# SoyeonHH/MMDA

Measured on AMD Instinct MI355X. Metric: training samples/sec on MOSEI-shaped synthetic batch, higher is better.
Workload: dtype bf16; 1 GPU; MISA train step, MOSEI shapes B=32/GPU T=50 (d_t,d_v,d_a)=(300,35,74) hidden=128 V=20000, bf16 MFMA operands fp32 accumulate, dropout on, full lengths; global_batch=32, seq_len=50, parallelism=single, use_confidNet=False, rnncell=lstm, dp_global_stats=False

## Files before the change

include/mmda_hip.h:

```cpp
#ifndef MMDA_HIP_H
#define MMDA_HIP_H
#include <stddef.h>
#include <stdint.h>

#ifdef __cplusplus
extern "C" {
#endif

#define MMDA_F32 0
#define MMDA_BF16 1

#define MMDA_CELL_LSTM 0
#define MMDA_CELL_GRU 1

#define MMDA_OK 0
#define MMDA_EINVAL (-1)
#define MMDA_ELAUNCH (-2)

#define MMDA_ACT_NONE 0
#define MMDA_ACT_RELU 1
#define MMDA_ACT_SIGMOID 2
#define MMDA_ACT_LEAKYRELU 3
#define MMDA_ACT_TANH 4
#define MMDA_ACT_ELU 5
// ... 323 lines not shown
int mmda_clamp(float* g, int64_t n, float clip, void* stream);
int mmda_clamp_adam_rows(float* p, const float* g, float* m, float* v, int rows, int dim, const unsigned char* mask, int want, float lr,
                         float beta1, float beta2, float eps, float clip, float grad_scale, int step, void* stream);
int mmda_mark_rows(unsigned char* mask, int rows, const int64_t* ids, int n, void* stream);
int mmda_embed_rows_sparse_adam(float* P, float* M, float* V, const int64_t* ids, int n, int D, const float* rows, const int32_t* lengths,
                                int B, int table_rows, float lr, float beta1, float beta2, float eps, float clip, float grad_scale, int step,
                                void* stream);
int64_t mmda_embed_deferred_scalar_floats(int window);
int mmda_embed_deferred_reset(int32_t* row_step, int table_rows, void* stream);
int mmda_embed_rows_dense_adam(float* P, float* M, float* V, int32_t* row_step, float* step_scalars, int window, const int64_t* ids, int n,
                               int D, const float* rows, const int32_t* lengths, int B, int table_rows, float lr, float beta1, float beta2,
                               float eps, float clip, float grad_scale, int seq, int step, void* stream);
int mmda_embed_rows_catch_up(float* P, float* M, float* V, int32_t* row_step, const float* step_scalars, int window, const int64_t* ids,
                             int n, int D, const int32_t* lengths, int B, int table_rows, float beta1, float beta2, float eps, int upto,
                             void* stream);
int mmda_embed_rows_flush(float* P, float* M, float* V, int32_t* row_step, const float* step_scalars, int window, int D, int table_rows,
                          float beta1, float beta2, float eps, int upto, void* stream);
int mmda_clamp_rmsprop(float* p, const float* g, float* square_avg, int64_t n, float lr, float alpha, float eps, float clip,
                       float grad_scale, void* stream);
int mmda_grad_accumulate(float* acc, const float* g, int64_t n, int first, void* stream);
int mmda_clamp_adam_sum(float* p, const float* acc, const float* g, float* m, float* v, int64_t n, float lr, float beta1, float beta2,
                        float eps, float clip, float grad_scale, int step, void* stream);
int mmda_embed_rows_append(int64_t* ids_out, float* rows_out, int64_t offset, int64_t capacity, const int64_t* ids, const float* rows,
                           int n, int D, const int32_t* lengths, int B, void* stream);
typedef struct mmda_run { int64_t begin, len, first; } mmda_run;
int64_t mmda_runs_build(const int64_t* begin, const int64_t* len, int n, int64_t bucket_floats, mmda_run* out, int* n_out);
int mmda_clamp_adam_runs(float* p, const float* g, float* m, float* v, const mmda_run* runs, int n_runs, int64_t items, float lr,
                         float beta1, float beta2, float eps, float clip, float grad_scale, int step, void* stream);
int mmda_clamp_adam_sum_runs(float* p, const float* acc, const float* g, float* m, float* v, const mmda_run* runs, int n_runs,
                             int64_t items, float lr, float beta1, float beta2, float eps, float clip, float grad_scale, int step,
                             void* stream);
int mmda_clamp_rmsprop_runs(float* p, const float* g, float* square_avg, const mmda_run* runs, int n_runs, int64_t items, float lr,
                            float alpha, float eps, float clip, float grad_scale, void* stream);
typedef struct mmda_adam_opts {
  float beta1, beta2, eps, weight_decay;
  int decoupled;
  const float* scale_dev;
} mmda_adam_opts;
int mmda_clamp_adam_opts(float* p, const float* acc, const float* g, float* m, float* v, int64_t n, const mmda_run* runs, int n_runs,
                         int64_t items, float lr, float clip, float grad_scale, int step, const mmda_adam_opts* opts, void* stream);
int mmda_clamp_adam_rows_opts(float* p, const float* g, float* m, float* v, int rows, int dim, const unsigned char* mask, int want, float lr,
                              float clip, float grad_scale, int step, const mmda_adam_opts* opts, void* stream);
int64_t mmda_grad_norm_partials(int64_t n_or_items);
int mmda_grad_norm(const float* g, const float* acc, int64_t n, const mmda_run* runs, int n_runs, int64_t items, float max_norm,
                   float grad_scale, double* partials, int64_t partials_capacity, float* out2, void* stream);
int mmda_grad_scale(float* g, int64_t n, const mmda_run* runs, int n_runs, int64_t items, const float* scale_dev, void* stream);

typedef struct mmda_misa mmda_misa;
typedef struct mmda_misa_config {
  int vocab, d_t, d_v, d_a, hidden, ncls;
  int act;
  int use_cmd_sim, use_confidNet;
  float dropout;
  float fusion_dropout;
  float threshold, reverse_grad_weight;
  float diff_weight, sim_weight, recon_weight, conf_weight;
  int mode;
  int rnncell;
} mmda_misa_config;

int mmda_misa_create(const mmda_misa_config* cfg, mmda_misa** out);
void mmda_misa_destroy(mmda_misa* m);
int mmda_misa_num_params(const mmda_misa* m);
int mmda_misa_param_info(const mmda_misa* m, int i, const char** name, int64_t* offset, int* rows, int* cols);
int64_t mmda_misa_flat_floats(const mmda_misa* m);
int64_t mmda_misa_dense_floats(const mmda_misa* m);
int mmda_misa_bind(mmda_misa* m, float* params, float* grads, float* adam_m, float* adam_v);
int64_t mmda_misa_workspace_floats(const mmda_misa* m, int B, int T);
#define MMDA_MISA_STEP_SWITCHES 13
typedef struct mmda_misa_step_request { int fused, has_labels, has_opt_step, enc_cached; } mmda_misa_step_request;
typedef struct mmda_misa_step_plan {
  int fused, inf, enc_cut, enc_nostash, enc_cached, bfg, gm, kdg, tn_wgrad, want_b, want_c, want_wT, wT_merge, skinny, row_fuse,
      ffn_fuse_fwd, ffn_fuse_bwd, seed_recon, seed_cls, fj_on, fj_fwd, fj_device, zg_here, rec_hoisted, sort_early, embed_update,
      embed_deferred, embed_bg, embed_bg_late, embed_bg_wgs, embed_bg_lds;
} mmda_misa_step_plan;
int mmda_misa_plan_describe(const mmda_misa* m, int B, int T, const mmda_misa_step_request* req, const int* switches, int n_switches,
                            mmda_misa_step_plan* out);
int mmda_misa_set_workspace(mmda_misa* m, float* ws, int64_t floats, int B, int T);
int mmda_misa_set_workspace_async(mmda_misa* m, float* ws, int64_t floats, int B, int T, void* stream);
int64_t mmda_misa_tensor_offset(const mmda_misa* m, const char* name);
int mmda_misa_set_mode(mmda_misa* m, int mode);
int mmda_misa_set_recurrence(mmda_misa* m, int resident_weights);
int mmda_misa_set_gemm_operands(mmda_misa* m, int bf16_copies);
int mmda_misa_set_inference(mmda_misa* m, int forward_only);
int mmda_misa_set_fusion_fp8(mmda_misa* m, int on);
int mmda_misa_set_embed_update(mmda_misa* m, int mode);
int mmda_misa_set_trainable(mmda_misa* m, const unsigned char* flags, int n_params);
int mmda_misa_trainable_info(const mmda_misa* m, mmda_run* runs, int capacity, int* n_runs, int64_t* trainable_floats, int* encoder_cut_on);
int mmda_misa_set_cut_forward(mmda_misa* m, int keep_stash);
int mmda_misa_set_embed_deferred(mmda_misa* m, int32_t* row_step, float* step_scalars, int window, void* stream);
int mmda_misa_embed_deferred_step(mmda_misa* m, float lr, float beta1, float beta2, float eps, float clip, float grad_scale, int step,
                                  void* stream);
int mmda_misa_embed_flush(mmda_misa* m, void* stream);
int mmda_misa_set_embed_background(mmda_misa* m, int on, int workgroups);
int mmda_misa_embed_background_active(const mmda_misa* m);
int64_t mmda_misa_early_grad_floats(const mmda_misa* m);
int mmda_misa_wait_early_grads(mmda_misa* m, void* stream);
int mmda_misa_set_overlap(mmda_misa* m, int side_stream);
int mmda_misa_cluster_status(const mmda_misa* m, int* aborted_host);

int mmda_misa_forward(mmda_misa* m, const int64_t* t_ids, const float* v, const float* a, const int32_t* lengths,
                      int training, uint64_t seed, void* stream);
int mmda_misa_losses(mmda_misa* m, const float* emo, int with_grads, void* stream);
int mmda_misa_set_external_batch_losses(mmda_misa* m, int on);
int mmda_misa_backward(mmda_misa* m, const int64_t* t_ids, const float* v, const float* a, const int32_t* lengths,
                       void* stream);
int mmda_misa_zero_grad(mmda_misa* m, void* stream);
int mmda_misa_zero_act_grads(mmda_misa* m, void* stream);
int mmda_misa_adam_step(mmda_misa* m, float lr, float clip, float grad_scale, int step, void* stream);
int mmda_misa_set_adam(mmda_misa* m, const mmda_adam_opts* opts, float clip_norm);
int mmda_misa_set_cls_loss(mmda_misa* m, const mmda_cls_opts* opts);
int mmda_misa_set_task(mmda_misa* m, int task, int loss_kind);
int mmda_misa_grad_accumulate(mmda_misa* m, float* acc, int first, int64_t* list_ids, float* list_rows, int64_t list_used,
                              int64_t list_capacity, void* stream);
int mmda_misa_adam_step_accumulated(mmda_misa* m, const float* acc, int64_t* list_ids, float* list_rows, int64_t list_used,
                                    int64_t list_capacity, float lr, float clip, float grad_scale, int step, void* stream);
int mmda_misa_train_step(mmda_misa* m, const int64_t* t_ids, const float* v, const float* a, const int32_t* lengths,
                         const float* emo, int training, uint64_t seed, int do_adam, float lr, float clip, int step,
                         void* stream);

int mmda_misa_timing_stride(mmda_misa* m, int stride);
int mmda_misa_timing_rotate(mmda_misa* m, int on);
int mmda_misa_timing_begin(mmda_misa* m, int max_steps);
int mmda_misa_timing_collect(mmda_misa* m, float mean_ms[4], int* steps);
int mmda_misa_timing_end(mmda_misa* m);

int mmda_collate_gather(const int32_t* words, const float* visual, const float* acoustic, const int64_t* offsets, const float* emo,
                        const float* sentiment, const int32_t* order, int B, int T, int dv, int da, int pad_id, int64_t* out_ids,
                        float* out_v, float* out_a, float* out_emo, float* out_y, void* stream);

typedef struct mmda_infer_src {
  const float* scores; const float* labels; const float* tcp; const float* hfused; const float* x6; const float* probs;
  int ncls, hs, nhead;
} mmda_infer_src;
typedef struct mmda_infer_out {
  float* scores; float* labels; float* tcp; float* hidden; float* utterance; float* attention;
} mmda_infer_out;
int mmda_infer_collect(const mmda_infer_src* src, const mmda_infer_out* out, const int32_t* dst, int64_t base, int B, void* stream);
int mmda_misa_infer_collect(mmda_misa* m, const mmda_infer_out* out, const int32_t* dst, int64_t base, void* stream);

int mmda_encoded_collect(const float* utt_t, const float* utt_v, const float* utt_a, int wt, int wv, int wa, float* tab_t, float* tab_v,
                         float* tab_a, const int32_t* dst, int64_t base, int B, void* stream);
int mmda_encoded_gather(const float* tab_t, const float* tab_v, const float* tab_a, int wt, int wv, int wa, const float* tab_emo, int ncls,
                        const int32_t* rows, int B, float* utt_t, float* utt_v, float* utt_a, float* emo, void* stream);
int mmda_misa_encoded_collect(mmda_misa* m, float* tab_t, float* tab_v, float* tab_a, const int32_t* dst, int64_t base, void* stream);
typedef struct mmda_encoded_batch {
  const float* tab_t; const float* tab_v; const float* tab_a; const float* tab_emo;
  const int32_t* rows; int B;
} mmda_encoded_batch;
int mmda_misa_forward_encoded(mmda_misa* m, const mmda_encoded_batch* eb, int training, uint64_t seed, void* stream);
int mmda_misa_train_step_encoded(mmda_misa* m, const mmda_encoded_batch* eb, float* emo_out, int training, uint64_t seed, int do_adam,
                                 float lr, float clip, int step, void* stream);

typedef struct mmda_modality_p { float p[3]; } mmda_modality_p;
int mmda_collate_gather_masked(const int32_t* words, const float* visual, const float* acoustic, const int64_t* offsets, const float* emo,
                               const float* sentiment, const int32_t* order, int B, int T, int dv, int da, int pad_id, int keep_const,
                               mmda_modality_p p, uint64_t seed, int unk_id, int64_t* out_ids, float* out_v, float* out_a,
                               float* out_emo, float* out_y, uint8_t* out_keep, void* stream);
int mmda_modality_mask(const int64_t* ids, const float* v, const float* a, int T, int B, int dv, int da, const uint8_t* keep,
                       int keep_const, int pad_id, int unk_id, int64_t* out_ids, float* out_v, float* out_a, void* stream);
int mmda_modality_attrib(const float* V, int64_t n, int C, float* phi, float* loo, int32_t* dominant, int64_t* counts, void* stream);

#ifdef __cplusplus
}
#endif
#endif
// ... 1 lines not shown
```

mmda_amd/_lib.py:

```python
from __future__ import annotations

import ctypes as C
import os

_HERE = os.path.dirname(os.path.abspath(__file__))
LIB_PATH = os.path.join(_HERE, "libmmda_hip.so")

F32, BF16 = 0, 1
ACT = {"none": 0, "relu": 1, "sigmoid": 2, "leakyrelu": 3, "tanh": 4, "elu": 5, "hardtanh": 6, "hardshrink": 7, "prelu": 8, "rrelu": 9}

c_f32p = C.c_void_p
c_stream = C.c_void_p


class GemmArgs(C.Structure):
    _fields_ = [("mode", C.c_int), ("transA", C.c_int), ("transB", C.c_int), ("M", C.c_int), ("N", C.c_int), ("K", C.c_int),
                ("batch", C.c_int),
                ("A", C.c_void_p), ("lda", C.c_int), ("strideA", C.c_int64),
                ("A2", C.c_void_p), ("gather", C.c_void_p),
                ("B", C.c_void_p), ("ldb", C.c_int), ("strideB", C.c_int64),
                ("C", C.c_void_p), ("ldc", C.c_int), ("strideC", C.c_int64),
                ("bias", C.c_void_p), ("bias2", C.c_void_p), ("strideBias", C.c_int64),
                ("accumulate", C.c_int), ("act", C.c_int),
                ("drop_p", C.c_float), ("drop_seed", C.c_uint64), ("drop_site", C.c_int),
                ("gate", C.c_void_p), ("ldgate", C.c_int), ("gate_scale", C.c_float),
                ("alpha", C.c_float), ("bias_grad", C.c_void_p), ("bias_grad2", C.c_void_p)]


class GemmBf16Args(C.Structure):
    _fields_ = [("M", C.c_int), ("N", C.c_int), ("K", C.c_int), ("A", C.c_void_p), ("lda", C.c_int), ("B", C.c_void_p), ("ldb", C.c_int),
                ("C", C.c_void_p), ("ldc", C.c_int), ("bias", C.c_void_p), ("bias2", C.c_void_p), ("bias_grad", C.c_void_p),
                ("bias_grad2", C.c_void_p), ("accumulate", C.c_int), ("alpha", C.c_float), ("perm_n_H", C.c_int), ("perm_m_H", C.c_int),
                ("tn", C.c_int)]


class GemmBf16PlanRow(C.Structure):
    _fields_ = [("cls", C.c_int), ("mixed", C.c_int), ("tx", C.c_int), ("ty", C.c_int), ("sk", C.c_int), ("per", C.c_int),
                ("last", C.c_int), ("launch", C.c_int)]


class ConvertJob(C.Structure):
    _fields_ = [("src", C.c_void_p), ("ld", C.c_int), ("rows", C.c_int), ("cols", C.c_int), ("gather", C.c_void_p),
                ("plain", C.c_void_p), ("ldp", C.c_int), ("transposed", C.c_void_p), ("ldt", C.c_int), ("row_perm_H", C.c_int),
                ("src_bf16", C.c_int)]


class SkinnyArgs(C.Structure):
    _fields_ = [("M", C.c_int), ("N", C.c_int), ("K", C.c_int), ("transB", C.c_int),
                ("A", C.c_void_p), ("A2", C.c_void_p), ("lda", C.c_int), ("B", C.c_void_p), ("ldb", C.c_int),
                ("K2", C.c_int), ("A_2nd", C.c_void_p), ("lda_2nd", C.c_int), ("B_2nd", C.c_void_p), ("ldb_2nd", C.c_int),
                ("C", C.c_void_p), ("ldc", C.c_int), ("C2", C.c_void_p), ("ldc2", C.c_int), ("bias", C.c_void_p),
                ("accumulate", C.c_int), ("alpha", C.c_float), ("act", C.c_int),
                ("drop_p", C.c_float), ("drop_seed", C.c_uint64), ("drop_site", C.c_int),
                ("gate", C.c_void_p), ("ldgate", C.c_int), ("gate_scale", C.c_float),
                ("dsig", C.c_void_p), ("dsig2", C.c_void_p), ("lddsig", C.c_int)]


class TransposeJob(C.Structure):
    _fields_ = [("src", C.c_void_p), ("rows", C.c_int), ("cols", C.c_int), ("ld", C.c_int), ("dst", C.c_void_p), ("ldd", C.c_int)]


class ActParams(C.Structure):
    _fields_ = [("slope", C.c_void_p), ("dslope", C.c_void_p), ("lo", C.c_float), ("hi", C.c_float), ("rand", C.c_int),
                ("seed", C.c_uint64), ("site", C.c_int)]


class LnArgs(C.Structure):
    _fields_ = [("rows", C.c_int), ("n", C.c_int), ("x", C.c_void_p), ("res", C.c_void_p), ("gamma", C.c_void_p),
                ("beta", C.c_void_p), ("y", C.c_void_p), ("mean", C.c_void_p), ("rstd", C.c_void_p), ("act", C.c_int),
                ("drop_p", C.c_float), ("drop_seed", C.c_uint64), ("drop_site", C.c_int),
                ("permute_S", C.c_int), ("permute_B", C.c_int), ("eps", C.c_float), ("actp", ActParams),
                ("y_bf16", C.c_void_p), ("ld_bf16", C.c_int)]


class LnBwdArgs(C.Structure):
    _fields_ = [("rows", C.c_int), ("n", C.c_int), ("dy", C.c_void_p), ("x", C.c_void_p), ("res", C.c_void_p),
                ("gamma", C.c_void_p), ("mean", C.c_void_p), ("rstd", C.c_void_p),
                ("d_x", C.c_void_p), ("accumulate_dx", C.c_int), ("d_res", C.c_void_p),
                ("dgamma", C.c_void_p), ("dbeta", C.c_void_p),
                ("act", C.c_int), ("drop_p", C.c_float), ("drop_seed", C.c_uint64), ("drop_site", C.c_int),
                ("permute_S", C.c_int), ("permute_B", C.c_int), ("actp", ActParams)]


class LstmDesc(C.Structure):
    _fields_ = [("H", C.c_int), ("gates", C.c_void_p), ("cstash", C.c_void_p), ("hseq", C.c_void_p),
                ("wpack", C.c_void_p * 2), ("wpack_c", C.c_void_p * 2), ("utt", C.c_void_p), ("layer", C.c_int), ("d_hseq", C.c_void_p),
                ("xchg", C.c_void_p), ("epoch_base", C.c_uint32), ("gate_minor", C.c_int), ("forward_only", C.c_int),
                ("cell", C.c_int), ("dg_bf16", C.c_void_p), ("dg_bf16_only", C.c_int)]


class LstmPlan(C.Structure):
    _fields_ = [("ok", C.c_int), ("form", C.c_int), ("wpb", C.c_int), ("groups", C.c_int), ("groups_per_launch", C.c_int),
                ("launches", C.c_int), ("wg_per_group", C.c_int), ("wg_per_desc", C.c_int * 4), ("gru", C.c_int),
                ("gate_minor", C.c_int), ("no_stash", C.c_int), ("dhseq", C.c_int), ("pair", C.c_int),
                ("kernel", C.c_int)]


class MisaStepRequest(C.Structure):
    _fields_ = [("fused", C.c_int), ("has_labels", C.c_int), ("has_opt_step", C.c_int), ("enc_cached", C.c_int)]


STEP_PLAN_FIELDS = ("fused", "inf", "enc_cut", "enc_nostash", "enc_cached", "bfg", "gm", "kdg", "tn_wgrad", "want_b", "want_c", "want_wT",
                    "wT_merge", "skinny", "row_fuse", "ffn_fuse_fwd", "ffn_fuse_bwd", "seed_recon", "seed_cls", "fj_on", "fj_fwd",
                    "fj_device", "zg_here", "rec_hoisted", "sort_early", "embed_update", "embed_deferred", "embed_bg", "embed_bg_late",
                    "embed_bg_wgs", "embed_bg_lds")
STEP_SWITCHES = {"MMDA_GEMM_TN": 1, "MMDA_WT_MERGE": 1, "MMDA_ROW_FUSE": 1, "MMDA_FFN_FUSE": 1, "MMDA_LOSS_SEEDS": 1, "MMDA_FLAG_JOIN": 1,
                 "MMDA_ZERO_GRAD_SIDE": -1, "MMDA_FUSED_SPLIT": 1, "MMDA_SORT_EARLY": 1, "MMDA_EMBED_BG": 1, "MMDA_EMBED_BG_WGS": 0,
                 "MMDA_EMBED_BG_LATE": 0, "MMDA_EMBED_BG_LDS": 1024}


class MisaStepPlan(C.Structure):
    _fields_ = [(k, C.c_int) for k in STEP_PLAN_FIELDS]


class LossForms(C.Structure):
    _fields_ = [("diff_form", C.c_int), ("diff_products", C.c_int), ("diff_loss_sum", C.c_int), ("diff_combine_blocks", C.c_int),
                ("cmd_form", C.c_int), ("cmd_grid", C.c_int), ("recon_blocks", C.c_int), ("misc_recon_blocks", C.c_int)]


class RankPlan(C.Structure):
    _fields_ = [("rows_per_wg", C.c_int), ("tile", C.c_int), ("tiles", C.c_int), ("splits", C.c_int), ("tiles_per_split", C.c_int),
                ("grid_x", C.c_int), ("grid_y", C.c_int), ("grid_z", C.c_int), ("counts_bytes", C.c_int64)]


class GruPadJob(C.Structure):
    _fields_ = [("H", C.c_int), ("D", C.c_int), ("w_ih", C.c_void_p * 2), ("w_hh", C.c_void_p * 2), ("b_ih", C.c_void_p * 2),
                ("b_hh", C.c_void_p * 2), ("pw_ih", C.c_void_p), ("pw_hh", C.c_void_p * 2), ("pb_ih", C.c_void_p), ("pb_hh", C.c_void_p)]


class MisaConfig(C.Structure):
    _fields_ = [("vocab", C.c_int), ("d_t", C.c_int), ("d_v", C.c_int), ("d_a", C.c_int), ("hidden", C.c_int), ("ncls", C.c_int),
                ("act", C.c_int), ("use_cmd_sim", C.c_int), ("use_confidNet", C.c_int),
                ("dropout", C.c_float), ("fusion_dropout", C.c_float), ("threshold", C.c_float),
                ("reverse_grad_weight", C.c_float),
                ("diff_weight", C.c_float), ("sim_weight", C.c_float), ("recon_weight", C.c_float), ("conf_weight", C.c_float),
                ("mode", C.c_int), ("rnncell", C.c_int)]


# ... 103 lines not shown
    "mmda_attn_bwd": (_I, [_P, _P, _P, _I, _I, _I, _I, _P, _F, _U64, _I, _P]),
    "mmda_add": (_I, [_P, _P, _P, _I64, _P]),
    "mmda_sigmoid_bwd_inplace": (_I, [_P, _P, _I64, _P]),
    "mmda_act_dropout_fwd": (_I, [_P, _P, _I64, _I, _F, _U64, _I, _P]),
    "mmda_act_dropout_bwd": (_I, [_P, _P, _P, _I64, _I, _F, _U64, _I, _P]),
    "mmda_act_dropout_fwd_p": (_I, [_P, _P, _I64, _I, C.POINTER(ActParams), _F, _U64, _I, _P]),
    "mmda_act_dropout_bwd_p": (_I, [_P, _P, _P, _I64, _I, C.POINTER(ActParams), _F, _U64, _I, _P]),
    "mmda_heads_fwd": (_I, [_P, _I, _I, _F, _P, _P, _P, _F, _U64, _I, _P]),
    "mmda_heads_bwd": (_I, [_P, _P, _P, _P, _I, _I, _P, _F, _U64, _I, _P]),
    "mmda_heads_fwd_task": (_I, [_P, _I, _I, _F, _P, _P, _P, _F, _U64, _I, _I, _P]),
    "mmda_heads_bwd_task": (_I, [_P, _P, _P, _P, _I, _I, _P, _F, _U64, _I, _I, _P]),
    "mmda_loss_reg": (_I, [_P, _P, _I, _I, _I, _F, _P, _P, _P]),
    "mmda_senti_accumulate": (_I, [_P, _P, _I64, _P, _P]),
    "mmda_senti_finish": (_I, [_P, _P, _P]),
    "mmda_reliab_accumulate": (_I, [_P, _P, _I64, _I, _I, _P, _P]),
    "mmda_reliab_finish": (_I, [_P, _I, _I, _P, _P, _P]),
    "mmda_scaling_work_bytes": (_I64, [_I64, _I]),
    "mmda_scaling_fit": (_I, [_P, _P, _I64, _I, _I, _I, _I, _P, _I64, _P, _P, _P, _P, _P]),
    "mmda_scaling_apply": (_I, [_P, _P, _P, _I64, _I, _P, _P]),
    "mmda_misa_set_task": (_I, [_P, _I, _I]),
    "mmda_loss_cls": (_I, [_P, _P, _I, _I, _F, _P, _P, _P]),
    "mmda_loss_cls_opts": (_I, [_P, _P, _I, _I, _F, _P, _P, C.POINTER(ClsOpts), _P]),
    "mmda_loss_misc_opts": (_I, [_P, _P, _P, _I, _I, _P, _P, _I, _I, _F, _P, _P, _I64, _F, _P, _P, _P, _F, _F, _F, _F, _I,
                                 C.POINTER(ClsOpts), _P]),
    "mmda_label_counts": (_I, [_P, _I64, _I, _P, _P]),
    "mmda_misa_set_cls_loss": (_I, [_P, C.POINTER(ClsOpts)]),
    "mmda_loss_conf": (_I, [_P, _P, _P, _I, _I, _F, _P, _P, _P, _P]),
    "mmda_loss_diff": (_I, [_P, _I64, _I, _I, _F, _P, _P, _P, _P]),
    "mmda_loss_diff_work_floats": (_I64, [_I, _I]),
    "mmda_loss_diff_pairs": (_I, [_P, _I64, _I, _I, C.POINTER(C.c_int), _I, _I, _F, _P, _P, _P, _P]),
    "mmda_loss_cmd_pairs": (_I, [_P, _I64, _I, _I, C.POINTER(C.c_int), _I, _I, _I, _F, _F, _P, _P, _P]),
    "mmda_loss_cmd": (_I, [_P, _I64, _I, _I, _F, _P, _P, _P]),
    "mmda_loss_recon": (_I, [_P, _P, _I64, _I, _I, _F, _P, _P, _P, _P]),
    "mmda_loss_misc": (_I, [_P, _P, _P, _I, _I, _P, _P, _I, _I, _F, _P, _P, _I64, _F, _P, _P, _P, _F, _F, _F, _F, _I, _P]),
    "mmda_eval_accumulate": (_I, [_P, _P, _I, _I, _P, _P]),
    "mmda_calib_accumulate": (_I, [_P, _P, _I64, _I, _P, _I, _P, _P, _P]),
    "mmda_calib_select": (_I, [_P, _P, _I, _I, _P, _I, _I, _P, _P, _P, _P]),
    "mmda_eval_accumulate_thr": (_I, [_P, _P, _I, _I, _P, _P, _P, _P]),
    "mmda_rank_plan_describe": (_I, [_I64, _I, C.POINTER(RankPlan)]),
    "mmda_rank_counts": (_I, [_P, _P, _I64, _I, _P, _P]),
    "mmda_rank_finish": (_I, [_P, _P, _I64, _I, C.c_double, _P, _P]),
    "mmda_rank_rows_accumulate": (_I, [_P, _P, _I64, _I, _P, _P]),
    "mmda_loss_domain": (_I, [_P, _I, _F, _P, _P, _P]),
    "mmda_loss_forms_describe": (_I, [_I, _I, _I, _I, _I, _I64, C.POINTER(LossForms)]),
    "mmda_clamp_adam": (_I, [_P, _P, _P, _P, _I64, _F, _F, _F, _F, _F, _F, _I, _P]),
    "mmda_clamp_adam_rows": (_I, [_P, _P, _P, _P, _I, _I, _P, _I, _F, _F, _F, _F, _F, _F, _I, _P]),
    "mmda_embed_rows_sparse_adam": (_I, [_P, _P, _P, _P, _I, _I, _P, _P, _I, _I, _F, _F, _F, _F, _F, _F, _I, _P]),
    "mmda_mark_rows": (_I, [_P, _I, _P, _I, _P]),
    "mmda_embed_deferred_scalar_floats": (_I64, [_I]),
    "mmda_embed_deferred_reset": (_I, [_P, _I, _P]),
    "mmda_embed_rows_dense_adam": (_I, [_P, _P, _P, _P, _P, _I, _P, _I, _I, _P, _P, _I, _I, _F, _F, _F, _F, _F, _F, _I, _I, _P]),
    "mmda_embed_rows_catch_up": (_I, [_P, _P, _P, _P, _P, _I, _P, _I, _I, _P, _I, _I, _F, _F, _F, _I, _P]),
    "mmda_embed_rows_flush": (_I, [_P, _P, _P, _P, _P, _I, _I, _I, _F, _F, _F, _I, _P]),
    "mmda_clamp": (_I, [_P, _I64, _F, _P]),
    "mmda_clamp_rmsprop": (_I, [_P, _P, _P, _I64, _F, _F, _F, _F, _F, _P]),
    "mmda_grad_accumulate": (_I, [_P, _P, _I64, _I, _P]),
    "mmda_clamp_adam_sum": (_I, [_P, _P, _P, _P, _P, _I64, _F, _F, _F, _F, _F, _F, _I, _P]),
    "mmda_embed_rows_append": (_I, [_P, _P, _I64, _I64, _P, _P, _I, _I, _P, _I, _P]),
    "mmda_runs_build": (_I64, [C.POINTER(_I64), C.POINTER(_I64), _I, _I64, C.POINTER(Run), C.POINTER(_I)]),
    "mmda_clamp_adam_runs": (_I, [_P, _P, _P, _P, _P, _I, _I64, _F, _F, _F, _F, _F, _F, _I, _P]),
    "mmda_clamp_adam_sum_runs": (_I, [_P, _P, _P, _P, _P, _P, _I, _I64, _F, _F, _F, _F, _F, _F, _I, _P]),
    "mmda_clamp_rmsprop_runs": (_I, [_P, _P, _P, _P, _I, _I64, _F, _F, _F, _F, _F, _P]),
    "mmda_clamp_adam_opts": (_I, [_P, _P, _P, _P, _P, _I64, _P, _I, _I64, _F, _F, _F, _I, C.POINTER(AdamOpts), _P]),
    "mmda_clamp_adam_rows_opts": (_I, [_P, _P, _P, _P, _I, _I, _P, _I, _F, _F, _F, _I, C.POINTER(AdamOpts), _P]),
    "mmda_grad_norm_partials": (_I64, [_I64]),
    "mmda_grad_norm": (_I, [_P, _P, _I64, _P, _I, _I64, _F, _F, _P, _I64, _P, _P]),
    "mmda_grad_scale": (_I, [_P, _I64, _P, _I, _I64, _P, _P]),
    "mmda_misa_set_adam": (_I, [_P, C.POINTER(AdamOpts), _F]),
    "mmda_misa_create": (_I, [C.POINTER(MisaConfig), C.POINTER(C.c_void_p)]),
    "mmda_misa_destroy": (None, [_P]),
    "mmda_misa_num_params": (_I, [_P]),
    "mmda_misa_param_info": (_I, [_P, _I, C.POINTER(C.c_char_p), C.POINTER(_I64), C.POINTER(_I), C.POINTER(_I)]),
    "mmda_misa_flat_floats": (_I64, [_P]),
    "mmda_misa_dense_floats": (_I64, [_P]),
    "mmda_misa_bind": (_I, [_P, _P, _P, _P, _P]),
    "mmda_misa_workspace_floats": (_I64, [_P, _I, _I]),
    "mmda_misa_plan_describe": (_I, [_P, _I, _I, C.POINTER(MisaStepRequest), C.POINTER(C.c_int), _I, C.POINTER(MisaStepPlan)]),
    "mmda_misa_set_workspace": (_I, [_P, _P, _I64, _I, _I]),
    "mmda_misa_set_workspace_async": (_I, [_P, _P, _I64, _I, _I, _P]),
    "mmda_misa_tensor_offset": (_I64, [_P, C.c_char_p]),
    "mmda_misa_set_mode": (_I, [_P, _I]),
    "mmda_misa_set_overlap": (_I, [_P, _I]),
    "mmda_misa_set_recurrence": (_I, [_P, _I]),
    "mmda_misa_set_gemm_operands": (_I, [_P, _I]),
    "mmda_misa_early_grad_floats": (_I64, [_P]),
    "mmda_misa_wait_early_grads": (_I, [_P, _P]),
    "mmda_misa_set_inference": (_I, [_P, _I]),
    "mmda_misa_set_fusion_fp8": (_I, [_P, _I]),
    "mmda_misa_set_embed_update": (_I, [_P, _I]),
    "mmda_misa_set_trainable": (_I, [_P, C.c_char_p, _I]),
    "mmda_misa_trainable_info": (_I, [_P, C.POINTER(Run), _I, C.POINTER(_I), C.POINTER(_I64), C.POINTER(_I)]),
    "mmda_misa_set_cut_forward": (_I, [_P, _I]),
    "mmda_misa_set_embed_deferred": (_I, [_P, _P, _P, _I, _P]),
    "mmda_misa_embed_deferred_step": (_I, [_P, _F, _F, _F, _F, _F, _F, _I, _P]),
    "mmda_misa_embed_flush": (_I, [_P, _P]),
    "mmda_misa_set_embed_background": (_I, [_P, _I, _I]),
    "mmda_misa_embed_background_active": (_I, [_P]),
    "mmda_misa_cluster_status": (_I, [_P, C.POINTER(_I)]),
    "mmda_misa_forward": (_I, [_P, _P, _P, _P, _P, _I, _U64, _P]),
    "mmda_misa_losses": (_I, [_P, _P, _I, _P]),
    "mmda_misa_set_external_batch_losses": (_I, [_P, _I]),
    "mmda_misa_backward": (_I, [_P, _P, _P, _P, _P, _P]),
    "mmda_misa_zero_grad": (_I, [_P, _P]),
    "mmda_misa_zero_act_grads": (_I, [_P, _P]),
    "mmda_misa_adam_step": (_I, [_P, _F, _F, _F, _I, _P]),
    "mmda_misa_grad_accumulate": (_I, [_P, _P, _I, _P, _P, _I64, _I64, _P]),
    "mmda_misa_adam_step_accumulated": (_I, [_P, _P, _P, _P, _I64, _I64, _F, _F, _F, _I, _P]),
    "mmda_misa_timing_stride": (_I, [_P, _I]),
    "mmda_misa_timing_rotate": (_I, [_P, _I]),
    "mmda_misa_timing_begin": (_I, [_P, _I]),
    "mmda_misa_timing_collect": (_I, [_P, C.POINTER(C.c_float * 4), C.POINTER(_I)]),
    "mmda_misa_timing_end": (_I, [_P]),
    "mmda_misa_train_step": (_I, [_P, _P, _P, _P, _P, _P, _I, _U64, _I, _F, _F, _I, _P]),
    "mmda_collate_gather": (_I, [_P, _P, _P, _P, _P, _P, _P, _I, _I, _I, _I, _I, _P, _P, _P, _P, _P, _P]),
    "mmda_infer_collect": (_I, [C.POINTER(InferSrc), C.POINTER(InferOut), _P, _I64, _I, _P]),
    "mmda_misa_infer_collect": (_I, [_P, C.POINTER(InferOut), _P, _I64, _P]),
    "mmda_encoded_collect": (_I, [_P, _P, _P, _I, _I, _I, _P, _P, _P, _P, _I64, _I, _P]),
    "mmda_encoded_gather": (_I, [_P, _P, _P, _I, _I, _I, _P, _I, _P, _I, _P, _P, _P, _P, _P]),
    "mmda_misa_encoded_collect": (_I, [_P, _P, _P, _P, _P, _I64, _P]),
    "mmda_misa_forward_encoded": (_I, [_P, C.POINTER(EncodedBatch), _I, _U64, _P]),
    "mmda_misa_train_step_encoded": (_I, [_P, C.POINTER(EncodedBatch), _P, _I, _U64, _I, _F, _F, _I, _P]),
    "mmda_collate_gather_masked": (_I, [_P, _P, _P, _P, _P, _P, _P, _I, _I, _I, _I, _I, _I, ModalityP, _U64, _I, _P, _P, _P, _P, _P, _P, _P]),
    "mmda_modality_mask": (_I, [_P, _P, _P, _I, _I, _I, _I, _P, _I, _I, _I, _P, _P, _P, _P]),
    "mmda_modality_attrib": (_I, [_P, _I64, _I, _P, _P, _P, _P, _P]),
}

_lib = None


class MMDAError(RuntimeError):
    pass


def load():
    global _lib
    if _lib is not None:
        return _lib
    if not os.path.exists(LIB_PATH):
        raise MMDAError(f"{LIB_PATH} not found: the HIP hot-path library is not built (make -C mmda_amd/csrc); "
                        "there is no CPU/PyTorch fallback")
    lib = C.CDLL(LIB_PATH)
    for name, (res, args) in SIGNATURES.items():
        fn = getattr(lib, name)
        fn.restype = res
        fn.argtypes = args
    _lib = lib
    return lib


def check(rc, what=""):
    if rc != 0:
        lib = load()
        msg = lib.mmda_last_error()
        raise MMDAError(f"{what} failed with code {rc}: {msg.decode() if msg else ''}")


def ptr(t):
    return None if t is None else t.data_ptr()


def stream_ptr():
    import torch
    return torch.cuda.current_stream().cuda_stream
```

mmda_amd/csrc/lstm.hip:

```cpp
#include "common.h"
#include "internal.h"
#include "convert_tile.h"
#include "transpose_tile.h"

namespace {

constexpr int NW = 4;
constexpr int MAXDESC = 4;

struct LstmLaunch {
  mmda_lstm_desc d[MAXDESC];
  int n, B, T, nbt;
  const int32_t* lengths;
};

__device__ __forceinline__ int pad16(int h) { return (h + 15) & ~15; }
__device__ __forceinline__ int pad32(int h) { return (h + 31) & ~31; }

template <int MODE>
__global__ void pack_kernel(int H, const float* __restrict__ W, void* outF, void* outB) {
  const int Hp = pad16(H), nHT = Hp / 16;
  const int per = (MODE == MMDA_BF16) ? 8 : 4;
  const int kspan = (MODE == MMDA_BF16) ? 32 : 16;
  const int KS = (MODE == MMDA_BF16) ? pad32(H) / 32 : Hp / 16;
// ... 432 lines not shown
  if (mode == MMDA_BF16) {
    int used = 0;
    int rc = mmda_lstm_cluster_launch(n, descs, B, T, lengths, stream, bwd, &used);
    if (rc != MMDA_OK) return rc;
    if (used) return MMDA_OK;
  }
  for (int i = 0; i < n; ++i)
    if (descs[i].gate_minor) return MMDA_EINVAL;
  int Hp = round_up(maxH, 16), Kp = round_up(maxH, 32);
  size_t lds;
  if (!bwd) lds = (mode == MMDA_BF16) ? (size_t)2 * 16 * (Kp + 8) * 2 : (size_t)2 * 16 * (Kp + 2) * 4;
  else lds = (mode == MMDA_BF16) ? (size_t)16 * (4 * Hp + 8) * 2 : (size_t)16 * (4 * Hp + 2) * 4;
  if (lds > 160 * 1024) return MMDA_EINVAL;
  int maxt = pick_maxt(n, descs);
  hipStream_t s = (hipStream_t)stream;
  int rc;
  const bool gru = descs[0].cell == MMDA_CELL_GRU;
#define PICK(MODE_)                                                                                              \
  (gru ? (bwd ? launch<MODE_, true, MMDA_CELL_GRU>(maxt, L, lds, s) : launch<MODE_, false, MMDA_CELL_GRU>(maxt, L, lds, s))  \
       : (bwd ? launch<MODE_, true, MMDA_CELL_LSTM>(maxt, L, lds, s) : launch<MODE_, false, MMDA_CELL_LSTM>(maxt, L, lds, s)))
  if (mode == MMDA_BF16) rc = PICK(MMDA_BF16);
  else rc = PICK(MMDA_F32);
#undef PICK
  if (rc != MMDA_OK) return rc;
  MMDA_CHECK_LAUNCH(bwd ? "mmda_lstm_bwd" : "mmda_lstm_fwd");
  return MMDA_OK;
}

}

extern "C" int64_t mmda_lstm_packed_bytes(int mode, int H, int backward) {
  if (H <= 0 || H > 512) return MMDA_EINVAL;
  int Hp = round_up(H, 16), nHT = Hp / 16;
  if (backward == 2) return mode == MMDA_BF16 ? (int64_t)nHT * nHT * 2 * 64 * 8 * 2 : MMDA_EINVAL;
  if (mode == MMDA_BF16) {
    int KS = round_up(H, 32) / 32, KSB = 4 * Hp / 32;
    return backward ? (int64_t)nHT * KSB * 64 * 8 * 2 : (int64_t)nHT * 4 * KS * 64 * 8 * 2;
  } else if (mode == MMDA_F32) {
    int KG = Hp / 16, KGB = 4 * Hp / 16;
    return backward ? (int64_t)nHT * KGB * 64 * 4 * 4 : (int64_t)nHT * 4 * KG * 64 * 4 * 4;
  }
  return MMDA_EINVAL;
}

extern "C" int mmda_lstm_pack_whh(int mode, int H, const float* whh, void* packed_fwd, void* packed_bwd, void* stream) {
  if (!whh || H <= 0 || H > 512 || (!packed_fwd && !packed_bwd)) return MMDA_EINVAL;
  hipStream_t s = (hipStream_t)stream;
  int64_t total = (mmda_lstm_packed_bytes(mode, H, 0) + mmda_lstm_packed_bytes(mode, H, 1)) / (mode == MMDA_BF16 ? 2 : 4);
  int blocks = (int)((total + 255) / 256);
  if (blocks > 2048) blocks = 2048;
  if (mode == MMDA_BF16) hipLaunchKernelGGL(pack_kernel<MMDA_BF16>, dim3(blocks), dim3(256), 0, s, H, whh, packed_fwd, packed_bwd);
  else if (mode == MMDA_F32) hipLaunchKernelGGL(pack_kernel<MMDA_F32>, dim3(blocks), dim3(256), 0, s, H, whh, packed_fwd, packed_bwd);
  else return MMDA_EINVAL;
  MMDA_CHECK_LAUNCH("mmda_lstm_pack_whh");
  return MMDA_OK;
}

namespace {
int pack_build(int mode, int n, const int* H, const float* const* whh, void* const* packed_fwd, void* const* packed_bwd,
               void* const* packed_c, PackMulti& P, int& blocks) {
  if (n <= 0 || n > 16 || !H || !whh || !packed_fwd || !packed_bwd || (mode != MMDA_BF16 && mode != MMDA_F32)) return MMDA_EINVAL;
  P.n = n;
  blocks = 0;
  for (int i = 0; i < n; ++i) {
    if (H[i] <= 0 || H[i] > 512 || !whh[i] || (!packed_fwd[i] && !packed_bwd[i])) return MMDA_EINVAL;
    P.H[i] = H[i]; P.W[i] = whh[i]; P.F[i] = packed_fwd[i]; P.Bk[i] = packed_bwd[i];
    P.Ck[i] = (packed_c && mode == MMDA_BF16) ? packed_c[i] : nullptr;
    P.start[i] = blocks;
    int64_t total = (mmda_lstm_packed_bytes(mode, H[i], 0) + mmda_lstm_packed_bytes(mode, H[i], 1)) / 16;
    if (P.Ck[i]) total += mmda_lstm_packed_bytes(mode, H[i], 2) / 16;
    blocks += (int)((total + 255) / 256);
  }
  for (int i = n; i < 16; ++i) { P.H[i] = P.H[0]; P.W[i] = P.W[0]; P.F[i] = P.F[0]; P.Bk[i] = P.Bk[0]; P.Ck[i] = P.Ck[0]; }
  for (int i = n; i <= 16; ++i) P.start[i] = blocks;
  return MMDA_OK;
}
}

int mmda_lstm_pack_convert_transpose_stamped(int n, const int* H, const float* const* whh, void* const* packed_fwd, void* const* packed_bwd,
                                             void* const* packed_c, const mmda_convert_job* jobs, int njobs, const mmda_transpose_job* tjobs,
                                             int ntjobs, const RowStamp* st, void* stream) {
  if (!jobs || njobs < 0 || njobs > CONV_MAX) return MMDA_EINVAL;
  if (st && (!st->stamp || !st->ids || st->n < 0 || st->table_rows <= 0)) return MMDA_EINVAL;
  PackMulti P;
  int pblocks = 0, cblocks = 0, tblocks = 0;
  int rc = pack_build(MMDA_BF16, n, H, whh, packed_fwd, packed_bwd, packed_c, P, pblocks);
  if (rc) return rc;
  ConvLaunch L;
  rc = conv_build(jobs, njobs, L, cblocks);
  if (rc) return rc;
  TrLaunch R;
  rc = tr_build(tjobs, ntjobs, R, tblocks);
  if (rc) return rc;
  if (pblocks + cblocks + tblocks == 0) return st ? MMDA_EINVAL : MMDA_OK;
  hipLaunchKernelGGL(pack_convert_kernel, dim3(pblocks + cblocks + tblocks), dim3(256), 0, (hipStream_t)stream, P, L, R, pblocks,
                     pblocks + cblocks, st ? *st : RowStamp{nullptr, 0u, 0, nullptr, 0});
  MMDA_CHECK_LAUNCH("mmda_lstm_pack_convert_transpose");
  return MMDA_OK;
}

extern "C" int mmda_lstm_pack_convert_transpose(int n, const int* H, const float* const* whh, void* const* packed_fwd,
                                                void* const* packed_bwd, void* const* packed_c, const mmda_convert_job* jobs, int njobs,
                                                const mmda_transpose_job* tjobs, int ntjobs, void* stream) {
  return mmda_lstm_pack_convert_transpose_stamped(n, H, whh, packed_fwd, packed_bwd, packed_c, jobs, njobs, tjobs, ntjobs, nullptr, stream);
}

extern "C" int mmda_lstm_pack_whh_and_convert(int n, const int* H, const float* const* whh, void* const* packed_fwd, void* const* packed_bwd,
                                              void* const* packed_c, const mmda_convert_job* jobs, int njobs, void* stream) {
  return mmda_lstm_pack_convert_transpose(n, H, whh, packed_fwd, packed_bwd, packed_c, jobs, njobs, nullptr, 0, stream);
}

extern "C" int mmda_lstm_pack_whh_multi(int mode, int n, const int* H, const float* const* whh, void* const* packed_fwd,
                                        void* const* packed_bwd, void* const* packed_c, void* stream) {
  PackMulti P;
  int blocks = 0;
  const int rc0 = pack_build(mode, n, H, whh, packed_fwd, packed_bwd, packed_c, P, blocks);
  if (rc0) return rc0;
  hipStream_t s = (hipStream_t)stream;
  if (mode == MMDA_BF16) hipLaunchKernelGGL(pack_multi_kernel<MMDA_BF16>, dim3(blocks), dim3(256), 0, s, P);
  else hipLaunchKernelGGL(pack_multi_kernel<MMDA_F32>, dim3(blocks), dim3(256), 0, s, P);
  MMDA_CHECK_LAUNCH("mmda_lstm_pack_whh_multi");
  return MMDA_OK;
}

extern "C" int mmda_lstm_pack_whh_cluster(int H, const float* whh, void* packed_c, void* stream) {
  if (!whh || !packed_c || H <= 0 || H > 512) return MMDA_EINVAL;
  PackMulti P;
  P.n = 1;
  for (int i = 0; i < 16; ++i) { P.H[i] = H; P.W[i] = whh; P.F[i] = nullptr; P.Bk[i] = nullptr; P.Ck[i] = packed_c; }
  const int64_t total = (mmda_lstm_packed_bytes(MMDA_BF16, H, 0) + mmda_lstm_packed_bytes(MMDA_BF16, H, 1) +
                         mmda_lstm_packed_bytes(MMDA_BF16, H, 2)) / 16;
  const int blocks = (int)((total + 255) / 256);
  P.start[0] = 0;
  for (int i = 1; i <= 16; ++i) P.start[i] = blocks;
  hipLaunchKernelGGL(pack_multi_kernel<MMDA_BF16>, dim3(blocks), dim3(256), 0, (hipStream_t)stream, P);
  MMDA_CHECK_LAUNCH("mmda_lstm_pack_whh_cluster");
  return MMDA_OK;
}

namespace {
struct GruPad { mmda_gru_pad_job j[MMDA_GRU_PAD_MAX]; int start[MMDA_GRU_PAD_MAX + 1]; int n; };

template <bool UNPAD>
__global__ void gru_pad_kernel(GruPad P) {
  int i = 0;
#pragma unroll
  for (int k = 1; k < MMDA_GRU_PAD_MAX; ++k)
    if (k < P.n && (int)blockIdx.x >= P.start[k]) i = k;
  const mmda_gru_pad_job& J = P.j[i];
  const int H = J.H, D = J.D;
  const int64_t nih = (int64_t)8 * H * D, nhh = (int64_t)4 * H * H, nb = 8 * H;
  int64_t e = (int64_t)(blockIdx.x - P.start[i]) * blockDim.x + threadIdx.x;
  if (e < nih) {
    const int row = (int)(e / D), col = (int)(e % D);
    const int dir = row / (4 * H), slot = (row % (4 * H)) / H, u = row % H;
    float* t = J.w_ih[dir] + ((int64_t)slot * H + u) * D + col;
    if (!UNPAD) J.pw_ih[e] = slot < 3 ? *t : 0.f;
    else { float v = J.pw_ih[e]; J.pw_ih[e] = 0.f; if (slot < 3) *t += v; }
    return;
  }
  e -= nih;
  if (e < 2 * nhh) {
    const int dir = (int)(e / nhh);
    const int64_t e3 = e % nhh;
    const int row = (int)(e3 / H), col = (int)(e3 % H), slot = row / H, u = row % H;
    const int tg = slot == 3 ? 2 : slot;
    float* t = J.w_hh[dir] + ((int64_t)tg * H + u) * H + col;
    if (!UNPAD) J.pw_hh[dir][e3] = slot != 2 ? *t : 0.f;
    else { float v = J.pw_hh[dir][e3]; J.pw_hh[dir][e3] = 0.f; if (slot != 2) *t += v; }
    return;
  }
  e -= 2 * nhh;
  if (e < nb) {
    const int dir = (int)e / (4 * H), slot = ((int)e % (4 * H)) / H, u = (int)e % H;
    const int tg = slot == 3 ? 2 : slot;
    float* ti = J.b_ih[dir] + slot * H + u;
    float* th = J.b_hh[dir] + tg * H + u;
    if (!UNPAD) {
      J.pb_ih[e] = slot < 3 ? *ti : 0.f;
      J.pb_hh[e] = slot != 2 ? *th : 0.f;
    } else {
      float v = J.pb_ih[e]; J.pb_ih[e] = 0.f;
      if (slot < 3) *ti += v;
      if (slot != 2) *th += v;
    }
  }
// ... 36 lines not shown
```

mmda_amd/csrc/misa.hip:

```cpp
#include "step_plan.h"
#include <algorithm>
#include <cstring>

using namespace mmda_step;

namespace {

enum { SITE_ATTN = 1, SITE_DROP1 = 2, SITE_FFN = 3, SITE_DROP2 = 4, SITE_CLS = 5, SITE_DISC = 6,
       SITE_RRELU = 7 , SITE_RRELU_DISC = 10 };

struct OptStep { float lr, clip, grad_scale; int step; const float* acc; bool norm; };
struct PendingRows {
  const int64_t* ids = nullptr; const int32_t* lengths = nullptr; bool on = false;
  void set(const int64_t* i, const int32_t* l) { ids = i; lengths = l; on = true; }
  PendingRows take() { const PendingRows r = *this; *this = PendingRows{}; return r; }
};
struct RowList { int64_t* ids; float* rows; int64_t used, capacity; };
struct StepRequest {
  bool fused = false;
  const float* emo = nullptr;
  const OptStep* opt = nullptr;
  bool enc_cached = false;
};

}

struct mmda_misa {
  explicit mmda_misa(const mmda_misa_config& c) : cfg(c), par(build_params(c)) {}
  mmda_misa(const mmda_misa&) = delete;
  mmda_misa_config cfg;
  const ParamTable par;
  const Workspace& lay = lay_;
  void rebind(const Workspace& v) { lay_ = v; }
  float *P = nullptr, *G = nullptr, *M1 = nullptr, *V1 = nullptr;
  float* ws = nullptr;
  float* xchg_ws = nullptr; int xchg_B = 0; int abort_sticky = 0;
  mmda_adam_opts adam = {0.9f, 0.999f, 1e-8f, 0.f, 0, nullptr};
  float clip_norm = 0.f;
  mmda_cls_opts cls_opts = {}; int cls_on = 0;
  const mmda_cls_opts* cls() const { return cls_on ? &cls_opts : nullptr; }
  int reg = REG_NONE;
  int fusion_fp8 = 0;
  int embed_update = EU_DENSE;
  std::vector<mmda_run> runs;
  int prefix_frozen = 0;
  int embed_flag = 1;
  int enc_frozen = 0;
  int cut_keep_stash = 0;
  int32_t* df_row_step = nullptr; float* df_ring = nullptr; int df_window = 0;
  int use_side = 1;
  int use_cluster = 1;
  int use_bf16_gemm = 1;
  int inference = 0;
  int ext_batch_losses = 0;
  int ev_stride = 1;
  int ev_rotate = 0;
  hipStream_t side = nullptr;
  hipEvent_t ev_fork = nullptr, ev_join = nullptr, ev_pack = nullptr;
  hipEvent_t ev_early = nullptr;
  hipStream_t bg = nullptr; hipEvent_t ev_bg_fork = nullptr, ev_bg_done = nullptr;
  unsigned* row_stamp = nullptr; unsigned bg_epoch = 0u;
  int bg_on = -1, bg_wgs = 0;
  int bg_pending = 0, bg_active = 0;
  unsigned* jflags = nullptr;
  mmda_run* runs_dev = nullptr; int runs_dev_cap = 0; int runs_dirty = 1;
  std::vector<hipEvent_t> ev;
  StepPlan plan;
  int64_t early_floats = 0; int early_valid = 0;
  int64_t adam_early_done = 0;
  int wT_valid = 0;
  int wT_pending = 0;
  PendingRows eu;
  int df_seq = 0, df_flushed = 0;
  int training = 0; uint64_t seed = 0;
  unsigned epoch = 1;
  int side_pending = 0;
  int zero_grad_pending = 0;
  int eager_done = 0;
  const float* misc_deferred = nullptr;
  unsigned jval[2] = {0u, 0u};
  int esort_valid = 0; unsigned esort_val = 0u;
  int fj1 = 0, fj2 = 0, fj1_armed = 0;
  int ev_steps = 0, ev_fwd = 0, ev_bwd = 0;
  int ev_seen_f = 0, ev_seen_b = 0;
  std::vector<char> ev_done;

 private:
  Workspace lay_{};
};

namespace {

struct Ctx {
  mmda_misa* m; void* s; int rc = 0;
  bool grouping = false; std::vector<mmda_gemm_args> pending;
  bool absent_next = false; std::vector<mmda_gemm_args> absent;
  bool deferring = false; std::vector<mmda_gemm_args> deferred;
};

void group_begin(Ctx& c) { c.grouping = true; c.pending.clear(); c.absent.clear(); }
void group_end(Ctx& c) {
  c.grouping = false;
  if (!c.rc && !c.pending.empty())
    c.rc = mmda_gemm_grouped_sized(c.pending.data(), (int)c.pending.size(), c.absent.data(), (int)c.absent.size(), c.s);
  c.pending.clear(); c.absent.clear();
}

void gemm(Ctx& c, int mode, int tA, int tB, int M, int N, int K, const float* A, int lda, const float* Bp, int ldb, float* C,
          int ldc, const float* bias = nullptr, const float* bias2 = nullptr, int acc = 0, int act = 0, int batch = 1,
          int64_t sA = 0, int64_t sB = 0, int64_t sC = 0, int64_t sBias = 0, mmda_gemm_args* extra = nullptr) {
  if (c.rc) return;
  mmda_gemm_args g = {};
  if (extra) g = *extra;
  g.mode = mode; g.transA = tA; g.transB = tB; g.M = M; g.N = N; g.K = K; g.batch = batch;
  g.A = A; g.lda = lda; g.strideA = sA; g.B = Bp; g.ldb = ldb; g.strideB = sB; g.C = C; g.ldc = ldc; g.strideC = sC;
  g.bias = bias; g.bias2 = bias2; g.strideBias = sBias; g.accumulate = acc; g.act = act;
  if (c.absent_next) { c.absent_next = false; if (c.grouping) c.absent.push_back(g); return; }
  if (c.deferring && tA && acc) c.deferred.push_back(g);
  else if (c.grouping) c.pending.push_back(g);
  else c.rc = mmda_gemm(&g, c.s);
}

int side_fork(mmda_misa* m, void* main_stream, void** out);
int side_launch(mmda_misa* m, std::vector<mmda_gemm_args>& list, void* main_stream);
int side_join(mmda_misa* m, void* main_stream);
void lin_fwd(Ctx& c, int mode, int M, int N, int K, const float* x, const float* W, const float* b, float* y, int act = 0) {
  gemm(c, mode, 0, 1, M, N, K, x, K, W, K, y, N, b, nullptr, 0, act);
}
void lin_dx(Ctx& c, int mode, int M, int N, int K, const float* dy, const float* W, float* dx, int acc) {
  gemm(c, mode, 0, 0, M, K, N, dy, N, W, K, dx, K, nullptr, nullptr, acc);
}
void lin_dw(Ctx& c, int mode, int M, int N, int K, const float* dy, const float* x, float* dW, float* db) {
  mmda_gemm_args e = {};
  e.bias_grad = db;
  gemm(c, mode, 1, 0, N, K, M, dy, N, x, K, dW, K, nullptr, nullptr, 1, 0, 1, 0, 0, 0, 0, &e);
}

mmda_skinny_args sk_nt(int M, int N, int K, const float* x, int ldx, const float* W, const float* b, float* y, int ldy, int act = 0) {
  mmda_skinny_args g = {};
  g.M = M; g.N = N; g.K = K; g.transB = 1; g.A = x; g.lda = ldx; g.B = W; g.ldb = K; g.C = y; g.ldc = ldy; g.bias = b; g.act = act;
  return g;
}
mmda_skinny_args sk_nn(int M, int N, int K, const float* dy, int lddy, const float* W, float* dx, int lddx, int acc) {
  mmda_skinny_args g = {};
  g.M = M; g.N = K; g.K = N; g.transB = 0; g.A = dy; g.lda = lddy; g.B = W; g.ldb = K; g.C = dx; g.ldc = lddx; g.accumulate = acc;
  return g;
}
mmda_skinny_args sk_dx(int M, int N, int K, const float* dy, int lddy, const float* WT, float* dx, int lddx, int acc) {
  mmda_skinny_args g = {};
  g.M = M; g.N = K; g.K = N; g.transB = 1; g.A = dy; g.lda = lddy; g.B = WT; g.ldb = N; g.C = dx; g.ldc = lddx; g.accumulate = acc;
  return g;
}
mmda_skinny_args sk_dxw(bool wt, int M, int N, int K, const float* dy, int lddy, const float* WT, const float* W, float* dx, int lddx,
// ... 188 lines not shown
  *r0 = a; *n = b - a; *items = m->runs[b].first - m->runs[a].first;
}
int runs_ready(mmda_misa* m, void* stream) {
  if (!m->runs_dirty && m->runs_dev) return MMDA_OK;
  const int need = (int)m->runs.size();
  if (hipStreamSynchronize((hipStream_t)stream) != hipSuccess) return MMDA_ELAUNCH;
  if (m->side && hipStreamSynchronize(m->side) != hipSuccess) return MMDA_ELAUNCH;
  if (need > m->runs_dev_cap) {
    if (m->runs_dev) (void)hipFree(m->runs_dev);
    m->runs_dev = nullptr; m->runs_dev_cap = 0;
    const int cap = (int)m->par.params.size() + 1;
    if (hipMalloc(reinterpret_cast<void**>(&m->runs_dev), sizeof(mmda_run) * cap) != hipSuccess) { m->runs_dev = nullptr; return MMDA_ELAUNCH; }
    m->runs_dev_cap = cap;
  }
  if (hipMemcpy(m->runs_dev, m->runs.data(), sizeof(mmda_run) * need, hipMemcpyHostToDevice) != hipSuccess) return MMDA_ELAUNCH;
  m->runs_dirty = 0;
  return MMDA_OK;
}
constexpr mmda_adam_opts kAdamDefaults = {0.9f, 0.999f, 1e-8f, 0.f, 0, nullptr};
int bucket_adam(mmda_misa* m, int64_t lo, int64_t hi, const float* acc, float lr, float clip, float grad_scale, int step, const FlagWait& w,
                void* stream, const float* scale_dev = nullptr) {
  const AdamHyper h{lr, m->adam.beta1, m->adam.beta2, m->adam.eps, clip, grad_scale, step, m->adam.weight_decay, m->adam.decoupled, scale_dev};
  if (!masked(m)) return mmda_adam_launch(m->P + lo, acc ? acc + lo : nullptr, m->G + lo, m->M1 + lo, m->V1 + lo, hi - lo, nullptr, h, w, stream);
  int r0 = 0, n = 0; int64_t items = 0;
  runs_slice(m, lo, hi, &r0, &n, &items);
  if (n > 0 && (m->runs_dirty || !m->runs_dev)) return MMDA_EINVAL;
  const RunTable t{n > 0 ? m->runs_dev + r0 : nullptr, n, items};
  return mmda_adam_launch(m->P, acc, m->G, m->M1, m->V1, 0, &t, h, w, stream);
}
int bucket_norm(mmda_misa* m, const float* acc, float grad_scale, void* stream) {
  if (!m->ws || m->lay.gnorm < 0) return MMDA_EINVAL;
  double* parts = reinterpret_cast<double*>(m->ws + m->lay.gnorm_parts);
  const int64_t cap = mmda_grad_norm_partials(INT64_MAX);
  const int64_t hi = grad_floats(m);
  if (!masked(m)) return mmda_grad_norm_launch(m->G, acc, hi, nullptr, m->clip_norm, grad_scale, parts, cap, m->ws + m->lay.gnorm, stream);
  int r0 = 0, n = 0; int64_t items = 0;
  runs_slice(m, 0, hi, &r0, &n, &items);
  if (n > 0 && (m->runs_dirty || !m->runs_dev)) return MMDA_EINVAL;
  const RunTable t{n > 0 ? m->runs_dev + r0 : nullptr, n, items};
  return mmda_grad_norm_launch(m->G, acc, 0, &t, m->clip_norm, grad_scale, parts, cap, m->ws + m->lay.gnorm, stream);
}
bool adam_settings_refused(const mmda_misa* m) {
  if (m->adam.weight_decay > 0.f && m->df_row_step) return true;
  if (m->clip_norm > 0.f && (m->embed_update == EU_SPARSE || m->df_row_step)) return true;
  return false;
}
int apply_trainable(mmda_misa* m, const unsigned char* flags) {
  const int np = (int)m->par.params.size();
  std::vector<int64_t> begin, len;
  int prefix_frozen = 0, embed_flag = 1, enc_frozen = 1;
  for (int i = 0; i < np; ++i) {
    const ParamInfo& p = m->par.params[i];
    const bool on = !flags || flags[i] != 0;
    const std::string top = p.name.substr(0, p.name.find('.'));
    if (p.off == m->par.embed) embed_flag = on ? 1 : 0;
    else if (!on) prefix_frozen = 1;
    if (on && ((p.off >= m->par.rnn2_begin && p.off < m->par.embed) || top == "tlayer_norm" || top == "vlayer_norm" || top == "alayer_norm")) enc_frozen = 0;
    if (!on) continue;
    begin.push_back(p.off);
    len.push_back((i + 1 < np ? m->par.params[i + 1].off : m->par.flat) - p.off);
  }
  const int64_t cuts[3] = {m->par.rnn2_begin, m->par.rnn1_begin, m->par.embed};
  std::vector<mmda_run> runs(begin.size() + 1);
  int n = 0;
  const int64_t items = mmda_runs_build_cut(begin.data(), len.data(), (int)begin.size(), m->par.flat, cuts, 3, runs.data(), &n);
  if (items < 0) return MMDA_EINVAL;
  runs.resize(n + 1);
  runs[n] = mmda_run{m->par.flat, 0, items};
  m->runs.swap(runs);
  m->prefix_frozen = prefix_frozen; m->embed_flag = embed_flag; m->enc_frozen = enc_frozen;
  m->runs_dirty = 1;
  return MMDA_OK;
}

const StepSwitches& step_switches() {
  static const StepSwitches d, sw = {
      mmda_env_int("MMDA_GEMM_TN", d.gemm_tn), mmda_env_int("MMDA_WT_MERGE", d.wt_merge), mmda_env_int("MMDA_ROW_FUSE", d.row_fuse),
      mmda_env_int("MMDA_FFN_FUSE", d.ffn_fuse), mmda_env_int("MMDA_LOSS_SEEDS", d.loss_seeds), mmda_env_int("MMDA_FLAG_JOIN", d.flag_join),
      mmda_env_int("MMDA_ZERO_GRAD_SIDE", d.zero_grad_side), mmda_env_int("MMDA_FUSED_SPLIT", d.fused_split),
      mmda_env_int("MMDA_SORT_EARLY", d.sort_early), mmda_env_int("MMDA_EMBED_BG", d.embed_bg), mmda_env_int("MMDA_EMBED_BG_WGS", d.embed_bg_wgs),
      mmda_env_int("MMDA_EMBED_BG_LATE", d.embed_bg_late), mmda_env_int("MMDA_EMBED_BG_LDS", d.embed_bg_lds)};
  return sw;
}
PlanInput plan_input(const mmda_misa* m, const StepRequest& r, int B, int T) {
  PlanInput in = {};
  in.cfg = m->cfg; in.B = B; in.T = T;
  for (int i = 0; i < 3; ++i) { in.H[i] = m->par.mod[i].H; in.xchg[i] = mmda_lstm_xchg_bytes(in.H[i], B) > 0; }
  in.use_side = m->use_side != 0; in.use_cluster = m->use_cluster != 0; in.use_bf16_gemm = m->use_bf16_gemm != 0;
  in.inference = m->inference != 0; in.fusion_fp8 = m->fusion_fp8 != 0;
  in.embed_update = m->embed_update; in.embed_deferred = m->embed_update == EU_DENSE && m->df_row_step != nullptr;
  in.masked = masked(m); in.encoder_cut = encoder_cut(m); in.cut_keep_stash = m->cut_keep_stash != 0;
  in.bg_on = m->bg_on; in.bg_wgs = m->bg_wgs; in.moments = m->M1 && m->V1;
  in.fused = r.fused; in.has_labels = r.emo != nullptr; in.has_opt = r.opt != nullptr; in.enc_cached = r.enc_cached;
  return in;
}

}

extern "C" int mmda_misa_create(const mmda_misa_config* cfg, mmda_misa** out) {
  if (!cfg || !out) return MMDA_EINVAL;
  if (cfg->vocab <= 0 || cfg->d_t <= 0 || cfg->d_v <= 0 || cfg->d_a <= 0 || cfg->hidden <= 0 || cfg->ncls <= 0) return MMDA_EINVAL;
  if (cfg->d_t > 512 || cfg->d_v > 512 || cfg->d_a > 512 || cfg->hidden % NHEAD || cfg->hidden > 1024) return MMDA_EINVAL;
  if (cfg->mode != MMDA_F32 && cfg->mode != MMDA_BF16) return MMDA_EINVAL;
  if (cfg->rnncell != MMDA_CELL_LSTM && cfg->rnncell != MMDA_CELL_GRU) return MMDA_EINVAL;
  mmda_misa* m = new mmda_misa(*cfg);
  if (apply_trainable(m, nullptr)) { delete m; return MMDA_EINVAL; }
  *out = m;
  return MMDA_OK;
}
extern "C" void mmda_misa_destroy(mmda_misa* m) {
  if (!m) return;
  if (m->ev_fork) (void)hipEventDestroy(m->ev_fork);
  if (m->ev_join) (void)hipEventDestroy(m->ev_join);
  if (m->ev_pack) (void)hipEventDestroy(m->ev_pack);
  if (m->ev_early) (void)hipEventDestroy(m->ev_early);
  if (m->bg) { (void)hipStreamSynchronize(m->bg); (void)hipStreamDestroy(m->bg); }
  if (m->ev_bg_fork) (void)hipEventDestroy(m->ev_bg_fork);
  if (m->ev_bg_done) (void)hipEventDestroy(m->ev_bg_done);
  if (m->row_stamp) (void)hipFree(m->row_stamp);
  if (m->side) (void)hipStreamDestroy(m->side);
  if (m->jflags) (void)hipFree(m->jflags);
  if (m->runs_dev) (void)hipFree(m->runs_dev);
  for (hipEvent_t e : m->ev) (void)hipEventDestroy(e);
  delete m;
}
extern "C" int mmda_misa_num_params(const mmda_misa* m) { return m ? (int)m->par.params.size() : MMDA_EINVAL; }
extern "C" int mmda_misa_param_info(const mmda_misa* m, int i, const char** name, int64_t* offset, int* rows, int* cols) {
  if (!m || i < 0 || i >= (int)m->par.params.size()) return MMDA_EINVAL;
  const ParamInfo& p = m->par.params[i];
  if (name) *name = p.name.c_str();
  if (offset) *offset = p.off;
  if (rows) *rows = p.rows;
  if (cols) *cols = p.cols;
  return MMDA_OK;
}
extern "C" int64_t mmda_misa_flat_floats(const mmda_misa* m) { return m ? m->par.flat : MMDA_EINVAL; }
extern "C" int64_t mmda_misa_dense_floats(const mmda_misa* m) { return m ? m->par.dense : MMDA_EINVAL; }
extern "C" int mmda_misa_bind(mmda_misa* m, float* params, float* grads, float* adam_m, float* adam_v) {
  if (!m || !params) return MMDA_EINVAL;
  if (((uintptr_t)params | (uintptr_t)grads | (uintptr_t)adam_m | (uintptr_t)adam_v) & 15) return MMDA_EINVAL;
  m->P = params; m->G = grads; m->M1 = adam_m; m->V1 = adam_v;
  return MMDA_OK;
}
extern "C" int64_t mmda_misa_workspace_floats(const mmda_misa* m, int B, int T) {
  if (!m || B <= 0 || T <= 0) return MMDA_EINVAL;
  return carve(m->cfg, m->par, B, T).floats;
}
extern "C" int mmda_misa_plan_describe(const mmda_misa* m, int B, int T, const mmda_misa_step_request* req, const int* switches,
                                       int n_switches, mmda_misa_step_plan* out) {
  if (!m || !req || !out || B <= 0 || T <= 0 || (switches && n_switches != MMDA_MISA_STEP_SWITCHES)) return MMDA_EINVAL;
  static const float labels = 0.f; static const OptStep opt = {};
  const StepRequest r{req->fused != 0, req->has_labels ? &labels : nullptr, req->has_opt_step ? &opt : nullptr, req->enc_cached != 0};
  StepSwitches sw;
  if (switches) memcpy(&sw, switches, sizeof(sw));
  const StepPlan P = plan_step(plan_input(m, r, B, T), sw);
  *out = mmda_misa_step_plan{P.fused, P.inf, P.enc_cut, P.enc_nostash, P.enc_cached, P.bfg, P.gm, P.kdg, P.tn_wgrad, P.want_b, P.want_c,
                             P.want_wT, P.wT_merge, P.skinny, P.row_fuse, P.ffn_fuse_fwd, P.ffn_fuse_bwd, P.seed_recon, P.seed_cls, P.fj_on,
                             P.fj_fwd, P.fj_device, P.zg_here, P.rec_hoisted, P.sort_early, P.embed_update, P.embed_deferred, P.embed_bg,
                             P.embed_bg_late, P.embed_bg_wgs, P.embed_bg_lds};
  return MMDA_OK;
}
namespace {
int harvest_abort(mmda_misa* m) {
  if (!m->ws || !m->xchg_ws || m->xchg_ws != m->ws) return MMDA_OK;
  for (int i = 0; i < 3; ++i) {
    if (m->lay.mod[i].xchg < 0) continue;
    unsigned w = 0;
    if (hipMemcpy(&w, m->ws + m->lay.mod[i].xchg, sizeof(w), hipMemcpyDeviceToHost) != hipSuccess) return MMDA_ELAUNCH;
    if (w) m->abort_sticky = 1;
  }
  return MMDA_OK;
}
}

extern "C" int mmda_misa_set_workspace_async(mmda_misa* m, float* ws, int64_t floats, int B, int T, void* stream) {
  if (!m || !ws || B <= 0 || T <= 0 || ((uintptr_t)ws & 15)) return MMDA_EINVAL;
  const Workspace w = carve(m->cfg, m->par, B, T);
  if (floats < w.floats) return MMDA_EINVAL;
  const bool keep = m->xchg_ws == ws && m->xchg_B == B;
  if (!keep && m->xchg_ws == ws) { int rc = harvest_abort(m); if (rc) return rc; }
  m->rebind(w);
  m->ws = ws;
  hipStream_t s = (hipStream_t)stream;
  if (!keep) {
    for (int i = 0; i < 3; ++i)
      if (w.mod[i].xchg >= 0 && hipMemsetAsync(ws + w.mod[i].xchg, 0, sizeof(float) * w.mod[i].xchg_floats, s) != hipSuccess) return MMDA_ELAUNCH;
    m->xchg_ws = ws; m->xchg_B = B;
  }
  if (w.gpad_end > w.gpad_begin && hipMemsetAsync(ws + w.gpad_begin, 0, sizeof(float) * (w.gpad_end - w.gpad_begin), s) != hipSuccess)
    return MMDA_ELAUNCH;
  return MMDA_OK;
}
extern "C" int mmda_misa_set_workspace(mmda_misa* m, float* ws, int64_t floats, int B, int T) {
  return mmda_misa_set_workspace_async(m, ws, floats, B, T, nullptr);
}
extern "C" int64_t mmda_misa_tensor_offset(const mmda_misa* m, const char* name) {
  if (!m || !name || !m->ws) return -1;
  return tensor_offset(m->lay, name);
}
extern "C" int mmda_misa_set_mode(mmda_misa* m, int mode) {
  if (!m || (mode != MMDA_F32 && mode != MMDA_BF16)) return MMDA_EINVAL;
  m->cfg.mode = mode;
  return MMDA_OK;
}
extern "C" int mmda_misa_set_overlap(mmda_misa* m, int side_stream) {
  if (!m) return MMDA_EINVAL;
  m->use_side = side_stream ? 1 : 0;
  return MMDA_OK;
}
extern "C" int mmda_misa_set_recurrence(mmda_misa* m, int resident_weights) {
  if (!m) return MMDA_EINVAL;
  m->use_cluster = resident_weights ? 1 : 0;
  return MMDA_OK;
}
extern "C" int mmda_misa_set_gemm_operands(mmda_misa* m, int bf16_copies) {
  if (!m) return MMDA_EINVAL;
  m->use_bf16_gemm = bf16_copies ? 1 : 0;
  return MMDA_OK;
}
extern "C" int64_t mmda_misa_early_grad_floats(const mmda_misa* m) {
  return (m && m->early_valid) ? m->early_floats : 0;
}
extern "C" int mmda_misa_wait_early_grads(mmda_misa* m, void* stream) {
  if (!m || !m->early_valid || !m->ev_early) return MMDA_EINVAL;
  if (hipStreamWaitEvent((hipStream_t)stream, m->ev_early, 0) != hipSuccess) return MMDA_ELAUNCH;
  return MMDA_OK;
}
extern "C" int mmda_misa_set_external_batch_losses(mmda_misa* m, int on) {
  if (!m) return MMDA_EINVAL;
  m->ext_batch_losses = on ? 1 : 0;
  return MMDA_OK;
}
extern "C" int mmda_misa_set_inference(mmda_misa* m, int forward_only) {
  if (!m) return MMDA_EINVAL;
  m->inference = forward_only ? 1 : 0;
  return MMDA_OK;
}
extern "C" int mmda_misa_cluster_status(const mmda_misa* m, int* aborted_host) {
  if (!m || !m->ws || !aborted_host) return MMDA_EINVAL;
  *aborted_host = m->abort_sticky;
  if (m->jflags) {
    unsigned w = 0;
    if (hipMemcpy(&w, m->jflags + 2, sizeof(w), hipMemcpyDeviceToHost) != hipSuccess) return MMDA_ELAUNCH;
    if (w) *aborted_host |= 2;
  }
  for (int i = 0; i < 3; ++i) {
    if (m->lay.mod[i].xchg < 0) continue;
    unsigned w = 0;
    if (hipMemcpy(&w, m->ws + m->lay.mod[i].xchg, sizeof(w), hipMemcpyDeviceToHost) != hipSuccess) return MMDA_ELAUNCH;
    if (w) *aborted_host = 1;
  }
  return MMDA_OK;
}

namespace {
void weight_transpose_jobs(mmda_misa* m, std::vector<mmda_transpose_job>& tj) {
  const mmda_misa_config& c = m->cfg;
  const ParamTable& p = m->par; const Workspace& w = m->lay;
  const int hs_ = c.hidden, NC_ = 6 + c.ncls;
  auto T_ = [&](int64_t src, int rows, int cols, int64_t dst) { tj.push_back(mmda_transpose_job{PP(src), rows, cols, cols, WS(dst), rows}); };
  T_(p.head_w, NC_, 6 * hs_, w.head_wT); T_(p.l2_w, hs_, FFN, w.l2_wT); T_(p.l1_w, FFN, hs_, w.l1_wT);
  T_(p.out_w, hs_, hs_, w.out_wT); T_(p.in_w, 3 * hs_, hs_, w.in_wT); T_(p.sh_w, hs_, hs_, w.sh_wT);
  for (int i = 0; i < 3; ++i) {
    T_(p.rec_w + (int64_t)i * hs_ * hs_, hs_, hs_, w.rec_wT + (int64_t)i * hs_ * hs_);
    T_(p.priv_w + (int64_t)i * hs_ * hs_, hs_, hs_, w.priv_wT + (int64_t)i * hs_ * hs_);
    T_(p.mod[i].pw, hs_, 4 * p.mod[i].H, w.pwT[i]);
  }
  if (!c.use_cmd_sim) { T_(p.d1_w, hs_, hs_, w.d1_wT); T_(p.d2_w, 3, hs_, w.d2_wT); }
}
int weight_transposes(mmda_misa* m, void* ss) {
  std::vector<mmda_transpose_job> tj;
  weight_transpose_jobs(m, tj);
  const int rc = mmda_transpose_f32(tj.data(), (int)tj.size(), ss);
  m->wT_valid = rc ? 0 : 1;
  m->wT_pending = 0;
  return rc;
}

int backward_only_jobs(mmda_misa* m, mmda_convert_job* cj) {
  const ParamTable& p = m->par; const Workspace& w = m->lay;
  const int R = w.B * w.T;
  int n = 0;
  for (int i = 0; i < 3; ++i) {
    const ModP& md = p.mod[i]; const ModW& mw = w.mod[i];
    for (int l = 0; l < 2; ++l) {
      const RnnP& r = md.rnn[l]; const RnnW& rw = mw.rnn[l];
      if (m->plan.tn_wgrad) {
        for (int d = 0; d < 2; ++d)
          cj[n++] = mmda_convert_job{WS(mw.hseq[l]) + d * md.H, 2 * md.H, R, md.H, nullptr, WS(rw.hbp[d]), r.ldH, nullptr, 0};
      } else {
        cj[n++] = mmda_convert_job{WS(mw.hseq[l]), 2 * md.H, R, 2 * md.H, nullptr, nullptr, 0, WS(rw.hbT), w.ldR};
      }
    }
    if (!m->plan.tn_wgrad) cj[n++] = mmda_convert_job{WS(mw.normed), 2 * md.H, R, 2 * md.H, nullptr, nullptr, 0, WS(mw.rnn[1].xbT), w.ldR};
  }
  return n;
}

int eager_side_losses(mmda_misa* m, void* stream) {
  const StepPlan& P = m->plan;
  if (!P.fused) return MMDA_OK;
  const mmda_misa_config& c = m->cfg; const Workspace& w = m->lay;
  const int B = w.B, hs = c.hidden;
  const int64_t BH = (int64_t)B * hs;
  void* ss = nullptr;
  int rc = side_fork(m, stream, &ss);
  if (!rc && m->wT_pending) rc = weight_transposes(m, B >= 128 ? stream : ss);
  const int64_t zend = P.seed_cls ? w.zero_cls : P.seed_recon ? w.zero_recon : w.zero_end;
  if (!rc && P.zg_here && m->zero_grad_pending) {
    rc = mmda_zero2(WS(w.zero_begin), zend - w.zero_begin, m->G, grad_floats(m), ss);
    m->zero_grad_pending = 0;
  } else if (!rc) {
    if (hipMemsetAsync(WS(w.zero_begin), 0, sizeof(float) * (zend - w.zero_begin), (hipStream_t)ss) != hipSuccess) rc = MMDA_ELAUNCH;
  }
  float* L = WS(w.losses);
  if (!rc) rc = mmda_loss_diff(WS(w.x6), BH, B, hs, c.diff_weight, L + 1, WS(w.d_x6), WS(w.diff_work), ss);
  m->fj1_armed = (!rc && c.use_cmd_sim && P.fj_fwd && m->jflags && mmda_loss_cmd_sets_flag(B, hs)) ? 1 : 0;
  if (!rc && c.use_cmd_sim) {
    static const int sim_pairs[6] = {0, 1, 0, 2, 2, 1};
    rc = mmda_loss_cmd_pairs_tail(WS(w.x6 + 3 * BH), BH, 3, 3, sim_pairs, 5, B, hs, c.sim_weight, 1.0f / 3.0f, L + 2, WS(w.d_x6 + 3 * BH), ss,
                                  m->fj1_armed ? m->jflags + 0 : nullptr, m->jval[0] + 1);
  }
  if (!rc && m->zero_grad_pending) { rc = mmda_misa_zero_grad(m, stream); m->zero_grad_pending = 0; }
  m->eager_done = 1;
  return rc;
}
}

namespace {
int ffn_fp8(mmda_misa* m, float p_tf, uint64_t seed, void* stream) {
  const mmda_misa_config& c = m->cfg; const ParamTable& p = m->par; const Workspace& w = m->lay;
  const int hs = c.hidden, R6 = 6 * w.B;
  if ((hs % 128) != 0) return MMDA_EINVAL;
  auto U8 = [&](int64_t off) { return reinterpret_cast<unsigned char*>(m->ws + off); };
  mmda_mx8_quant_job q[3] = {
      {m->ws + w.x1, hs, R6, hs, U8(w.x1q), U8(w.x1s)},
      {m->P + p.l1_w, hs, FFN, hs, U8(w.w1q), U8(w.w1s)},
      {m->P + p.l2_w, FFN, hs, FFN, U8(w.w2q), U8(w.w2s)}};
  int rc = mmda_mx8_quant(q, 3, stream);
  if (rc) return rc;
  mmda_mx8_args g = {};
  g.M = R6; g.N = FFN; g.K = hs; g.Aq = U8(w.x1q); g.As = U8(w.x1s); g.Bq = U8(w.w1q); g.Bs = U8(w.w1s);
  g.C = m->ws + w.f1; g.ldc = FFN; g.bias = m->P + p.l1_b; g.act = MMDA_ACT_RELU; g.drop_p = p_tf; g.drop_seed = seed; g.drop_site = SITE_FFN;
  rc = mmda_gemm_mx8(&g, stream);
  if (rc) return rc;
  mmda_mx8_quant_job qf = {m->ws + w.f1, FFN, R6, FFN, U8(w.f1q), U8(w.f1s)};
  rc = mmda_mx8_quant(&qf, 1, stream);
  if (rc) return rc;
  mmda_mx8_args h = {};
  h.M = R6; h.N = hs; h.K = FFN; h.Aq = U8(w.f1q); h.As = U8(w.f1s); h.Bq = U8(w.w2q); h.Bs = U8(w.w2s);
  h.C = m->ws + w.f2; h.ldc = hs; h.bias = m->P + p.l2_b;
  return mmda_gemm_mx8(&h, stream);
}
}

extern "C" int mmda_misa_set_adam(mmda_misa* m, const mmda_adam_opts* opts, float clip_norm) {
  if (!m || !(clip_norm >= 0.f)) return MMDA_EINVAL;
  const mmda_adam_opts o = opts ? *opts : kAdamDefaults;
  if (!mmda_adam_opts_valid(&o)) return MMDA_EINVAL;
// ... 117 lines not shown
    end = r.begin + r.len;
  }
  if (n_runs) *n_runs = n;
  if (trainable_floats) *trainable_floats = floats;
  if (encoder_cut_on) *encoder_cut_on = encoder_cut(m) ? 1 : 0;
  return MMDA_OK;
}
extern "C" int mmda_misa_set_cut_forward(mmda_misa* m, int keep_stash) {
  if (!m) return MMDA_EINVAL;
  m->cut_keep_stash = keep_stash ? 1 : 0;
  return MMDA_OK;
}

namespace {
struct Pass : Ctx {
  const StepPlan& P;
  const mmda_misa_config& c;
  const ParamTable& p; const Workspace& w;
  const int B, T, R, hs, NC, mode;
  static constexpr int fmode = MMDA_F32;
  const int64_t BH; const float p_tf, p_cls; const uint64_t seed;
  const float* emo; const OptStep* opt;
  Pass(mmda_misa* m_, void* s_, const float* emo_ = nullptr, const OptStep* opt_ = nullptr)
      : Ctx{m_, s_}, P(m_->plan), c(m_->cfg), p(m_->par), w(m_->lay), B(w.B), T(w.T), R(w.T * w.B), hs(c.hidden), NC(6 + c.ncls), mode(c.mode),
        BH((int64_t)B * hs), p_tf(m_->training ? c.fusion_dropout : 0.f), p_cls(m_->training ? c.dropout : 0.f), seed(m_->seed), emo(emo_), opt(opt_) {}
  mmda_ln_args proj_ln_fwd(int i), norm1_fwd(), norm2_fwd();
  mmda_ln_bwd_args proj_ln_bwd(int i), norm1_bwd(), norm2_bwd();
  void fwd_operands(const int64_t* t_ids, const float* const* xin);
  void fwd_encoder_layer(int l, const float* const* xin, const int32_t* lengths);
  void fwd_fusion_skinny(), fwd_fusion_tiled();
  void bwd_fusion_fused(), bwd_fusion_skinny(), bwd_fusion_tiled(), skinny_ffn_dx(bool wt), skinny_proj_dx(bool wt);
  void fusion_wgrads(), bwd_side_chain(bool pg_pending, const int64_t* t_ids, const int32_t* lengths);
  void bwd_encoder_layer(int l, const float* const* xin, const int64_t* t_ids, const int32_t* lengths);
  void bwd_text_rows(const int64_t* t_ids, const int32_t* lengths);
  const unsigned* take_sorted();
};

mmda_ln_args Pass::proj_ln_fwd(int i) {
  mmda_ln_args ln = {};
  ln.rows = B; ln.n = hs; ln.x = WS(w.z + i * BH); ln.gamma = PP(p.mod[i].plw); ln.beta = PP(p.mod[i].plb);
  ln.y = WS(w.orig + i * BH); ln.mean = WS(w.pmean + i * B); ln.rstd = WS(w.prstd + i * B); ln.act = c.act;
  ln.eps = 1e-5f; ln.actp = act_params(m, m->training, seed, SITE_RRELU + i, false);
  return ln;
}
mmda_ln_args Pass::norm1_fwd() {
  mmda_ln_args ln = {};
  ln.rows = 6 * B; ln.n = hs; ln.x = WS(w.x6); ln.res = WS(w.attn_out); ln.gamma = PP(p.n1_w); ln.beta = PP(p.n1_b);
  ln.y = WS(w.x1); ln.mean = WS(w.ln1_mean); ln.rstd = WS(w.ln1_rstd); ln.drop_p = p_tf; ln.drop_seed = seed;
  ln.drop_site = SITE_DROP1; ln.eps = 1e-5f;
  return ln;
}
mmda_ln_args Pass::norm2_fwd() {
  mmda_ln_args ln = {};
  ln.rows = 6 * B; ln.n = hs; ln.x = WS(w.x1); ln.res = WS(w.f2); ln.gamma = PP(p.n2_w); ln.beta = PP(p.n2_b);
  ln.y = WS(w.hfused); ln.mean = WS(w.ln2_mean); ln.rstd = WS(w.ln2_rstd); ln.drop_p = p_tf; ln.drop_seed = seed;
  ln.drop_site = SITE_DROP2; ln.permute_S = S6; ln.permute_B = B; ln.eps = 1e-5f;
  return ln;
}
mmda_ln_bwd_args Pass::proj_ln_bwd(int i) {
  mmda_ln_bwd_args l = {};
  l.rows = B; l.n = hs; l.dy = WS(w.d_orig + i * BH); l.x = WS(w.z + i * BH); l.gamma = PP(p.mod[i].plw);
  l.mean = WS(w.pmean + i * B); l.rstd = WS(w.prstd + i * B); l.d_x = WS(w.d_z + i * BH);
  l.dgamma = GG(p.mod[i].plw); l.dbeta = GG(p.mod[i].plb); l.act = c.act;
  l.actp = act_params(m, m->training, seed, SITE_RRELU + i, true);
  return l;
}
mmda_ln_bwd_args Pass::norm1_bwd() {
  mmda_ln_bwd_args l = {};
  l.rows = 6 * B; l.n = hs; l.dy = WS(w.d_x1); l.x = WS(w.x6); l.res = WS(w.attn_out); l.gamma = PP(p.n1_w);
  l.mean = WS(w.ln1_mean); l.rstd = WS(w.ln1_rstd); l.d_x = WS(w.d_x6); l.accumulate_dx = 1; l.d_res = WS(w.d_attn_out);
  l.dgamma = GG(p.n1_w); l.dbeta = GG(p.n1_b); l.drop_p = p_tf; l.drop_seed = seed; l.drop_site = SITE_DROP1;
  return l;
}
mmda_ln_bwd_args Pass::norm2_bwd() {
  mmda_ln_bwd_args l = {};
  l.rows = 6 * B; l.n = hs; l.dy = WS(w.d_hfused); l.x = WS(w.x1); l.res = WS(w.f2); l.gamma = PP(p.n2_w);
  l.mean = WS(w.ln2_mean); l.rstd = WS(w.ln2_rstd); l.d_x = WS(w.d_x1); l.d_res = WS(w.d_f2);
  l.dgamma = GG(p.n2_w); l.dbeta = GG(p.n2_b); l.drop_p = p_tf; l.drop_seed = seed; l.drop_site = SITE_DROP2;
  l.permute_S = S6; l.permute_B = B;
  return l;
}

void Pass::fwd_operands(const int64_t* t_ids, const float* const* xin) {
  auto first_jobs = [&](bool transposed, mmda_convert_job* cj) -> int {
    int n = 0;
    for (int i = 0; i < 3; ++i) {
      for (int l = 0; l < 2; ++l) {
        const RnnP& r = p.mod[i].rnn[l]; const RnnW& rw = w.mod[i].rnn[l];
        cj[n++] = mmda_convert_job{rW_ih(m, i, l), r.D, 8 * r.H, r.D, nullptr, WS(rw.wb), r.ldD,
                                   transposed ? WS(rw.wbT) : nullptr, transposed ? r.ldG : 0, P.gm ? r.H : 0};
      }
      const RnnP& r0 = p.mod[i].rnn[0]; const RnnW& rw0 = w.mod[i].rnn[0];
      const float* src = i == 0 ? PP(p.embed) : xin[i];
      const bool xt = transposed && !P.tn_wgrad;
      cj[n++] = mmda_convert_job{src, r0.D, R, r0.D, i == 0 ? t_ids : nullptr, WS(rw0.xb), r0.ldD, xt ? WS(rw0.xbT) : nullptr, xt ? w.ldR : 0};
    }
    return n;
  };
  m->wT_pending = 0;
  int Hs[12]; const float* Wp[12]; void* Fp[12]; void* Bp[12]; void* Cp[12];
  int k = 0;
  for (int i = 0; i < 3; ++i)
    for (int l = 0; l < 2; ++l)
      for (int d = 0; d < 2; ++d, ++k) {
        const RnnP& r = p.mod[i].rnn[l]; const RnnW& rw = w.mod[i].rnn[l];
        Hs[k] = r.H; Wp[k] = rW_hh(m, i, l, d); Fp[k] = WS(rw.pack_f[d]); Bp[k] = P.want_b ? WS(rw.pack_b[d]) : nullptr; Cp[k] = WS(rw.pack_c[d]);
      }
  m->wT_valid = 0;
  if (P.bfg) {
    mmda_convert_job cj[9];
    const int nj = first_jobs(!P.enc_nostash, cj);
    std::vector<mmda_transpose_job> tj;
    if (P.wT_merge) weight_transpose_jobs(m, tj);
    if (tj.size() > 20) tj.clear();
    RowStamp st;
    if (P.embed_bg) rc = bg_begin(m, t_ids, R, s, &st);
    if (!rc) rc = mmda_lstm_pack_convert_transpose_stamped(12, Hs, Wp, Fp, Bp, P.want_c ? Cp : nullptr, cj, nj, tj.data(), (int)tj.size(),
                                                           P.embed_bg ? &st : nullptr, s);
    m->wT_pending = (P.want_wT && tj.empty()) ? 1 : 0;
    if (!tj.empty()) m->wT_valid = rc ? 0 : 1;
  } else {
    void* ss = nullptr;
    rc = side_fork(m, s, &ss);
    if (!rc) rc = mmda_lstm_pack_whh_multi(mode, 12, Hs, Wp, Fp, Bp, P.want_c ? Cp : nullptr, ss);
    if (!rc && ss != s && hipEventRecord(m->ev_pack, (hipStream_t)ss) != hipSuccess) rc = MMDA_ELAUNCH;
    if (!rc && P.want_wT) rc = weight_transposes(m, ss);
    RowStamp st;
    if (!rc && P.embed_bg) rc = bg_begin(m, t_ids, R, s, &st);
    if (!rc) rc = mmda_embed_gather_stamped(PP(p.embed), t_ids, R, m->cfg.d_t, WS(w.mod[0].x), P.embed_bg ? &st : nullptr, s);
  }
  if (!rc && P.embed_bg && !P.embed_bg_late) rc = bg_launch(m, opt, s);
}

void Pass::fwd_encoder_layer(int l, const float* const* xin, const int32_t* lengths) {
  mmda_lstm_desc desc[3];
  mmda_gemm_bf16_args bg[3];
  group_begin(*this);
  for (int i = 0; i < 3; ++i) {
    const RnnP& r = p.mod[i].rnn[l]; const ModW& mw = w.mod[i]; const RnnW& rw = mw.rnn[l];
    const float* in = l == 0 ? xin[i] : WS(mw.normed);
    if (P.bfg) {
      bg[i] = mmda_gemm_bf16_args{};
      bg[i].M = R; bg[i].N = 8 * r.H; bg[i].K = r.D; bg[i].A = WS(rw.xb); bg[i].lda = r.ldD; bg[i].B = WS(rw.wb); bg[i].ldb = r.ldD;
      bg[i].C = WS(mw.gates[l]); bg[i].ldc = 8 * r.H; bg[i].bias = rB_ih(m, i, l); bg[i].bias2 = rB_hh(m, i, l);
      bg[i].perm_n_H = P.gm ? r.H : 0;
    } else {
      gemm(*this, mode, 0, 1, R, 8 * r.H, r.D, in, r.D, rW_ih(m, i, l), r.D, WS(mw.gates[l]), 8 * r.H, rB_ih(m, i, l), rB_hh(m, i, l));
    }
    desc[i] = lstm_desc(m, i, l, false, P.gm, false);
    desc[i].forward_only = P.enc_nostash;
  }
  if (P.bfg && !rc) rc = mmda_gemm_bf16_grouped(bg, 3, s);
  m->epoch += (unsigned)T + 2u;
  group_end(*this);
  if (!rc && l == 0 && m->side_pending && m->use_side) {
    if (hipStreamWaitEvent((hipStream_t)s, m->ev_pack, 0) != hipSuccess) rc = MMDA_ELAUNCH;
  }
  if (rc) return;
  ev_rec(m, m->ev_fwd, l, 0, s);
  rc = mmda_lstm_fwd(mode, 3, desc, B, T, lengths, s);
  ev_rec(m, m->ev_fwd, l, 1, s);
  if (rc) return;
  if (l == 0 && P.embed_bg && P.embed_bg_late) { rc = bg_launch(m, opt, s); if (rc) return; }
  if (l == 0) {
    mmda_ln_args ln[3];
    for (int i = 0; i < 3; ++i) {
      const ModP& md = p.mod[i]; const ModW& mw = w.mod[i];
      ln[i] = mmda_ln_args{};
      ln[i].rows = R; ln[i].n = 2 * md.H; ln[i].x = WS(mw.hseq[0]); ln[i].gamma = PP(md.ln_w); ln[i].beta = PP(md.ln_b);
      ln[i].y = WS(mw.normed); ln[i].mean = WS(mw.ln_mean); ln[i].rstd = WS(mw.ln_rstd); ln[i].eps = 1e-5f;
    }
    if (P.bfg)
      for (int i = 0; i < 3; ++i) { ln[i].y_bf16 = WS(w.mod[i].rnn[1].xb); ln[i].ld_bf16 = p.mod[i].rnn[1].ldD; }
    if (P.bfg && (P.enc_nostash || P.tn_wgrad))
      for (int i = 0; i < 3; ++i) ln[i].y = nullptr;
    rc = mmda_layernorm_fwd_multi(ln, 3, s);
  } else if (!P.fused && ((P.bfg && !P.enc_nostash) || m->zero_grad_pending || m->wT_pending)) {
    void* ss = nullptr;
    rc = side_fork(m, s, &ss);
    if (!rc && m->wT_pending) rc = weight_transposes(m, ss);
    if (!rc && m->zero_grad_pending && !P.fused) { rc = mmda_misa_zero_grad(m, ss); m->zero_grad_pending = 0; }
  }
}

void Pass::fwd_fusion_skinny() {
  mmda_skinny_args g[8];
  mmda_ln_args ln[3];
  for (int i = 0; i < 3; ++i) {
    const ModP& md = p.mod[i]; const ModW& mw = w.mod[i];
    g[i] = sk_nt(B, hs, 4 * md.H, WS(mw.utt), 4 * md.H, PP(md.pw), PP(md.pb), WS(w.z + i * BH), hs);
    ln[i] = proj_ln_fwd(i);
  }
  sk_launch(*this, g, 3);
  if (!rc) rc = mmda_layernorm_fwd_multi(ln, 3, s);
  for (int i = 0; i < 3; ++i)
    g[i] = sk_nt(B, hs, hs, WS(w.orig + i * BH), hs, PP(p.priv_w + (int64_t)i * hs * hs), PP(p.priv_b + i * hs), WS(w.x6 + i * BH), hs,
                 MMDA_ACT_SIGMOID);
  g[3] = sk_nt(3 * B, hs, hs, WS(w.orig), hs, PP(p.sh_w), PP(p.sh_b), WS(w.x6 + 3 * BH), hs, MMDA_ACT_SIGMOID);
  sk_launch(*this, g, 4);
  if (!rc) rc = eager_side_losses(m, s);
  const mmda_ln_args l1 = norm1_fwd();
  if (P.row_fuse) {
    if (!rc) {
      FusedFwdA f = {};
// ... 63 lines not shown
    if (!rc)
      rc = mmda_heads_fwd_task(WS(w.logits), B, c.ncls, c.threshold, WS(w.tcp), WS(w.scores), WS(w.labels), p_cls, seed, SITE_CLS,
                                 m->reg != REG_NONE, s);
  }
}

void Pass::fwd_fusion_tiled() {
  for (int i = 0; i < 3 && !rc; ++i) {
    const ModP& md = p.mod[i]; const ModW& mw = w.mod[i];
    lin_fwd(*this, fmode, B, hs, 4 * md.H, WS(mw.utt), PP(md.pw), PP(md.pb), WS(w.z + i * BH));
    if (rc) break;
    const mmda_ln_args ln = proj_ln_fwd(i);
    rc = mmda_layernorm_fwd(&ln, s);
  }
  gemm(*this, fmode, 0, 1, B, hs, hs, WS(w.orig), hs, PP(p.priv_w), hs, WS(w.x6), hs, PP(p.priv_b), nullptr, 0, MMDA_ACT_SIGMOID, 3,
       BH, (int64_t)hs * hs, BH, hs);
  gemm(*this, fmode, 0, 1, 3 * B, hs, hs, WS(w.orig), hs, PP(p.sh_w), hs, WS(w.x6 + 3 * BH), hs, PP(p.sh_b), nullptr, 0,
       MMDA_ACT_SIGMOID);
  if (!rc) rc = eager_side_losses(m, s);
  if (!rc) rc = mmda_add(WS(w.x6), WS(w.x6 + 3 * BH), WS(w.rsum), 3 * BH, s);
  gemm(*this, fmode, 0, 1, B, hs, hs, WS(w.rsum), hs, PP(p.rec_w), hs, WS(w.recon), hs, PP(p.rec_b), nullptr, 0, 0, 3, BH,
       (int64_t)hs * hs, BH, hs);
  if (!c.use_cmd_sim) {
    lin_fwd(*this, fmode, 3 * B, hs, hs, WS(w.x6 + 3 * BH), PP(p.d1_w), PP(p.d1_b), WS(w.dom_z));
    if (!rc) {
      const mmda_act_params ap = act_params(m, m->training, seed, SITE_RRELU_DISC, false);
      rc = mmda_act_dropout_fwd_p(WS(w.dom_z), WS(w.dom_h), 3 * BH, c.act, &ap, p_cls, seed, SITE_DISC, s);
    }
    lin_fwd(*this, fmode, 3 * B, 3, hs, WS(w.dom_h), PP(p.d2_w), PP(p.d2_b), WS(w.dom));
  }
  lin_fwd(*this, fmode, 6 * B, 3 * hs, hs, WS(w.x6), PP(p.in_w), PP(p.in_b), WS(w.qkv));
  if (!rc) rc = mmda_attn_fwd(WS(w.qkv), S6, B, hs, NHEAD, WS(w.ctx), WS(w.probs), p_tf, seed, SITE_ATTN, s);
  lin_fwd(*this, fmode, 6 * B, hs, hs, WS(w.ctx), PP(p.out_w), PP(p.out_b), WS(w.attn_out));
  const mmda_ln_args l1 = norm1_fwd(), l2 = norm2_fwd();
  if (!rc) rc = mmda_layernorm_fwd(&l1, s);
  if (m->fusion_fp8) {
    if (!rc) rc = ffn_fp8(m, p_tf, seed, s);
  } else {
    mmda_gemm_args e = {};
    e.drop_p = p_tf; e.drop_seed = seed; e.drop_site = SITE_FFN;
    gemm(*this, fmode, 0, 1, 6 * B, FFN, hs, WS(w.x1), hs, PP(p.l1_w), hs, WS(w.f1), FFN, PP(p.l1_b), nullptr, 0, MMDA_ACT_RELU, 1, 0,
         0, 0, 0, &e);
    lin_fwd(*this, fmode, 6 * B, hs, FFN, WS(w.f1), PP(p.l2_w), PP(p.l2_b), WS(w.f2));
  }
  if (!rc) rc = mmda_layernorm_fwd(&l2, s);
  lin_fwd(*this, fmode, B, NC, 6 * hs, WS(w.hfused), PP(p.head_w), PP(p.head_b), WS(w.logits));
  if (!rc)
    rc = mmda_heads_fwd_task(WS(w.logits), B, c.ncls, c.threshold, WS(w.tcp), WS(w.scores), WS(w.labels), p_cls, seed, SITE_CLS,
                               m->reg != REG_NONE, s);
}
}

namespace {
int forward_from_projections(Pass& x, void* stream) {
  mmda_misa* m = x.m;
  if (m->plan.skinny) x.fwd_fusion_skinny();
  else x.fwd_fusion_tiled();
  if (!x.rc && m->wT_pending) {
    void* ss = nullptr;
    x.rc = side_fork(m, stream, &ss);
    if (!x.rc) x.rc = weight_transposes(m, ss);
  }
  if (!x.rc && m->plan.fj_fwd && m->side_pending && m->jflags) {
    x.rc = side_flag_signal(m, 0, m->fj1_armed != 0);
    m->fj1 = x.rc ? 0 : 1; m->fj1_armed = 0;
    return x.rc;
  }
  if (m->fj1_armed) return MMDA_ELAUNCH;
  if (!x.rc) x.rc = side_join(m, stream);
  return x.rc;
}

bool encoded_batch_ok(const mmda_misa* m, const mmda_encoded_batch* eb) {
  return eb && eb->tab_t && eb->tab_v && eb->tab_a && eb->rows && eb->B > 0 && eb->B == m->lay.B;
}

int forward_encoded(mmda_misa* m, const StepRequest& req, const mmda_encoded_batch* eb, float* emo_out, int training, uint64_t seed,
                    void* stream) {
  m->training = training; m->seed = seed;
  m->plan = plan_step(plan_input(m, req, m->lay.B, m->lay.T), step_switches());
  Pass x(m, stream, req.emo, req.opt);
  m->wT_valid = 0;
  m->wT_pending = m->plan.want_wT ? 1 : 0;
  x.rc = mmda_encoded_gather(eb->tab_t, eb->tab_v, eb->tab_a, 4 * m->par.mod[0].H, 4 * m->par.mod[1].H, 4 * m->par.mod[2].H,
                             emo_out ? eb->tab_emo : nullptr, m->cfg.ncls, eb->rows, m->lay.B, WS(m->lay.mod[0].utt), WS(m->lay.mod[1].utt),
                             WS(m->lay.mod[2].utt), emo_out, stream);
  if (x.rc) return x.rc;
  return forward_from_projections(x, stream);
}

int forward_pass(mmda_misa* m, const StepRequest& req, const int64_t* t_ids, const float* v, const float* a, const int32_t* lengths,
                 int training, uint64_t seed, void* stream) {
  if (check_ready(m) || !t_ids || !v || !a || !lengths) return MMDA_EINVAL;
  m->training = training; m->seed = seed;
  m->plan = plan_step(plan_input(m, req, m->lay.B, m->lay.T), step_switches());
  Pass x(m, stream, req.emo, req.opt);
  if (is_gru(m)) {
    mmda_gru_pad_job gj[MMDA_GRU_PAD_MAX];
    int n = gru_jobs(m, m->P, false, gj);
    x.rc = mmda_gru_pad_params(gj, n, stream);
    if (x.rc) return x.rc;
  }
  if (m->plan.embed_deferred) {
    if (!m->M1 || !m->V1) return MMDA_EINVAL;
    x.rc = mmda_embed_rows_catch_up(PP(m->par.embed), m->M1 + m->par.embed, m->V1 + m->par.embed, m->df_row_step, m->df_ring, m->df_window, t_ids,
                                    m->lay.B * m->lay.T, m->cfg.d_t, lengths, m->lay.B, m->cfg.vocab, m->adam.beta1, m->adam.beta2, m->adam.eps, m->df_seq, stream);
    if (x.rc) return x.rc;
  }
  const float* xin[3] = {WS(m->lay.mod[0].x), v, a};
  x.fwd_operands(t_ids, xin);
  for (int l = 0; l < 2 && !x.rc; ++l) x.fwd_encoder_layer(l, xin, lengths);
  if (x.rc) return x.rc;
  if (!m->ev.empty()) { if (m->ev_seen_f % m->ev_stride == 0) m->ev_fwd++; m->ev_seen_f++; }
  return forward_from_projections(x, stream);
}
}

extern "C" int mmda_misa_forward_encoded(mmda_misa* m, const mmda_encoded_batch* eb, int training, uint64_t seed, void* stream) {
  if (check_ready(m) || !encoded_batch_ok(m, eb)) return MMDA_EINVAL;
  if (!m->inference && !encoder_cut(m)) return MMDA_EINVAL;
  return forward_encoded(m, StepRequest{false, nullptr, nullptr, true}, eb, nullptr, training, seed, stream);
}

extern "C" int mmda_misa_forward(mmda_misa* m, const int64_t* t_ids, const float* v, const float* a, const int32_t* lengths,
                                 int training, uint64_t seed, void* stream) {
  return forward_pass(m, StepRequest{}, t_ids, v, a, lengths, training, seed, stream);
}

extern "C" int mmda_misa_zero_act_grads(mmda_misa* m, void* stream) {
  if (check_ready(m)) return MMDA_EINVAL;
  if (hipMemsetAsync(WS(m->lay.zero_begin), 0, sizeof(float) * (m->lay.zero_end - m->lay.zero_begin), (hipStream_t)stream) != hipSuccess)
    return MMDA_ELAUNCH;
  return MMDA_OK;
}

extern "C" int mmda_misa_losses(mmda_misa* m, const float* emo, int with_grads, void* stream) {
  if (check_ready(m) || !emo) return MMDA_EINVAL;
  const mmda_misa_config& c = m->cfg; const Workspace& w = m->lay;
  const int B = w.B, hs = c.hidden;
  const int64_t BH = (int64_t)B * hs;
  hipStream_t s = (hipStream_t)stream;
  int rc = MMDA_OK;
  float* L = WS(w.losses);
  const bool ext = m->ext_batch_losses && with_grads && c.use_cmd_sim;
  const bool eager = (m->eager_done || ext) && with_grads;
  const bool s_recon = m->eager_done && with_grads && m->plan.seed_recon, s_cls = m->eager_done && with_grads && m->plan.seed_cls;
  m->eager_done = 0;
  if (eager) {
    rc = side_join(m, stream);
    if (rc) return rc;
  } else {
    if (with_grads) { rc = mmda_misa_zero_act_grads(m, stream); if (rc) return rc; }
    else if (hipMemsetAsync(WS(w.losses), 0, sizeof(float) * 8, s) != hipSuccess) return MMDA_ELAUNCH;
    rc = mmda_loss_diff(WS(w.x6), BH, B, hs, c.diff_weight, L + 1, with_grads ? WS(w.d_x6) : nullptr, WS(w.diff_work), stream);
    if (rc) return rc;
  }
  if (c.use_cmd_sim) {
    if (!eager) rc = mmda_loss_cmd(WS(w.x6 + 3 * BH), BH, B, hs, c.sim_weight, L + 2, with_grads ? WS(w.d_x6 + 3 * BH) : nullptr, stream);
  } else {
    rc = mmda_loss_domain(WS(w.dom), B, c.sim_weight, L + 2, with_grads ? WS(w.d_dom) : nullptr, stream);
  }
  if (rc) return rc;
  if (s_recon && s_cls && c.use_cmd_sim) {
    m->misc_deferred = emo;
    return MMDA_OK;
  }
// ... 259 lines not shown
      if (tn) { g.tn = 1; g.A = WS(rw.dgb); g.lda = r.ldG; g.B = WS(rw.xb); g.ldb = r.ldD; }
      wq.push_back(g);
    } else {
      mmda_gemm_args e = {};
      e.bias_grad = gB_ih(m, i, l); e.bias_grad2 = gB_hh(m, i, l);
      gemm(*this, mode, 1, 0, G8, r.D, R, dG, G8, in, r.D, gW_ih(m, i, l), r.D, nullptr, nullptr, 1, 0, 1, 0, 0, 0, 0, &e);
    }
    if (T > 1) {
      if (bf_hh) {
        mmda_gemm_bf16_args g = {};
        g.M = 4 * H; g.N = H; g.K = (T - 1) * B; g.lda = w.ldR; g.ldb = w.ldR; g.ldc = H; g.accumulate = 1;
        g.perm_m_H = P.gm ? H : 0;
        if (tn) {
          const unsigned short* dg = reinterpret_cast<const unsigned short*>(WS(rw.dgb));
          const unsigned short* h0 = reinterpret_cast<const unsigned short*>(WS(rw.hbp[0]));
          const unsigned short* h1 = reinterpret_cast<const unsigned short*>(WS(rw.hbp[1]));
          g.tn = 1; g.lda = r.ldG; g.ldb = r.ldH;
          g.A = dg + (int64_t)B * r.ldG; g.B = h0; g.C = gW_hh(m, i, l, 0);
          wq.push_back(g);
          g.A = dg + 4 * H; g.B = h1 + (int64_t)B * r.ldH; g.C = gW_hh(m, i, l, 1);
          wq.push_back(g);
        } else {
          g.A = dgT + B; g.B = hT; g.C = gW_hh(m, i, l, 0);
          wq.push_back(g);
          g.A = dgT + (int64_t)4 * H * w.ldR; g.B = hT + (int64_t)H * w.ldR + B; g.C = gW_hh(m, i, l, 1);
          wq.push_back(g);
        }
      } else {
        const float* hs_ = WS(mw.hseq[l]);
        gemm(*this, mode, 1, 0, 4 * H, H, (T - 1) * B, dG + (int64_t)B * G8, G8, hs_, 2 * H, gW_hh(m, i, l, 0), H, nullptr, nullptr, 1);
        gemm(*this, mode, 1, 0, 4 * H, H, (T - 1) * B, dG + 4 * H, G8, hs_ + (int64_t)B * 2 * H + H, 2 * H, gW_hh(m, i, l, 1), H, nullptr,
             nullptr, 1);
      }
    }
    if (l == 1 || i == 0) {
      float* dst = l == 1 ? WS(mw.d_normed) : WS(mw.d_x);
      const bool skip = l == 0 && frozen;
      if (bfg) {
        mmda_gemm_bf16_args g = {};
        g.M = R; g.N = r.D; g.K = G8; g.A = WS(rw.dgb); g.lda = r.ldG; g.B = WS(rw.wbT); g.ldb = r.ldG; g.C = dst; g.ldc = r.D;
        if (!skip) bmain.push_back(g);
      } else {
        absent_next = skip;
        gemm(*this, mode, 0, 0, R, r.D, G8, dG, G8, rW_ih(m, i, l), r.D, dst, r.D);
      }
    }
  }
  group_end(*this);
  deferring = false;
  if (!rc && !bmain.empty()) rc = mmda_gemm_bf16_grouped(bmain.data(), (int)bmain.size(), s);
  if (rc) return;
  if (l == 1) {
    mmda_ln_bwd_args lb[3];
    for (int i = 0; i < 3; ++i) {
      const ModP& md = p.mod[i]; const ModW& mw = w.mod[i];
      lb[i] = mmda_ln_bwd_args{};
      lb[i].rows = R; lb[i].n = 2 * md.H; lb[i].dy = WS(mw.d_normed); lb[i].x = WS(mw.hseq[0]); lb[i].gamma = PP(md.ln_w);
      lb[i].mean = WS(mw.ln_mean); lb[i].rstd = WS(mw.ln_rstd); lb[i].d_x = WS(mw.d_hseq1);
    }
    const bool ln_split = mmda_ln_bwd_parts_applies(lb, 3) &&
                          mmda_ln_parts_floats(lb, 3) <= (int64_t)512 * 2 * 2 * (p.mod[0].H + p.mod[1].H + p.mod[2].H);
    if (ln_split) {
      for (int i = 0; i < 3; ++i) { lb[i].dgamma = GG(p.mod[i].ln_w); lb[i].dbeta = GG(p.mod[i].ln_b); }
      rc = mmda_ln_bwd_parts(lb, 3, WS(w.ln_parts), s);
    } else {
      rc = mmda_layernorm_bwd_multi(lb, 3, s);
    }
    void* ss = nullptr;
    if (!rc) rc = side_fork(m, s, &ss);
    for (int i = 0; i < 3; ++i) { lb[i].dgamma = GG(p.mod[i].ln_w); lb[i].dbeta = GG(p.mod[i].ln_b); if (!ln_split) lb[i].d_x = nullptr; }
    if (!rc && dg_on_side) rc = mmda_convert_bf16(dgj, 3, ss);
    if (!rc) rc = ln_split ? mmda_ln_parts_finish(lb, 3, WS(w.ln_parts), ss) : mmda_layernorm_param_grads(lb, 3, ss);
    if (!rc && !deferred.empty()) rc = mmda_gemm_grouped(deferred.data(), (int)deferred.size(), ss);
    const bool l2_early = !bside.empty();
    if (!rc && l2_early) { rc = mmda_gemm_bf16_grouped(bside.data(), (int)bside.size(), ss); bside.clear(); }
    deferred.clear();
    if (rc) return;
    if (!m->ev_early && hipEventCreateWithFlags(&m->ev_early, hipEventDisableTiming) != hipSuccess) rc = MMDA_ELAUNCH;
    if (!rc && hipEventRecord(m->ev_early, (hipStream_t)ss) != hipSuccess) rc = MMDA_ELAUNCH;
    m->early_floats = (l2_early && !is_gru(m) && P.bfg) ? p.rnn1_begin : p.rnn2_begin;
    m->early_valid = 1;
    if (!rc && opt && m->early_floats > 0 && m->M1 && m->V1) {
      rc = bucket_adam(m, 0, m->early_floats, nullptr, opt->lr, opt->clip, opt->grad_scale, opt->step, kNoWait, ss);
      if (!rc) m->adam_early_done = m->early_floats;
    }
  } else {
    bwd_text_rows(t_ids, lengths);
  }
}

const unsigned* Pass::take_sorted() {
  if (!m->esort_valid) return nullptr;
  if (m->esort_valid == 2) {
    hipLaunchKernelGGL(flag_wait_kernel, dim3(1), dim3(64), 0, (hipStream_t)s, m->jflags + 3, m->esort_val, m->jflags + 2);
    if (hipGetLastError() != hipSuccess) rc = MMDA_ELAUNCH;
  }
  m->esort_valid = 0;
  return reinterpret_cast<const unsigned*>(WS(w.esort));
}

void Pass::bwd_text_rows(const int64_t* t_ids, const int32_t* lengths) {
  const float* dx = WS(w.mod[0].d_x);
  if (P.embed_update == EU_SPARSE || P.embed_deferred) {
    m->eu.take();
    if (!opt) { m->eu.set(t_ids, lengths); return; }
  }
  if (P.embed_update == EU_FROZEN) return;
  const EmbedList list{t_ids, take_sorted(), R, c.d_t, dx, lengths, B};
  if (rc) return;
  if (P.embed_update == EU_SPARSE) {
    SparseAdamArgs ad;
    rc = mmda_sparse_adam_args(&ad, PP(p.embed), m->M1 ? m->M1 + p.embed : nullptr, m->V1 ? m->V1 + p.embed : nullptr, c.vocab, opt->lr,
                               m->adam.beta1, m->adam.beta2, m->adam.eps, opt->clip, opt->grad_scale, opt->step);
    if (!rc) rc = mmda_embed_list_sparse_adam(ad, list, s);
  } else if (P.embed_deferred) {
    if (!m->M1 || !m->V1) { rc = MMDA_EINVAL; return; }
    rc = deferred_apply(m, t_ids, list.sorted, lengths, opt->lr, m->adam.beta1, m->adam.beta2, m->adam.eps, opt->clip, opt->grad_scale,
                        opt->step, false, s);
  } else {
    rc = mmda_embed_list_add(GG(p.embed), list, c.vocab, s);
  }
}
}

namespace {
int backward_pass(mmda_misa* m, const int64_t* t_ids, const float* v, const float* a, const int32_t* lengths, const OptStep* opt,
                  void* stream) {
  if (check_ready(m) || !m->G) return MMDA_EINVAL;
  if (m->plan.inf) return MMDA_EINVAL;
  if ((!t_ids || !v || !a || !lengths) && !(m->plan.enc_cached && m->plan.enc_cut)) return MMDA_EINVAL;
  if (m->plan.enc_cached && !m->plan.enc_cut) return MMDA_EINVAL;
  if (m->plan.enc_cut && !encoder_cut(m)) return MMDA_EINVAL;
  if (masked(m) && opt) { const int rr = runs_ready(m, stream); if (rr) return rr; }
  m->early_valid = 0; m->adam_early_done = 0;
  Pass x(m, stream, nullptr, opt);
  const StepPlan& P = m->plan;
  const bool row_fuse = P.row_fuse && m->wT_valid;
  if (m->fj1 && !row_fuse) { x.rc = flag_join_fallback(m, stream); m->fj1 = 0; if (x.rc) return x.rc; }
  if (row_fuse) x.bwd_fusion_fused();
  else if (P.skinny) x.bwd_fusion_skinny();
  else x.bwd_fusion_tiled();
  x.fusion_wgrads();
  if (x.rc) return x.rc;
  x.bwd_side_chain(row_fuse, t_ids, lengths);
  const float* xin[3] = {WS(m->lay.mod[0].x), v, a};
  for (int l = 1; l >= 0 && !x.rc && !P.enc_cut; --l) x.bwd_encoder_layer(l, xin, t_ids, lengths);
  if (x.rc) return x.rc;
  if (!m->ev.empty() && !P.enc_cached) { if (m->ev_seen_b % m->ev_stride == 0) m->ev_bwd++; m->ev_seen_b++; }
  if (P.fj_on && opt && !is_gru(m) && m->side_pending && m->jflags && m->adam_early_done > 0 &&
      m->adam_early_done == m->par.rnn1_begin) {
    x.rc = bg_join(m, m->side);
    if (!x.rc) x.rc = side_flag_signal(m, 1);
    m->fj2 = x.rc ? 0 : 1;
    return x.rc;
  }
  x.rc = side_join(m, stream);
  if (!x.rc && is_gru(m) && !P.enc_cut) {
    mmda_gru_pad_job gj[MMDA_GRU_PAD_MAX];
    int n = gru_jobs(m, m->G, true, gj);
    x.rc = mmda_gru_unpad_grads(gj, n, stream);
  }
  return x.rc;
}
}

extern "C" int mmda_misa_backward(mmda_misa* m, const int64_t* t_ids, const float* v, const float* a, const int32_t* lengths,
                                  void* stream) {
  if (!t_ids || !v || !a || !lengths) return MMDA_EINVAL;
  return backward_pass(m, t_ids, v, a, lengths, nullptr, stream);
}

extern "C" int mmda_misa_timing_end(mmda_misa* m) {
  if (!m) return MMDA_EINVAL;
  for (hipEvent_t e : m->ev) (void)hipEventDestroy(e);
  m->ev.clear(); m->ev_steps = m->ev_fwd = m->ev_bwd = 0; m->ev_seen_f = m->ev_seen_b = 0;
  return MMDA_OK;
}
extern "C" int mmda_misa_timing_stride(mmda_misa* m, int stride) {
  if (!m || stride < 1) return MMDA_EINVAL;
  m->ev_stride = stride;
  return MMDA_OK;
}
extern "C" int mmda_misa_timing_begin(mmda_misa* m, int max_steps) {
  if (!m || max_steps <= 0 || max_steps > 4096) return MMDA_EINVAL;
  mmda_misa_timing_end(m);
  m->ev.resize((size_t)max_steps * 8);
  for (auto& e : m->ev)
    if (hipEventCreateWithFlags(&e, hipEventDisableSystemFence) != hipSuccess) return MMDA_ELAUNCH;
  m->ev_steps = max_steps;
  m->ev_done.assign((size_t)max_steps * 4, 0);
  return MMDA_OK;
}
extern "C" int mmda_misa_timing_rotate(mmda_misa* m, int on) {
  if (!m) return MMDA_EINVAL;
  m->ev_rotate = on ? 1 : 0;
  return MMDA_OK;
}
extern "C" int mmda_misa_timing_collect(mmda_misa* m, float mean_ms[4], int* steps) {
  if (!m || !mean_ms || m->ev.empty()) return MMDA_EINVAL;
  int n = m->ev_fwd < m->ev_bwd ? m->ev_fwd : m->ev_bwd;
  if (n > m->ev_steps) n = m->ev_steps;
  double acc[4] = {0, 0, 0, 0};
  int cnt[4] = {0, 0, 0, 0};
  for (int s = 0; s < n; ++s)
    for (int k = 0; k < 4; ++k) {
      if ((size_t)(s * 4 + k) >= m->ev_done.size() || !m->ev_done[s * 4 + k]) continue;
      float ms = 0.f;
      if (hipEventSynchronize(m->ev[(s * 4 + k) * 2 + 1]) != hipSuccess) return MMDA_ELAUNCH;
      if (hipEventElapsedTime(&ms, m->ev[(s * 4 + k) * 2], m->ev[(s * 4 + k) * 2 + 1]) != hipSuccess) return MMDA_ELAUNCH;
      acc[k] += ms; cnt[k]++;
    }
  int least = n;
  for (int k = 0; k < 4; ++k) { mean_ms[k] = cnt[k] > 0 ? (float)(acc[k] / cnt[k]) : 0.f; least = cnt[k] < least ? cnt[k] : least; }
  if (steps) *steps = least;
  return MMDA_OK;
}

namespace {
int accum_append_rows(mmda_misa* m, const RowList& l, void* stream) {
  if (!m->eu.on || !m->ws || m->lay.T <= 0 || !l.ids || !l.rows) return MMDA_EINVAL;
  const PendingRows r = m->eu.take();
  return mmda_embed_rows_append(l.ids, l.rows, l.used, l.capacity, r.ids, WS(m->lay.mod[0].d_x), m->lay.B * m->lay.T, m->cfg.d_t, r.lengths, m->lay.B, stream);
}
bool accum_ready(const mmda_misa* m) { return m && m->P && m->G && !m->df_row_step; }
bool accum_list_ok(const mmda_misa* m, const RowList& l) {
  if (m->embed_update != EU_SPARSE) return true;
  const int64_t R = (int64_t)m->lay.B * m->lay.T;
  return m->eu.on && m->ws && m->lay.T > 0 && l.ids && l.rows && l.used >= 0 && l.used <= l.capacity && R <= l.capacity - l.used &&
         l.used + R <= INT32_MAX;
}

int opt_step_refused(const mmda_misa* m, const OptStep& o) {
  if (!m->P || !m->G || !m->M1 || !m->V1 || o.step < 1 || (o.norm && !m->ws)) return MMDA_EINVAL;
  return adam_settings_refused(m) ? MMDA_EINVAL : MMDA_OK;
}

int opt_step(mmda_misa* m, const OptStep& o, int64_t lo, const FlagWait& w, const RowList* list, void* stream) {
  int rc = masked(m) ? runs_ready(m, stream) : MMDA_OK;
  if (!rc && o.norm) rc = bucket_norm(m, o.acc, o.grad_scale, stream);
  if (!rc) rc = bucket_adam(m, lo, grad_floats(m), o.acc, o.lr, o.clip, o.grad_scale, o.step, w, stream, o.norm ? m->ws + m->lay.gnorm + 1 : nullptr);
  if (rc) return rc;
  float* const p = PP(m->par.embed); float* const m1 = m->M1 + m->par.embed; float* const v1 = m->V1 + m->par.embed; const mmda_adam_opts& h = m->adam;
  if (m->embed_update == EU_SPARSE && list) {
    const int n = (int)(list->used + (int64_t)m->lay.B * m->lay.T);
    rc = accum_append_rows(m, *list, stream);
    if (!rc) rc = mmda_embed_rows_sparse_adam(p, m1, v1, list->ids, n, m->cfg.d_t, list->rows, nullptr, 0, m->cfg.vocab, o.lr, h.beta1, h.beta2,
                                              h.eps, o.clip, o.grad_scale, o.step, stream);
  } else if (m->embed_update == EU_SPARSE && m->eu.on) {
    const PendingRows r = m->eu.take();
    if (!m->ws || m->lay.T <= 0) return MMDA_EINVAL;
    rc = mmda_embed_rows_sparse_adam(p, m1, v1, r.ids, m->lay.B * m->lay.T, m->cfg.d_t, WS(m->lay.mod[0].d_x), r.lengths, m->lay.B, m->cfg.vocab, o.lr, h.beta1,
                                     h.beta2, h.eps, o.clip, o.grad_scale, o.step, stream);
  } else if (m->embed_update == EU_DENSE && m->df_row_step && m->eu.on) {
    rc = mmda_misa_embed_deferred_step(m, o.lr, h.beta1, h.beta2, h.eps, o.clip, o.grad_scale, o.step, stream);
  }
  return rc;
}
}

extern "C" int mmda_misa_adam_step(mmda_misa* m, float lr, float clip, float grad_scale, int step, void* stream) {
  if (!m) return MMDA_EINVAL;
  const OptStep o{lr, clip, grad_scale, step, nullptr, m->clip_norm > 0.f};
  const int rc = opt_step_refused(m, o);
  return rc ? rc : opt_step(m, o, 0, kNoWait, nullptr, stream);
}

extern "C" int mmda_misa_grad_accumulate(mmda_misa* m, float* acc, int first, int64_t* list_ids, float* list_rows, int64_t list_used,
                                         int64_t list_capacity, void* stream) {
  const RowList l{list_ids, list_rows, list_used, list_capacity};
  if (!accum_ready(m) || !acc || !accum_list_ok(m, l)) return MMDA_EINVAL;
  int rc = mmda_grad_accumulate(acc, m->G, grad_floats(m), first, stream);
  if (!rc && m->embed_update == EU_SPARSE) rc = accum_append_rows(m, l, stream);
  return rc;
}

extern "C" int mmda_misa_adam_step_accumulated(mmda_misa* m, const float* acc, int64_t* list_ids, float* list_rows, int64_t list_used,
                                               int64_t list_capacity, float lr, float clip, float grad_scale, int step, void* stream) {
  const RowList l{list_ids, list_rows, list_used, list_capacity};
  if (!accum_ready(m) || !accum_list_ok(m, l)) return MMDA_EINVAL;
  const OptStep o{lr, clip, grad_scale, step, acc, m->clip_norm > 0.f};
  const int rc = opt_step_refused(m, o);
  return rc ? rc : opt_step(m, o, 0, kNoWait, &l, stream);
}

namespace {
int train_step_body(mmda_misa* m, const int64_t* t_ids, const float* v, const float* a, const int32_t* lengths, const mmda_encoded_batch* eb,
                    float* emo_gathered, const float* emo, int training, uint64_t seed, int do_adam, float lr, float clip, int step,
                    void* stream) {
  if (check_ready(m) || !m->G) return MMDA_EINVAL;
  const OptStep o{lr, clip, 1.0f, step, nullptr, do_adam && m->clip_norm > 0.f};
  const bool early = do_adam && !o.norm;
  int rc = do_adam ? opt_step_refused(m, o) : MMDA_OK;
  if (!rc && do_adam && masked(m)) rc = runs_ready(m, stream);
  if (rc) return rc;
  m->inference = 0;
  m->zero_grad_pending = m->lay.T > 0 ? 1 : 0;
  m->eager_done = 0; m->misc_deferred = nullptr;
  m->fj1 = m->fj2 = 0;
  const StepRequest req{true, emo, (early && !eb) ? &o : nullptr, eb != nullptr};
  rc = m->zero_grad_pending ? MMDA_OK : mmda_misa_zero_grad(m, stream);
  if (!rc) rc = eb ? forward_encoded(m, req, eb, emo_gathered, training, seed, stream) : forward_pass(m, req, t_ids, v, a, lengths, training, seed, stream);
  if (rc) return rc;
  if (m->zero_grad_pending) return MMDA_ELAUNCH;
  rc = mmda_misa_losses(m, emo, 1, stream);
  if (rc) return rc;
  rc = backward_pass(m, t_ids, v, a, lengths, early ? &o : nullptr, stream);
  if (rc) return rc;
  if (m->fj1) { rc = flag_join_fallback(m, stream); m->fj1 = 0; if (rc) return rc; }
  if (m->fj2 && !early) { rc = flag_join_fallback(m, stream); m->fj2 = 0; if (rc) return rc; }
  if (!do_adam) return MMDA_OK;
  const bool fj = m->fj2 != 0;
  m->fj2 = 0;
  const FlagWait w = fj ? FlagWait{m->jflags + 1, m->jval[1], m->jflags + 2} : kNoWait;
  if (!m->bg_active) return opt_step(m, o, m->adam_early_done, w, nullptr, stream);
  const int64_t lo = m->adam_early_done;
  return mmda_adam_tail_launch(m->P + lo, m->G + lo, m->M1 + lo, m->V1 + lo, m->par.embed - lo, bg_table(m), bg_hyper(m, o), w, stream);
}

int train_step(mmda_misa* m, const int64_t* t_ids, const float* v, const float* a, const int32_t* lengths, const mmda_encoded_batch* eb,
               float* emo_gathered, const float* emo, int training, uint64_t seed, int do_adam, float lr, float clip, int step,
               void* stream) {
  if (m) m->bg_active = 0;
  const int rc = train_step_body(m, t_ids, v, a, lengths, eb, emo_gathered, emo, training, seed, do_adam, lr, clip, step, stream);
  const int rj = (m && m->bg_pending) ? bg_join(m, stream) : MMDA_OK;
  return rc ? rc : rj;
}
}

extern "C" int mmda_misa_train_step(mmda_misa* m, const int64_t* t_ids, const float* v, const float* a, const int32_t* lengths,
                                    const float* emo, int training, uint64_t seed, int do_adam, float lr, float clip, int step,
                                    void* stream) {
  return train_step(m, t_ids, v, a, lengths, nullptr, nullptr, emo, training, seed, do_adam, lr, clip, step, stream);
}

extern "C" int mmda_misa_train_step_encoded(mmda_misa* m, const mmda_encoded_batch* eb, float* emo_out, int training, uint64_t seed,
                                            int do_adam, float lr, float clip, int step, void* stream) {
  if (check_ready(m) || !m->G || !encoded_batch_ok(m, eb) || !eb->tab_emo || !emo_out) return MMDA_EINVAL;
  if (!encoder_cut(m)) return MMDA_EINVAL;
  return train_step(m, nullptr, nullptr, nullptr, nullptr, eb, emo_out, emo_out, training, seed, do_adam, lr, clip, step, stream);
}

extern "C" int mmda_misa_encoded_collect(mmda_misa* m, float* tab_t, float* tab_v, float* tab_a, const int32_t* dst, int64_t base,
                                         void* stream) {
  if (!m || !m->ws || m->lay.B <= 0) return MMDA_EINVAL;
  return mmda_encoded_collect(tab_t ? WS(m->lay.mod[0].utt) : nullptr, tab_v ? WS(m->lay.mod[1].utt) : nullptr, tab_a ? WS(m->lay.mod[2].utt) : nullptr,
                              4 * m->par.mod[0].H, 4 * m->par.mod[1].H, 4 * m->par.mod[2].H, tab_t, tab_v, tab_a, dst, base, m->lay.B, stream);
}

extern "C" int mmda_misa_infer_collect(mmda_misa* m, const mmda_infer_out* out, const int32_t* dst, int64_t base, void* stream) {
  if (!m || !out || !m->ws || m->lay.B <= 0) return MMDA_EINVAL;
  const Workspace& w = m->lay;
  mmda_infer_src src = {};
  src.scores = WS(w.scores); src.labels = WS(w.labels); src.tcp = WS(w.tcp); src.hfused = WS(w.hfused); src.x6 = WS(w.x6);
  src.probs = WS(w.probs);
  src.ncls = m->cfg.ncls; src.hs = m->cfg.hidden; src.nhead = NHEAD;
  return mmda_infer_collect(&src, out, dst, base, w.B, stream);
}
```

mmda_amd/models.py:

```python
from __future__ import annotations

import ctypes as C
import math
import operator
import os
from typing import Dict, List, Tuple

import torch
import torch.nn as nn

from . import _lib, step_rules
from . import optim as _optim
from .config import activation_name

FFN_DIM = 2048
FUSION_DROPOUT = 0.1

_TOP_ORDER = ["activation", "embed", "trnn1", "trnn2", "vrnn1", "vrnn2", "arnn1", "arnn2", "project_t", "project_v", "project_a",
              "private_t", "private_v", "private_a", "shared", "recon_t", "recon_v", "recon_a", "discriminator",
              "sp_discriminator", "confidence", "classifier", "tlayer_norm", "vlayer_norm", "alayer_norm",
              "transformer_encoder"]
_RNN_ORDER = ["weight_ih_l0", "weight_hh_l0", "bias_ih_l0", "bias_hh_l0", "weight_ih_l0_reverse", "weight_hh_l0_reverse",
              "bias_ih_l0_reverse", "bias_hh_l0_reverse"]

# ... 72 lines not shown
            raise ValueError("config.accum_steps must be an int >= 1")

        step_rules.task_check(getattr(config, "task", "emotion"), getattr(config, "senti_loss", "l1"), num_classes=self.output_size,
                              use_confidNet=bool(getattr(config, "use_confidNet", False)), pos_weight=getattr(config, "pos_weight", None),
                              focal_gamma=getattr(config, "focal_gamma", 0.0))

        lib = _lib.load()
        cc = _lib.MisaConfig(
            vocab=len(config.word2id), d_t=self.text_size, d_v=self.visual_size, d_a=self.acoustic_size,
            hidden=config.hidden_size, ncls=config.num_classes, act=_lib.ACT[self.activation_name],
            use_cmd_sim=int(bool(config.use_cmd_sim)), use_confidNet=int(bool(getattr(config, "use_confidNet", False))),
            dropout=float(config.dropout), fusion_dropout=FUSION_DROPOUT, threshold=float(config.threshold),
            reverse_grad_weight=float(getattr(config, "reverse_grad_weight", 1.0)),
            diff_weight=float(getattr(config, "diff_weight", 0.3)), sim_weight=float(getattr(config, "sim_weight", 0.7)),
            recon_weight=float(getattr(config, "recon_weight", 0.7)), conf_weight=float(getattr(config, "conf_weight", 0.3)),
            mode=_lib.BF16 if self.precision == "bf16" else _lib.F32, rnncell=_lib.CELL[self.rnncell])
        h = C.c_void_p()
        _lib.check(lib.mmda_misa_create(C.byref(cc), C.byref(h)), "mmda_misa_create")
        self._h = h
        self._lib = lib
        self.fusion_fp8 = bool(getattr(config, "fusion_fp8", False))
        if self.fusion_fp8:
            _lib.check(lib.mmda_misa_set_fusion_fp8(h, 1), "set_fusion_fp8")
        _lib.check(lib.mmda_misa_set_embed_update(h, EMBED_UPDATE[self.embed_update]), "set_embed_update")
        pw = getattr(config, "pos_weight", None)
        if isinstance(pw, str) and pw != "balanced":
            raise ValueError("config.pos_weight must be None, a list of num_classes floats or 'balanced'")
        self.task, self.senti_loss = "emotion", "l1"
        self.set_cls_loss(None if isinstance(pw, str) else pw, getattr(config, "focal_gamma", 0.0))
        self.set_task(getattr(config, "task", "emotion"), getattr(config, "senti_loss", "l1"))
        self._layout: Dict[str, Tuple[int, Tuple[int, ...]]] = {}
        self._native_names: List[str] = []
        for i in range(lib.mmda_misa_num_params(h)):
            name, off, rows, cols = C.c_char_p(), C.c_int64(), C.c_int(), C.c_int()
            _lib.check(lib.mmda_misa_param_info(h, i, C.byref(name), C.byref(off), C.byref(rows), C.byref(cols)))
            shape = (rows.value, cols.value) if cols.value > 0 else (rows.value,)
            self._layout[name.value.decode()] = (off.value, shape)
            self._native_names.append(name.value.decode())
        self._flat_floats = lib.mmda_misa_flat_floats(h)
        self._dense_floats = lib.mmda_misa_dense_floats(h)
        self._names: List[str] = sorted(self._layout, key=_reference_sort_key)
        self._aliases: Dict[str, str] = {}
        if "activation.weight" in self._layout:
            after = {f"project_{m_}.project_{m_}.bias": f"project_{m_}.project_{m_}_activation.weight" for m_ in "tva"}
            after["discriminator.discriminator_layer_1.bias"] = "discriminator.discriminator_layer_1_activation.weight"
            names = []
            for n_ in self._names:
                names.append(n_)
                if n_ in after:
                    names.append(after[n_])
                    self._aliases[after[n_]] = "activation.weight"
            self._names = names
        for name in self._names:
            if name in self._aliases:
                self._layout[name] = self._layout[self._aliases[name]]
                self._register(name, None, shared=self._get(self._aliases[name]))
            else:
                self._register(name, self._layout[name][1])
        self._plist = [(n, self._get(n)) for n in self._names]
        self.reset_parameters()
        if self.embed_update == "frozen":
            self.embed.weight.requires_grad_(False)
        self._native_params = [self._get(n) for n in self._native_names]
        self._embed_index = self._native_names.index("embed.weight")
        self._trainable_sent = (True,) * len(self._native_names)
        self._trainable_sends = 0
        self._runs_cache = None
        self._cut_flags = None
        self._rules_passed = None
        self._adam_pushed = _ADAM_DEFAULTS
        self._df_row_step = self._df_ring = None
        self._df_dirty = False
        self._rows_pending = False
        self._rows_clip = None
        self._rows_keep = None

        self._acc = None
        self._acc_list = None
        self._acc_used = 0
        self._acc_next = 0
        self._acc_count = 1

        self._P = self._G = self._M = self._V = None
        self._ws = None
        self._ws_shape = None
        self._len_dev = None
        self._len_cache = None
        self._fwd_id = 0
        self._step = 0
        self._seed = 0x5EED
        self._anchor = None
        self._last = {}
        self._abort_seen = False
        self._seg_work = None

    def _register(self, dotted: str, shape, shared=None):
        mod = self
        parts = dotted.split(".")
        for p in parts[:-1]:
            if not hasattr(mod, p):
                mod.add_module(p, _Bag())
            mod = getattr(mod, p)
        mod.register_parameter(parts[-1], shared if shared is not None else nn.Parameter(torch.empty(shape, dtype=torch.float32)))

    def _get(self, dotted: str) -> nn.Parameter:
        mod = self
        for p in dotted.split("."):
            mod = getattr(mod, p)
        return mod

    @torch.no_grad()
    def reset_parameters(self):
        for name, p in self._plist:
            if name.endswith("activation.weight"):
                p.fill_(0.25)
            elif name == "embed.weight":
                p.normal_(0.0, 1.0)
            elif "rnn" in name.split(".")[0]:
                h = self._layout[name.rsplit(".", 1)[0] + ".weight_hh_l0"][1][1]
                k = 1.0 / math.sqrt(h)
                p.uniform_(-k, k)
            elif "layer_norm" in name or ".norm1." in name or ".norm2." in name:
                p.fill_(1.0 if name.endswith("weight") else 0.0)
            elif name.endswith("in_proj_weight"):
                nn.init.xavier_uniform_(p)
            elif name.endswith("in_proj_bias") or name.endswith("out_proj.bias"):
                p.zero_()
            elif name.endswith("weight"):
                k = 1.0 / math.sqrt(p.shape[1])
                p.uniform_(-k, k)
            else:
                w = self._get(name[:-4] + "weight")
                k = 1.0 / math.sqrt(w.shape[1])
                p.uniform_(-k, k)

    def _apply(self, fn, *args, **kwargs):
        self.flush_embedding()
        out = super()._apply(fn, *args, **kwargs)
        self._P = None
        return out

    def _views_valid(self) -> bool:
        if self._P is None:
            return False
        base = self._P.data_ptr()
        for name, p in self._plist:
            if p.data_ptr() != base + 4 * self._layout[name][0]:
                return False
        return True

    @torch.no_grad()
    def _materialize(self, device):
        if device.type != "cuda":
            raise _lib.MMDAError("mmda_amd.MISA runs on an MI355X only (no CPU fallback); move the model with .to('cuda')")
        P = torch.zeros(self._flat_floats, dtype=torch.float32, device=device)
        for name, p in self._plist:
            off, shape = self._layout[name]
            n = p.numel()
            P[off:off + n].copy_(p.data.reshape(-1))
            p.data = P[off:off + n].view(shape)
        self._P = P
        if self._G is None or self._G.device != device:
            self._G = torch.zeros_like(P)
            self._M = torch.zeros_like(P)
            self._V = torch.zeros_like(P)
        for name, p in self._plist:
            off, shape = self._layout[name]
            p.grad = None
        _lib.check(self._lib.mmda_misa_bind(self._h, P.data_ptr(), self._G.data_ptr(), self._M.data_ptr(), self._V.data_ptr()),
                   "mmda_misa_bind")
        self._ws_shape = None
        if self.embed_update == "deferred":
            self._bind_deferred()

    def _bind_deferred(self):
        V = self._layout["embed.weight"][1][0]
        dev = self._P.device
        if self._df_row_step is None or self._df_row_step.device != dev:
            self._df_row_step = torch.zeros(V, dtype=torch.int32, device=dev)
            self._df_ring = torch.zeros(int(self._lib.mmda_embed_deferred_scalar_floats(self.embed_window)), dtype=torch.float32, device=dev)
        _lib.check(self._lib.mmda_misa_set_embed_deferred(self._h, self._df_row_step.data_ptr(), self._df_ring.data_ptr(), self.embed_window,
                                                          _lib.stream_ptr()), "set_embed_deferred")
        self._df_dirty = False

    def flush_embedding(self):
        if self.embed_update != "deferred" or not self._df_dirty or self._P is None or not self._views_valid():
            return
        _lib.check(self._lib.mmda_misa_embed_flush(self._h, _lib.stream_ptr()), "embed_flush")
        self._df_dirty = False

    def state_dict(self, *args, **kwargs):
        self.flush_embedding()
        return super().state_dict(*args, **kwargs)

    def load_state_dict(self, state_dict, *args, **kwargs):
        self.flush_embedding()
        out = super().load_state_dict(state_dict, *args, **kwargs)
        if self.embed_update == "deferred" and self._P is not None and self._views_valid():
            self._bind_deferred()
        return out

    def set_embed_update(self, mode: str):
        if not isinstance(mode, str) or mode not in EMBED_UPDATE:
            raise ValueError("embed_update must be 'dense', 'sparse', 'frozen' or 'deferred'")
        self.flush_embedding()
        bound = self._P is not None and self._views_valid()
        if self.embed_update == "deferred":
            _lib.check(self._lib.mmda_misa_set_embed_deferred(self._h, None, None, 0, _lib.stream_ptr()), "set_embed_deferred")
        _lib.check(self._lib.mmda_misa_set_embed_update(self._h, EMBED_UPDATE[mode]), "set_embed_update")
        self.embed_update = mode
        if mode == "deferred" and self.embed_window < 1:
            self.embed_window = int(os.environ.get("MMDA_EMBED_WINDOW", 0) or getattr(self.config, "embed_deferred_window", 256))
        self._rows_pending = False
        self._rows_clip = None
        self._cut_flags = None
        self.embed.weight.requires_grad_(mode != "frozen")
        if mode != "dense":
            self.embed.weight.grad = None
        if mode == "deferred" and bound:
            self._bind_deferred()

    def set_cls_loss(self, pos_weight=None, focal_gamma: float = 0.0):
        w, g = step_rules.cls_setting(pos_weight, focal_gamma, self.output_size)
        step_rules.task_check(self.task, self.senti_loss, num_classes=self.output_size, pos_weight=w, focal_gamma=g)
        _lib.check(self._lib.mmda_misa_set_cls_loss(self._h, _lib.cls_opts(w, g)), "mmda_misa_set_cls_loss")
        self.cls_loss = dict(pos_weight=w, focal_gamma=g)
        return self.cls_loss

    def set_task(self, task: str = "emotion", senti_loss: str = "l1"):
        step_rules.task_check(task, senti_loss, num_classes=self.output_size,
                              use_confidNet=bool(getattr(self.config, "use_confidNet", False)),
                              pos_weight=self.cls_loss["pos_weight"], focal_gamma=self.cls_loss["focal_gamma"])
        _lib.check(self._lib.mmda_misa_set_task(self._h, _lib.TASK[task], _lib.SENTI_LOSS[senti_loss if task == "sentiment" else "l1"]),
                   "mmda_misa_set_task")
        self.task, self.senti_loss = task, (senti_loss if task == "sentiment" else self.senti_loss)
        return self.task

    def _match(self, prefixes) -> List[str]:
        names = []
        for pre in prefixes:
            hit = [n for n in self._names if n.startswith(pre)]
            if not isinstance(pre, str) or not pre or not hit:
                raise ValueError(f"no parameter of the state dict begins with {pre!r}")
            names += [n for n in hit if n not in names]
        return [n for n in self._names if n in names]

    def freeze(self, *prefixes: str) -> List[str]:
        names = self._match(prefixes)
        for n in names:
            self._get(n).requires_grad_(False)
        return names

    def unfreeze(self, *prefixes: str) -> List[str]:
        names = self._match(prefixes)
        if "embed.weight" in names and self.embed_update == "frozen":
            raise _lib.MMDAError("embed.weight is frozen by embed_update='frozen': switch the mode with set_embed_update('dense')")
        for n in names:
            self._get(n).requires_grad_(True)
        return names

    def _trainable_flags(self) -> Tuple[bool, ...]:
        flags = tuple(map(_REQUIRES_GRAD, self._native_params))
        if self.embed_update == "frozen" and flags[self._embed_index]:
            flags = flags[:self._embed_index] + (False,) + flags[self._embed_index + 1:]
        return flags

    def frozen_names(self, beyond_embed_update: bool = False) -> List[str]:
        out = [n for n in self._names if not self._get(n).requires_grad]
        if beyond_embed_update and self.embed_update == "frozen":
            out = [n for n in out if n != "embed.weight"]
        return out

    def _sync_trainable(self, exchange: bool = False) -> Tuple[bool, ...]:
        flags = self._trainable_flags()
        if flags == self._trainable_sent and not exchange and (flags[self._embed_index] or self.embed_update not in ("sparse", "deferred")):
            return flags
        frozen = [n for n, f in zip(self._native_names, flags) if not f]
        if "embed.weight" in frozen and self.embed_update in ("sparse", "deferred"):
            raise _lib.MMDAError(f"embed.weight.requires_grad=False under embed_update='{self.embed_update}': freeze the table with "
# ... 62 lines not shown
        lmin, lmax = int(lens.min()), int(lens.max())
        if lmin <= 0:
            raise RuntimeError("Length of all samples has to be greater than 0")
        if lmax > T:
            raise RuntimeError("a length exceeds the padded sequence length")
        self._carve(B, T, dev)
        lens32 = lens.to(device="cpu", dtype=torch.int32)
        cached = self._len_cache
        if cached is not None and cached[0].shape == lens32.shape and torch.equal(cached[0], lens32) and cached[1].device == dev:
            len_dev = cached[1]
        else:
            pin = torch.empty(B, dtype=torch.int32, pin_memory=True)
            pin.copy_(lens32)
            len_dev = pin.to(device=dev, non_blocking=True)
            self._len_cache = (lens32.clone(), len_dev, pin)
        t = sentences.contiguous()
        if t.dtype != torch.int64:
            t = t.long()
        v = video.contiguous().float()
        a = acoustic.contiguous().float()
        return t, v, a, len_dev

    def _carve(self, B: int, T: int, dev):
        if self._ws_shape != (B, T):
            need = self._lib.mmda_misa_workspace_floats(self._h, B, T)
            if self._ws is None or self._ws.numel() < need or self._ws.device != dev:
                if self._ws is not None and self._ws_shape is not None:
                    self._abort_seen = self._abort_seen or self.cluster_aborted()
                self._ws = torch.zeros(need, dtype=torch.float32, device=dev)
            _lib.check(self._lib.mmda_misa_set_workspace_async(self._h, self._ws.data_ptr(), self._ws.numel(), B, T, _lib.stream_ptr()),
                       "set_workspace")
            self._ws_shape = (B, T)

    def _off(self, name: str) -> int:
        o = self._lib.mmda_misa_tensor_offset(self._h, name.encode())
        if o < 0:
            raise KeyError(name)
        return o

    def _ws_view(self, name: str, shape):
        n = 1
        for s in shape:
            n *= s
        o = self._off(name)
        return self._ws[o:o + n].view(shape)

    def _public(self) -> Dict[str, torch.Tensor]:
        B, _ = self._ws_shape
        hs, nc = self.config.hidden_size, self.config.num_classes
        x6 = self._ws_view("x6", (6, B, hs))
        orig = self._ws_view("orig", (3, B, hs))
        recon = self._ws_view("recon", (3, B, hs))
        out = {"scores": self._ws_view("scores", (B, nc)), "tcp": self._ws_view("tcp", (B, 6)),
               "labels": self._ws_view("labels", (B, nc))}
        for i, m in enumerate("tva"):
            out[f"utt_{m}_orig"] = orig[i]
            out[f"utt_private_{m}"] = x6[i]
            out[f"utt_shared_{m}"] = x6[3 + i]
            out[f"utt_{m}_recon"] = recon[i]
        if not self.config.use_cmd_sim:
            dom = self._ws_view("dom", (3, B, 3))
            for i, m in enumerate("tva"):
                out[f"domain_label_{m}"] = dom[i]
        return out

    def _grad_slots(self) -> Dict[str, torch.Tensor]:
        B, _ = self._ws_shape
        hs, nc = self.config.hidden_size, self.config.num_classes
        dx6 = self._ws_view("d_x6", (6, B, hs))
        dorig = self._ws_view("d_orig", (3, B, hs))
        drec = self._ws_view("d_recon", (3, B, hs))
        out = {"scores": self._ws_view("d_scores", (B, nc)), "tcp": self._ws_view("d_tcp", (B, 6))}
        for i, m in enumerate("tva"):
            out[f"utt_{m}_orig"] = dorig[i]
            out[f"utt_private_{m}"] = dx6[i]
            out[f"utt_shared_{m}"] = dx6[3 + i]
            out[f"utt_{m}_recon"] = drec[i]
        if not self.config.use_cmd_sim:
            ddom = self._ws_view("d_dom", (3, B, 3))
            for i, m in enumerate("tva"):
                out[f"domain_label_{m}"] = ddom[i]
        return out

    def _next_seed(self) -> int:
        self._seed = (self._seed * 6364136223846793005 + 1442695040888963407) & 0xFFFFFFFFFFFFFFFF
        return self._seed

    def _forward_raw(self, t, v, a, len_dev, training: bool, seed: int, inference: bool = False):
        if not inference:
            self._sync_trainable()
        _lib.check(self._lib.mmda_misa_set_inference(self._h, int(inference)), "set_inference")
        _lib.check(self._lib.mmda_misa_forward(self._h, t.data_ptr(), v.data_ptr(), a.data_ptr(), len_dev.data_ptr(),
                                               int(training), seed, _lib.stream_ptr()), "mmda_misa_forward")
        self._fwd_id += 1
        self._last = dict(t=t, v=v, a=a, len_dev=len_dev)

    def alignment(self, sentences, visual, acoustic, lengths, bert_sent=None, bert_sent_type=None, bert_sent_mask=None):
        t, v, a, len_dev = self._prepare(sentences, visual, acoustic, lengths)
        seed = self._next_seed()
        if torch.is_grad_enabled():
            if self._anchor is None or self._anchor.device != t.device:
                self._anchor = torch.zeros(1, device=t.device, requires_grad=True)
            outs = _MISAFn.apply(self._anchor, self, t, v, a, len_dev, self.training, seed)
            named = dict(zip(_PUB, outs[:-1]))
            labels = outs[-1]
        else:
            self._forward_raw(t, v, a, len_dev, self.training, seed, inference=True)
            pub = self._public()
            named = {k: pub[k].clone() if k in pub else None for k in _PUB}
            labels = pub["labels"].clone()
        for k in _PUB:
            if k in ("scores",):
                continue
            val = named.get(k)
            if k.startswith("domain_label") and self.config.use_cmd_sim:
                val = None
            setattr(self, k, val)
        return named["scores"], labels

    def forward(self, sentences, video, acoustic, lengths, bert_sent=None, bert_sent_type=None, bert_sent_mask=None):
        return self.alignment(sentences, video, acoustic, lengths, bert_sent, bert_sent_type, bert_sent_mask)

    @property
    def utt_t(self):
        return self.utt_private_t + self.utt_shared_t

    @property
    def utt_v(self):
        return self.utt_private_v + self.utt_shared_v

    @property
    def utt_a(self):
        return self.utt_private_a + self.utt_shared_a

    def _sp_disc(self, x):
        from . import ops
        w = self.sp_discriminator.sp_discriminator_layer_1.weight
        b = self.sp_discriminator.sp_discriminator_layer_1.bias
        return ops.gemm(x.detach().contiguous(), w.detach(), mode="fp32", bias=b.detach())

    @property
    def shared_or_private_p_t(self):
        return self._sp_disc(self.utt_private_t)

    @property
    def shared_or_private_p_v(self):
        return self._sp_disc(self.utt_private_v)

    @property
    def shared_or_private_p_a(self):
        return self._sp_disc(self.utt_private_a)

    @property
    def shared_or_private_s(self):
        return self._sp_disc((self.utt_shared_t + self.utt_shared_v + self.utt_shared_a) / 3.0)

    def train_step(self, sentences, video, acoustic, lengths, emo_label, lr: float, clip: float, do_adam: bool = True,
                   training: bool = True, seed=None, grad_sync=None, optimizer=None, accum_index: int = 0, accum_count: int = 1,
                   clip_norm=None):
        if accum_count != 1 or accum_index != 0 or self._acc_next:
            return self._accum_micro_step(sentences, video, acoustic, lengths, emo_label, lr, clip, do_adam, training, seed, grad_sync,
                                          optimizer, accum_index, accum_count, clip_norm)
        (t, v, a, len_dev), emo, seed, custom, adam = self._step_begin((sentences, video, acoustic, lengths), emo_label, optimizer, clip_norm,
                                                                       do_adam, seed, exchange=grad_sync is not None)
        s = _lib.stream_ptr()
        fused_adam = do_adam and grad_sync is None and not custom
        gs_owner = getattr(grad_sync, "__self__", None)
        global_stats = getattr(gs_owner, "global_stats", False) and (gs_owner.world > 1 or gs_owner.force_collectives)
        if global_stats:
            self._global_stats_step(t, v, a, len_dev, emo, training, seed, gs_owner)
        else:
            _lib.check(self._lib.mmda_misa_train_step(self._h, t.data_ptr(), v.data_ptr(), a.data_ptr(), len_dev.data_ptr(),
                                                      emo.data_ptr(), int(training), seed, int(fused_adam), lr, clip, max(self._step, 1), s),
                       "mmda_misa_train_step")
        rows = self.embed_update in ("sparse", "deferred") and not fused_adam
        self._step_end(dict(t=t, v=v, a=a, len_dev=len_dev, emo=emo), rows, (t, len_dev) if rows else None, forwarded=not global_stats)
        self._df_dirty = self._df_dirty or (self.embed_update == "deferred" and fused_adam)
        if not do_adam or fused_adam:
            return
        step_no = max(self._step, 1)
        early = None
        if not custom:
            def early(n_floats, stream, _gs=1.0 / float(getattr(gs_owner, "world", 1))):
                self._adam_range(0, int(n_floats), lr, clip, _gs, step_no, stream.cuda_stream, adam, "adam(early)")
        scale, done = self._exchange(grad_sync, early) if grad_sync is not None else (1.0, 0)
        if custom:
            optimizer.step(clip_value=clip, grad_scale=scale)
        elif done > 0:
            self._adam_range(done, self.grad_floats - done, lr, clip, scale, step_no, s, adam, "adam(rest)")
        else:
            _lib.check(self._lib.mmda_misa_adam_step(self._h, lr, clip, scale, self._step, s), "adam_step")

    def _step_begin(self, batch, emo_label, optimizer, clip_norm, do_adam, seed, exchange=False, accumulate=False, encoded=False):
        if encoded:
            io, adam = self._encoded_begin(batch, "train_step_encoded", optimizer, clip_norm, exchange, accumulate, do_adam)
            if batch.cache.emo is None:
                raise _lib.MMDAError("train_step_encoded: the cache has no emotion labels (its dataset had none)")
            if batch.cache.task != self.task:
                raise _lib.MMDAError(f"train_step_encoded: the cache's label table was stored under task='{batch.cache.task}', the model's "
                                     f"task is '{self.task}': rebuild it (EncoderCache.build)")
            self._send_adam(adam)
            emo = torch.empty(batch.B, self.config.num_classes, dtype=torch.float32, device=batch.cache.device)
        else:
            adam = self._send_adam(self._rules(optimizer, clip_norm, exchange, accumulate, False, do_adam))
            self._sync_trainable(exchange=exchange)
            io = self._prepare(*batch)
            emo = emo_label.to(device=io[0].device, dtype=torch.float32).contiguous()
            if self.task == "sentiment" and emo.numel() != io[0].shape[1]:
                raise ValueError(f"task='sentiment' takes the (B,) or (B, 1) sentiment column: the target has {emo.numel()} entries, the "
                                 f"batch {io[0].shape[1]} samples")
        if seed is None:
            seed = self._next_seed()
        custom = do_adam and optimizer is not None and not isinstance(optimizer, _optim.Adam)
        if not custom and not accumulate:
            self._step += 1
        return io, emo, seed, custom, adam

    def _step_end(self, last, rows_pending=False, rows_keep=None, forwarded=True):
        if forwarded:
            self._fwd_id += 1
        self._last = last
        self._rows_pending, self._rows_clip, self._rows_keep = rows_pending, None, rows_keep

    def _exchange(self, grad_sync, early=None):
        owner = getattr(grad_sync, "__self__", None)
        hook = early is not None and all(hasattr(owner, x) for x in ("early_step", "early_stepped", "world"))
        if hook:
            owner.early_step = early
        try:
            scale = grad_sync(self._G, self._dense_floats, self) if _takes_model(grad_sync) else grad_sync(self._G, self._dense_floats)
        finally:
            if hook:
                owner.early_step = None
        return float(scale), (int(owner.early_stepped) if hook else 0)

    def _rules(self, optimizer=None, clip_norm=None, exchange=False, accumulate=False, encoded=False, do_adam=True):
        key = optimizer.settings() if isinstance(optimizer, _optim.Adam) else _ADAM_DEFAULTS[:5]
        case = (self.embed_update, type(optimizer), key[3], clip_norm, exchange, accumulate, encoded, do_adam)
        if case != self._rules_passed:
            kind, name = _optim.rule_kind(optimizer)
            step_rules.check(embed_update=self.embed_update, optimizer=kind, optimizer_name=name, weight_decay=key[3], clip_norm=clip_norm,
                             exchange=exchange, accumulate=accumulate, encoded=encoded, do_adam=do_adam)
            self._rules_passed = case
        return key + (0.0 if clip_norm is None else float(clip_norm),)

    def _send_adam(self, key):
        if key != self._adam_pushed:
            if self.embed_update == "deferred" and key[:3] != self._adam_pushed[:3]:
                self.flush_embedding()
            opts = _lib.AdamOpts(beta1=key[0], beta2=key[1], eps=key[2], weight_decay=key[3], decoupled=int(key[4]), scale_dev=None)
            _lib.check(self._lib.mmda_misa_set_adam(self._h, C.byref(opts), key[5]), "mmda_misa_set_adam")
            self._adam_pushed = key
        return key

    def _push_adam(self, optimizer, clip_norm, exchange: bool = False):
        return self._send_adam(self._rules(optimizer, clip_norm, exchange))

    def _adam_range(self, first: int, n: int, lr, clip, grad_scale, step, stream, adam, what: str):
        ptrs = [x.data_ptr() + first * 4 for x in (self._P, self._G, self._M, self._V)]
        _optim.clamp_adam(self._lib, *ptrs, n, None, lr, clip, grad_scale, step, adam, None, stream, what)

    def grad_norm(self) -> torch.Tensor:
        if self._ws is None:
            raise _lib.MMDAError("grad_norm(): no step has run yet")
        return self._ws_view("grad_norm", (2,))[0]

    def _encoded_begin(self, batch, what: str, optimizer=None, clip_norm=None, exchange=False, accumulate=False, do_adam=True):
        from .encoded import EncodedBatch
        if not isinstance(batch, EncodedBatch):
            raise TypeError(f"{what} takes an EncodedBatch (EncodedLoader yields them), not {type(batch).__name__}")
        dist = torch.distributed
        adam = self._rules(optimizer, clip_norm, exchange or (dist.is_available() and dist.is_initialized() and dist.get_world_size() > 1),
                           accumulate or self.accum_steps > 1 or bool(self._acc_next), True, do_adam)
        cache = batch.cache
        cache._refuse(self)
        flags = self._sync_trainable()
        if flags != self._cut_flags:
            if not self.trainable_info()[2]:
                from .encoded import ENCODER_PREFIXES
                live = [n for n, f in zip(self._native_names, flags) if f and n.split(".")[0] in ENCODER_PREFIXES]
                if self.embed_update in ("sparse", "deferred"):
                    live.append(f"embed.weight (embed_update='{self.embed_update}' trains the table through its rows)")
                raise _lib.MMDAError(f"{what} needs the encoder cut -- every recurrent layer, the three inter-layer LayerNorms and the "
                                     f"table frozen (MISA.freeze): the cached rows are constants only then.  Still trainable: {live}")
            self._cut_flags = flags
        if cache.device.type != "cuda":
            raise _lib.MMDAError(f"{what}: the cache is on {cache.device}: mmda_amd.MISA has no CPU path (HIP kernels only)")
        if not self._views_valid():
            self._materialize(cache.device)
        self._carve(batch.B, 1, cache.device)
        return _lib.EncodedBatch(tab_t=cache.utt_t.data_ptr(), tab_v=cache.utt_v.data_ptr(), tab_a=cache.utt_a.data_ptr(),
                                 tab_emo=_lib.ptr(cache.emo), rows=batch.rows_ptr, B=batch.B), adam

    def train_step_encoded(self, batch, lr: float, clip: float, do_adam: bool = True, training: bool = True, seed=None, optimizer=None,
                           grad_sync=None, accum_index: int = 0, accum_count: int = 1, clip_norm=None):
        eb, emo, seed, custom, _ = self._step_begin(batch, None, optimizer, clip_norm, do_adam, seed, exchange=grad_sync is not None,
                                                    accumulate=accum_index != 0 or accum_count != 1, encoded=True)
        _lib.check(self._lib.mmda_misa_train_step_encoded(self._h, C.byref(eb), emo.data_ptr(), int(training), seed, int(do_adam and not custom),
                                                          lr, clip, max(self._step, 1), _lib.stream_ptr()), "mmda_misa_train_step_encoded")
        self._step_end(dict(encoded=batch, emo=emo))
        if custom:
            optimizer.step(clip_value=clip, grad_scale=1.0)

    def forward_encoded(self, batch, keep=None):
        if keep is not None:
            from .modality import parse_keep
            step_rules.modality_check(parse_keep(keep), encoded=True)
        if torch.is_grad_enabled():
            raise _lib.MMDAError("autograd through forward_encoded is not built: call it under torch.no_grad() (train with train_step_encoded)")
        eb, _ = self._encoded_begin(batch, "forward_encoded")
        eb.tab_emo = None
        seed = self._next_seed()
        _lib.check(self._lib.mmda_misa_set_inference(self._h, 1), "set_inference")
        _lib.check(self._lib.mmda_misa_forward_encoded(self._h, C.byref(eb), int(self.training), seed, _lib.stream_ptr()),
                   "mmda_misa_forward_encoded")
        self._fwd_id += 1
        self._last = dict(encoded=batch)
        pub = self._public()
        for k in _PUB:
            if k == "scores":
                continue
            val = pub[k].clone() if k in pub else None
            if k.startswith("domain_label") and self.config.use_cmd_sim:
                val = None
            setattr(self, k, val)
        return pub["scores"].clone(), pub["labels"].clone()

    def _accum_micro_step(self, sentences, video, acoustic, lengths, emo_label, lr, clip, do_adam, training, seed, grad_sync, optimizer,
                          index, count, clip_norm=None) -> None:
        expected, self._acc_next = self._acc_next, 0
        self._acc_used = 0 if expected == 0 else self._acc_used
        for x in (index, count):
            if isinstance(x, bool) or not isinstance(x, int):
                raise _lib.MMDAError("accum_index / accum_count must be ints")
        if count < 1 or not 0 <= index < count:
            raise _lib.MMDAError(f"accum_index {index} is outside [0, accum_count = {count})")
        if index != expected or (index > 0 and count != self._acc_count):
            raise _lib.MMDAError(f"accumulated step: micro-batch {index} of {count} arrived where {expected} of "
                                 f"{self._acc_count if expected else count} was due (indices run 0 .. count - 1 with one count); "
                                 "the sequence starts over")
        (t, v, a, len_dev), emo, seed, _, _ = self._step_begin((sentences, video, acoustic, lengths), emo_label, optimizer, clip_norm, do_adam,
                                                               seed, exchange=grad_sync is not None, accumulate=True)
        s = _lib.stream_ptr()
        lib, h = self._lib, self._h
        _lib.check(lib.mmda_misa_train_step(h, t.data_ptr(), v.data_ptr(), a.data_ptr(), len_dev.data_ptr(), emo.data_ptr(), int(training),
                                            seed, 0, lr, clip, max(self._step, 1), s), "mmda_misa_train_step")
        self._step_end(dict(t=t, v=v, a=a, len_dev=len_dev, emo=emo))
        closing = index == count - 1
        n = self.grad_floats
        if count > 1 and (self._acc is None or self._acc.numel() < n or self._acc.device != t.device):
            if index > 0:
                raise _lib.MMDAError("accumulated step: the gradient bucket changed size or device between micro-batches")
            self._acc = torch.empty(n, dtype=torch.float32, device=t.device)
        ids_p = rows_p = None
        cap = 0
        if self.embed_update == "sparse":
            D = self._layout["embed.weight"][1][1]
            need = self._acc_used + t.numel()
            old = self._acc_list
            if old is None or old[0].numel() < need or old[0].device != t.device:
                room = max(need, count * t.numel())
                ids = torch.empty(room, dtype=torch.int64, device=t.device)
                rows = torch.empty((room, D), dtype=torch.float32, device=t.device)
                if old is not None and self._acc_used > 0:
                    ids[:self._acc_used].copy_(old[0][:self._acc_used])
                    rows[:self._acc_used].copy_(old[1][:self._acc_used])
                self._acc_list = (ids, rows)
            ids_p, rows_p, cap = self._acc_list[0].data_ptr(), self._acc_list[1].data_ptr(), self._acc_list[0].numel()
        if not closing:
            _lib.check(lib.mmda_misa_grad_accumulate(h, self._acc.data_ptr(), int(index == 0), ids_p, rows_p, self._acc_used, cap, s),
                       "mmda_misa_grad_accumulate")
            self._acc_used += t.numel()
            self._acc_next, self._acc_count = index + 1, count
            return
        self._step += 1
        _lib.check(lib.mmda_misa_adam_step_accumulated(h, self._acc.data_ptr() if count > 1 else None, ids_p, rows_p, self._acc_used, cap,
                                                       lr, clip, 1.0 / count, self._step, s), "mmda_misa_adam_step_accumulated")
        self._acc_used = 0

    def _global_stats_step(self, t, v, a, len_dev, emo, training: bool, seed: int, dp) -> None:
        lib, h, cfg = self._lib, self._h, self.config
        if not cfg.use_cmd_sim:
            raise NotImplementedError("global_stats: the CMD similarity branch only (config.use_cmd_sim)")
        s = _lib.stream_ptr()
        W, r = int(dp.world), int(dp.rank)
        _lib.check(lib.mmda_misa_zero_grad(h, s), "zero_grad")
        self._forward_raw(t, v, a, len_dev, training, seed, inference=False)
        _lib.check(lib.mmda_misa_zero_act_grads(h, s), "zero_act_grads")
        B, _ = self._ws_shape
        hs, nc = int(cfg.hidden_size), int(cfg.num_classes)
        Bg = W * B
        L = self._ws_view("losses", (8,))
        X = dp.gather_rows(self._ws_view("x6", (6, B, hs)), dim=1)
        dX = torch.zeros_like(X)
        work = torch.empty(int(lib.mmda_loss_diff_work_floats(Bg, hs)), dtype=torch.float32, device=X.device)
        _lib.check(lib.mmda_loss_diff(X.data_ptr(), Bg * hs, Bg, hs, float(getattr(cfg, "diff_weight", 0.3)), L.data_ptr() + 4, dX.data_ptr(),
                                      work.data_ptr(), s), "loss_diff(global)")
        _lib.check(lib.mmda_loss_cmd(X[3:].data_ptr(), Bg * hs, Bg, hs, float(getattr(cfg, "sim_weight", 0.7)), L.data_ptr() + 8,
                                     dX[3:].data_ptr(), s), "loss_cmd(global)")
        self._ws_view("d_x6", (6, B, hs)).add_(dX[:, r * B:(r + 1) * B], alpha=float(W))
        if nc == 6:
            S = dp.gather_rows(self._ws_view("scores", (B, nc)))
            Tc = dp.gather_rows(self._ws_view("tcp", (B, 6)))
            E = dp.gather_rows(emo)
            with_g = bool(getattr(cfg, "use_confidNet", False))
            dS = torch.zeros_like(S) if with_g else None
            dT = torch.zeros_like(Tc) if with_g else None
            _lib.check(lib.mmda_loss_conf(S.data_ptr(), Tc.data_ptr(), E.data_ptr(), Bg, nc, float(getattr(cfg, "conf_weight", 0.3)),
                                          L.data_ptr() + 16, dS.data_ptr() if with_g else None, dT.data_ptr() if with_g else None, s),
                       "loss_conf(global)")
            if with_g:
                self._ws_view("d_scores", (B, nc)).add_(dS[r * B:(r + 1) * B], alpha=float(W))
                self._ws_view("d_tcp", (B, 6)).add_(dT[r * B:(r + 1) * B], alpha=float(W))
        _lib.check(lib.mmda_misa_set_external_batch_losses(h, 1), "set_external_batch_losses")
        try:
            _lib.check(lib.mmda_misa_losses(h, emo.data_ptr(), 1, s), "mmda_misa_losses")
        finally:
            lib.mmda_misa_set_external_batch_losses(h, 0)
        _lib.check(lib.mmda_misa_backward(h, t.data_ptr(), v.data_ptr(), a.data_ptr(), len_dev.data_ptr(), s), "mmda_misa_backward")
        self._gs_keep = (X, dX, work)

    def early_grad_floats(self) -> int:
        return int(self._lib.mmda_misa_early_grad_floats(self._h))

    def wait_early_grads(self, stream) -> None:
        _lib.check(self._lib.mmda_misa_wait_early_grads(self._h, stream.cuda_stream), "wait_early_grads")

    def embedding_grad_rows(self):
        if self.embed_update == "frozen":
            raise _lib.MMDAError("embed_update='frozen': no gradient with respect to the embedding rows is computed")
        t = self._last["t"]
        T, B = t.shape
        R = T * B
        pad = torch.arange(T, device=t.device, dtype=torch.int32).unsqueeze(1) >= self._last["len_dev"].unsqueeze(0)
        ids = torch.where(pad, torch.full_like(t, -1), t)
        return ids.reshape(R), self._ws_view("d_x_t", (R, self._layout["embed.weight"][1][1]))

    def embedding_rows_per_step(self):
        return None if not getattr(self, "_last", None) else int(self._last["t"].numel())

    def embedding_table_rows(self):
        return int(self._layout["embed.weight"][1][0])

    def scatter_embedding_rows(self, ids: torch.Tensor, rows: torch.Tensor):
        if ids.numel() == 0:
            return
        off, (V, D) = self._layout["embed.weight"]
        g = self._G[off:off + V * D]
        _lib.check(self._lib.mmda_embed_scatter_add(g.data_ptr(), ids.contiguous().data_ptr(), ids.numel(), D,
                                                    rows.contiguous().data_ptr(), _lib.stream_ptr()), "embed_scatter_add")

    def set_embedding_grad_rows(self, ids: torch.Tensor, rows: torch.Tensor):
        n = ids.numel()
        if n == 0:
            return
        off, (V, D) = self._layout["embed.weight"]
        g = self._G[off:off + V * D]
        need = int(self._lib.mmda_embed_segment_sum_work_bytes(n, D))
# ... 142 lines not shown
```

Measured before the change: 55380 samples/s.

## Cache bf16 packed recurrent and transposed weight operands across steps via parameter token

Adds an operand cache keyed by a host-supplied parameter token. It lets the forward pass skip re-packing LSTM hidden weights, converting input weights and transposing fusion weights when the parameters have not changed since the last build. The cache is dropped whenever Adam steps a parameter range, on rebind, on mode switches or on errors, and Python bumps the token after every write. The gain only appears when parameters are not updated between calls, such as inference, frozen layers or accumulation micro-steps. In a normal train step, where every step updates the weights, it adds bookkeeping without skipping any work.

```diff
diff --git a/include/mmda_hip.h b/include/mmda_hip.h
--- a/include/mmda_hip.h
+++ b/include/mmda_hip.h
@@ -429,6 +429,12 @@
 int mmda_misa_set_mode(mmda_misa* m, int mode);
 int mmda_misa_set_recurrence(mmda_misa* m, int resident_weights);
 int mmda_misa_set_gemm_operands(mmda_misa* m, int bf16_copies);
+int mmda_misa_set_param_token(mmda_misa* m, uint64_t token);
+typedef struct mmda_operand_cache_info {
+  int enabled, token_known; uint64_t token; int have[3]; int64_t reused[3], made[3];
+} mmda_operand_cache_info;
+int mmda_misa_operand_cache_describe(const mmda_misa* m, mmda_operand_cache_info* out);
+int mmda_operand_cache_sim(const int64_t* events, int n_events, int* out);
 int mmda_misa_set_inference(mmda_misa* m, int forward_only);
 int mmda_misa_set_fusion_fp8(mmda_misa* m, int on);
 int mmda_misa_set_embed_update(mmda_misa* m, int mode);
diff --git a/mmda_amd/_lib.py b/mmda_amd/_lib.py
--- a/mmda_amd/_lib.py
+++ b/mmda_amd/_lib.py
@@ -54,6 +54,11 @@
                 ("drop_p", C.c_float), ("drop_seed", C.c_uint64), ("drop_site", C.c_int),
                 ("gate", C.c_void_p), ("ldgate", C.c_int), ("gate_scale", C.c_float),
                 ("dsig", C.c_void_p), ("dsig2", C.c_void_p), ("lddsig", C.c_int)]
+
+
+class OperandCacheInfo(C.Structure):
+    _fields_ = [("enabled", C.c_int), ("token_known", C.c_int), ("token", C.c_uint64), ("have", C.c_int * 3), ("reused", C.c_int64 * 3),
+                ("made", C.c_int64 * 3)]
 
 
 class TransposeJob(C.Structure):
@@ -323,6 +328,9 @@
     "mmda_misa_set_mode": (_I, [_P, _I]),
     "mmda_misa_set_overlap": (_I, [_P, _I]),
     "mmda_misa_set_recurrence": (_I, [_P, _I]),
+    "mmda_misa_set_param_token": (_I, [_P, C.c_uint64]),
+    "mmda_misa_operand_cache_describe": (_I, [_P, C.POINTER(OperandCacheInfo)]),
+    "mmda_operand_cache_sim": (_I, [C.POINTER(C.c_int64), _I, C.POINTER(C.c_int)]),
     "mmda_misa_set_gemm_operands": (_I, [_P, _I]),
     "mmda_misa_early_grad_floats": (_I64, [_P]),
     "mmda_misa_wait_early_grads": (_I, [_P, _P]),
diff --git a/mmda_amd/csrc/lstm.hip b/mmda_amd/csrc/lstm.hip
--- a/mmda_amd/csrc/lstm.hip
+++ b/mmda_amd/csrc/lstm.hip
@@ -538,9 +538,9 @@
                                              int ntjobs, const RowStamp* st, void* stream) {
   if (!jobs || njobs < 0 || njobs > CONV_MAX) return MMDA_EINVAL;
   if (st && (!st->stamp || !st->ids || st->n < 0 || st->table_rows <= 0)) return MMDA_EINVAL;
-  PackMulti P;
+  PackMulti P = {};
   int pblocks = 0, cblocks = 0, tblocks = 0;
-  int rc = pack_build(MMDA_BF16, n, H, whh, packed_fwd, packed_bwd, packed_c, P, pblocks);
+  int rc = n == 0 ? MMDA_OK : pack_build(MMDA_BF16, n, H, whh, packed_fwd, packed_bwd, packed_c, P, pblocks);
   if (rc) return rc;
   ConvLaunch L;
   rc = conv_build(jobs, njobs, L, cblocks);
@@ -558,6 +558,7 @@
 extern "C" int mmda_lstm_pack_convert_transpose(int n, const int* H, const float* const* whh, void* const* packed_fwd,
                                                 void* const* packed_bwd, void* const* packed_c, const mmda_convert_job* jobs, int njobs,
                                                 const mmda_transpose_job* tjobs, int ntjobs, void* stream) {
+  if (n <= 0) return MMDA_EINVAL;
   return mmda_lstm_pack_convert_transpose_stamped(n, H, whh, packed_fwd, packed_bwd, packed_c, jobs, njobs, tjobs, ntjobs, nullptr, stream);
 }
 
diff --git a/mmda_amd/csrc/misa.hip b/mmda_amd/csrc/misa.hip
--- a/mmda_amd/csrc/misa.hip
+++ b/mmda_amd/csrc/misa.hip
@@ -1,4 +1,5 @@
 #include "step_plan.h"
+#include "operand_cache.h"
 #include <algorithm>
 #include <cstring>
 
@@ -69,6 +70,7 @@
   int64_t early_floats = 0; int early_valid = 0;
   int64_t adam_early_done = 0;
   int wT_valid = 0;
+  OperandCache oc;
   int wT_pending = 0;
   PendingRows eu;
   int df_seq = 0, df_flushed = 0;
@@ -423,6 +425,15 @@
       mmda_env_int("MMDA_EMBED_BG_LATE", d.embed_bg_late), mmda_env_int("MMDA_EMBED_BG_LDS", d.embed_bg_lds)};
   return sw;
 }
+int operand_cache_switch() {
+  static const int on = mmda_env_int("MMDA_OPERAND_CACHE", 1);
+  return on;
+}
+bool oc_usable(const mmda_misa* m) { return m->oc.on && !is_gru(m); }
+unsigned oc_layer_forms(const StepPlan& P) {
+  return OCF_PACK_F | (P.want_b ? OCF_PACK_B : 0u) | (P.want_c ? OCF_PACK_C : 0u) | OCF_WIH | (P.enc_nostash ? 0u : OCF_WIH_T) |
+         (P.gm ? OCF_GATE_MINOR : OCF_GATE_MAJOR);
+}
 PlanInput plan_input(const mmda_misa* m, const StepRequest& r, int B, int T) {
   PlanInput in = {};
   in.cfg = m->cfg; in.B = B; in.T = T;
@@ -445,6 +456,7 @@
   if (cfg->mode != MMDA_F32 && cfg->mode != MMDA_BF16) return MMDA_EINVAL;
   if (cfg->rnncell != MMDA_CELL_LSTM && cfg->rnncell != MMDA_CELL_GRU) return MMDA_EINVAL;
   mmda_misa* m = new mmda_misa(*cfg);
+  m->oc.on = operand_cache_switch() != 0;
   if (apply_trainable(m, nullptr)) { delete m; return MMDA_EINVAL; }
   *out = m;
   return MMDA_OK;
@@ -481,6 +493,7 @@
   if (!m || !params) return MMDA_EINVAL;
   if (((uintptr_t)params | (uintptr_t)grads | (uintptr_t)adam_m | (uintptr_t)adam_v) & 15) return MMDA_EINVAL;
   m->P = params; m->G = grads; m->M1 = adam_m; m->V1 = adam_v;
+  m->oc.drop_all();
   return MMDA_OK;
 }
 extern "C" int64_t mmda_misa_workspace_floats(const mmda_misa* m, int B, int T) {
@@ -522,6 +535,7 @@
   if (!keep && m->xchg_ws == ws) { int rc = harvest_abort(m); if (rc) return rc; }
   m->rebind(w);
   m->ws = ws;
+  m->oc.drop_all();
   hipStream_t s = (hipStream_t)stream;
   if (!keep) {
     for (int i = 0; i < 3; ++i)
@@ -542,6 +556,7 @@
 extern "C" int mmda_misa_set_mode(mmda_misa* m, int mode) {
   if (!m || (mode != MMDA_F32 && mode != MMDA_BF16)) return MMDA_EINVAL;
   m->cfg.mode = mode;
+  m->oc.drop_all();
   return MMDA_OK;
 }
 extern "C" int mmda_misa_set_overlap(mmda_misa* m, int side_stream) {
@@ -552,11 +567,51 @@
 extern "C" int mmda_misa_set_recurrence(mmda_misa* m, int resident_weights) {
   if (!m) return MMDA_EINVAL;
   m->use_cluster = resident_weights ? 1 : 0;
+  m->oc.drop_all();
   return MMDA_OK;
 }
 extern "C" int mmda_misa_set_gemm_operands(mmda_misa* m, int bf16_copies) {
   if (!m) return MMDA_EINVAL;
   m->use_bf16_gemm = bf16_copies ? 1 : 0;
+  m->oc.drop_all();
+  return MMDA_OK;
+}
+extern "C" int mmda_misa_set_param_token(mmda_misa* m, uint64_t token) {
+  if (!m) return MMDA_EINVAL;
+  m->oc.set_token(token);
+  return MMDA_OK;
+}
+extern "C" int mmda_misa_operand_cache_describe(const mmda_misa* m, mmda_operand_cache_info* out) {
+  if (!m || !out) return MMDA_EINVAL;
+  *out = mmda_operand_cache_info{};
+  out->enabled = oc_usable(m) ? 1 : 0; out->token_known = m->oc.token_known ? 1 : 0; out->token = m->oc.token;
+  for (int g = 0; g < OC_GROUPS; ++g) {
+    out->have[g] = (int)m->oc.have[g]; out->reused[g] = m->oc.reused[g]; out->made[g] = m->oc.made[g];
+  }
+  return MMDA_OK;
+}
+extern "C" int mmda_operand_cache_sim(const int64_t* events, int n_events, int* out) {
+  if (n_events < 0 || (n_events > 0 && (!events || !out))) return MMDA_EINVAL;
+  OperandCache c;
+  for (int i = 0; i < n_events; ++i) {
+    const int64_t kind = events[3 * i], a = events[3 * i + 1], b = events[3 * i + 2];
+    int ans = 0;
+    const bool group_ok = a >= 0 && a < OC_GROUPS;
+    switch (kind) {
+      case OCE_TOKEN: c.set_token((uint64_t)a); break;
+      case OCE_TAKE:
+        if (!group_ok || b < 0) return MMDA_EINVAL;
+        ans = c.take((int)a, (unsigned)b) ? 1 : 0;
+        if (!ans) c.note_made((int)a, (unsigned)b);
+        break;
+      case OCE_STEPPED: if (!group_ok || b < 0) return MMDA_EINVAL; c.note_stepped((int)a, (unsigned)b); break;
+      case OCE_DROP: if (a == -1) c.drop_all(); else if (group_ok) c.drop((int)a); else return MMDA_EINVAL; break;
+      case OCE_SWITCH: c.on = a != 0; if (!c.on) c.drop_all(); break;
+      default: return MMDA_EINVAL;
+    }
+    out[4 * i] = ans;
+    for (int g = 0; g < OC_GROUPS; ++g) out[4 * i + 1 + g] = (int)c.have[g];
+  }
   return MMDA_OK;
 }
 extern "C" int64_t mmda_misa_early_grad_floats(const mmda_misa* m) {
@@ -615,7 +670,15 @@
   const int rc = mmda_transpose_f32(tj.data(), (int)tj.size(), ss);
   m->wT_valid = rc ? 0 : 1;
   m->wT_pending = 0;
+  if (!rc && oc_usable(m)) m->oc.note_made(OC_FUSION, OCF_WT); else m->oc.drop(OC_FUSION);
   return rc;
+}
+
+void oc_note_stepped(mmda_misa* m, int64_t lo, int64_t hi) {
+  const ParamTable& p = m->par;
+  const int64_t gb[OC_GROUPS] = {0, p.rnn2_begin, p.rnn1_begin}, ge[OC_GROUPS] = {p.rnn2_begin, p.rnn1_begin, p.dense};
+  for (int g = 0; g < OC_GROUPS; ++g)
+    if (ge[g] > lo && gb[g] < hi) m->oc.drop(g);
 }
 
 int backward_only_jobs(mmda_misa* m, mmda_convert_job* cj) {
@@ -899,10 +962,15 @@
 }
 
 void Pass::fwd_operands(const int64_t* t_ids, const float* const* xin) {
+  const bool oc_on = P.bfg && oc_usable(m);
+  const unsigned lforms = oc_layer_forms(P);
+  bool held[2] = {false, false};
+  for (int l = 0; l < 2; ++l) held[l] = oc_on && m->oc.take(l == 0 ? OC_L1 : OC_L2, lforms);
   auto first_jobs = [&](bool transposed, mmda_convert_job* cj) -> int {
     int n = 0;
     for (int i = 0; i < 3; ++i) {
       for (int l = 0; l < 2; ++l) {
+        if (held[l]) continue;
         const RnnP& r = p.mod[i].rnn[l]; const RnnW& rw = w.mod[i].rnn[l];
         cj[n++] = mmda_convert_job{rW_ih(m, i, l), r.D, 8 * r.H, r.D, nullptr, WS(rw.wb), r.ldD,
                                    transposed ? WS(rw.wbT) : nullptr, transposed ? r.ldG : 0, P.gm ? r.H : 0};
@@ -919,24 +987,32 @@
   int k = 0;
   for (int i = 0; i < 3; ++i)
     for (int l = 0; l < 2; ++l)
-      for (int d = 0; d < 2; ++d, ++k) {
+      for (int d = 0; d < 2; ++d) {
+        if (held[l]) continue;
         const RnnP& r = p.mod[i].rnn[l]; const RnnW& rw = w.mod[i].rnn[l];
         Hs[k] = r.H; Wp[k] = rW_hh(m, i, l, d); Fp[k] = WS(rw.pack_f[d]); Bp[k] = P.want_b ? WS(rw.pack_b[d]) : nullptr; Cp[k] = WS(rw.pack_c[d]);
+        ++k;
       }
   m->wT_valid = 0;
   if (P.bfg) {
     mmda_convert_job cj[9];
     const int nj = first_jobs(!P.enc_nostash, cj);
     std::vector<mmda_transpose_job> tj;
-    if (P.wT_merge) weight_transpose_jobs(m, tj);
+    const bool wT_held = P.want_wT && oc_on && m->oc.take(OC_FUSION, OCF_WT);
+    if (P.wT_merge && !wT_held) weight_transpose_jobs(m, tj);
     if (tj.size() > 20) tj.clear();
     RowStamp st;
     if (P.embed_bg) rc = bg_begin(m, t_ids, R, s, &st);
-    if (!rc) rc = mmda_lstm_pack_convert_transpose_stamped(12, Hs, Wp, Fp, Bp, P.want_c ? Cp : nullptr, cj, nj, tj.data(), (int)tj.size(),
+    if (!rc) rc = mmda_lstm_pack_convert_transpose_stamped(k, Hs, Wp, Fp, Bp, P.want_c ? Cp : nullptr, cj, nj, tj.data(), (int)tj.size(),
                                                            P.embed_bg ? &st : nullptr, s);
-    m->wT_pending = (P.want_wT && tj.empty()) ? 1 : 0;
+    m->wT_pending = (P.want_wT && !wT_held && tj.empty()) ? 1 : 0;
     if (!tj.empty()) m->wT_valid = rc ? 0 : 1;
+    if (wT_held) m->wT_valid = 1;
+    for (int l = 0; l < 2; ++l)
+      if (!held[l]) { if (!rc && oc_on) m->oc.note_made(l == 0 ? OC_L1 : OC_L2, lforms); else m->oc.drop(l == 0 ? OC_L1 : OC_L2); }
+    if (!tj.empty()) { if (!rc && oc_on) m->oc.note_made(OC_FUSION, OCF_WT); else m->oc.drop(OC_FUSION); }
   } else {
+    m->oc.drop(OC_L1); m->oc.drop(OC_L2);
     void* ss = nullptr;
     rc = side_fork(m, s, &ss);
     if (!rc) rc = mmda_lstm_pack_whh_multi(mode, 12, Hs, Wp, Fp, Bp, P.want_c ? Cp : nullptr, ss);
@@ -1166,6 +1242,7 @@
   Pass x(m, stream, req.emo, req.opt);
   m->wT_valid = 0;
   m->wT_pending = m->plan.want_wT ? 1 : 0;
+  if (m->wT_pending && oc_usable(m) && m->oc.take(OC_FUSION, OCF_WT)) { m->wT_valid = 1; m->wT_pending = 0; }
   x.rc = mmda_encoded_gather(eb->tab_t, eb->tab_v, eb->tab_a, 4 * m->par.mod[0].H, 4 * m->par.mod[1].H, 4 * m->par.mod[2].H,
                              emo_out ? eb->tab_emo : nullptr, m->cfg.ncls, eb->rows, m->lay.B, WS(m->lay.mod[0].utt), WS(m->lay.mod[1].utt),
                              WS(m->lay.mod[2].utt), emo_out, stream);
@@ -1591,6 +1668,7 @@
     m->early_valid = 1;
     if (!rc && opt && m->early_floats > 0 && m->M1 && m->V1) {
       rc = bucket_adam(m, 0, m->early_floats, nullptr, opt->lr, opt->clip, opt->grad_scale, opt->step, kNoWait, ss);
+      oc_note_stepped(m, 0, m->early_floats);
       if (!rc) m->adam_early_done = m->early_floats;
     }
   } else {
@@ -1748,6 +1826,7 @@
   int rc = masked(m) ? runs_ready(m, stream) : MMDA_OK;
   if (!rc && o.norm) rc = bucket_norm(m, o.acc, o.grad_scale, stream);
   if (!rc) rc = bucket_adam(m, lo, grad_floats(m), o.acc, o.lr, o.clip, o.grad_scale, o.step, w, stream, o.norm ? m->ws + m->lay.gnorm + 1 : nullptr);
+  oc_note_stepped(m, lo, grad_floats(m));
   if (rc) return rc;
   float* const p = PP(m->par.embed); float* const m1 = m->M1 + m->par.embed; float* const v1 = m->V1 + m->par.embed; const mmda_adam_opts& h = m->adam;
   if (m->embed_update == EU_SPARSE && list) {
@@ -1823,6 +1902,7 @@
   const FlagWait w = fj ? FlagWait{m->jflags + 1, m->jval[1], m->jflags + 2} : kNoWait;
   if (!m->bg_active) return opt_step(m, o, m->adam_early_done, w, nullptr, stream);
   const int64_t lo = m->adam_early_done;
+  oc_note_stepped(m, lo, m->par.embed);
   return mmda_adam_tail_launch(m->P + lo, m->G + lo, m->M1 + lo, m->V1 + lo, m->par.embed - lo, bg_table(m), bg_hyper(m, o), w, stream);
 }
 
@@ -1832,6 +1912,7 @@
   if (m) m->bg_active = 0;
   const int rc = train_step_body(m, t_ids, v, a, lengths, eb, emo_gathered, emo, training, seed, do_adam, lr, clip, step, stream);
   const int rj = (m && m->bg_pending) ? bg_join(m, stream) : MMDA_OK;
+  if (m && rc) m->oc.drop_all();
   return rc ? rc : rj;
 }
 }
diff --git a/mmda_amd/csrc/operand_cache.h b/mmda_amd/csrc/operand_cache.h
--- /dev/null
+++ b/mmda_amd/csrc/operand_cache.h
@@ -0,0 +1,37 @@
+#pragma once
+#include <cstdint>
+
+namespace mmda_step {
+
+enum { OC_FUSION = 0, OC_L2 = 1, OC_L1 = 2, OC_GROUPS = 3 };
+enum { OCF_PACK_F = 1, OCF_PACK_B = 2, OCF_PACK_C = 4, OCF_WIH = 8, OCF_WIH_T = 16, OCF_GATE_MAJOR = 32, OCF_GATE_MINOR = 64 };
+enum { OCF_WT = 1 };
+
+struct OperandCache {
+  bool on = true;
+  bool token_known = false; uint64_t token = 0;
+  unsigned have[OC_GROUPS] = {0u, 0u, 0u};
+  int64_t reused[OC_GROUPS] = {0, 0, 0}, made[OC_GROUPS] = {0, 0, 0};
+
+  void drop(int g) { have[g] = 0u; }
+  void drop_all() { for (int g = 0; g < OC_GROUPS; ++g) have[g] = 0u; }
+  void set_token(uint64_t t) {
+    if (!token_known || t != token) drop_all();
+    token = t; token_known = true;
+  }
+  bool holds(int g, unsigned want) const { return on && token_known && want != 0u && (have[g] & want) == want; }
+  bool take(int g, unsigned want) {
+    if (want == 0u) return true;
+    if (holds(g, want)) { ++reused[g]; return true; }
+    return false;
+  }
+  void note_made(int g, unsigned want) { if (on && token_known) { have[g] = want; ++made[g]; } else have[g] = 0u; }
+  void note_stepped(int g, unsigned with) {
+    have[g] = (on && token_known) ? with : 0u;
+  }
+};
+
+enum { OCE_TOKEN = 0 , OCE_TAKE = 1 ,
+       OCE_STEPPED = 2 , OCE_DROP = 3 , OCE_SWITCH = 4  };
+
+}
diff --git a/mmda_amd/models.py b/mmda_amd/models.py
--- a/mmda_amd/models.py
+++ b/mmda_amd/models.py
@@ -178,6 +178,7 @@
         self._acc_count = 1
 
         self._P = self._G = self._M = self._V = None
+        self._oc_writes, self._oc_sent = 0, None
         self._ws = None
         self._ws_shape = None
         self._len_dev = None
@@ -256,6 +257,7 @@
             P[off:off + n].copy_(p.data.reshape(-1))
             p.data = P[off:off + n].view(shape)
         self._P = P
+        self._params_written()
         if self._G is None or self._G.device != device:
             self._G = torch.zeros_like(P)
             self._M = torch.zeros_like(P)
@@ -291,6 +293,7 @@
 
     def load_state_dict(self, state_dict, *args, **kwargs):
         self.flush_embedding()
+        self._params_written()
         out = super().load_state_dict(state_dict, *args, **kwargs)
         if self.embed_update == "deferred" and self._P is not None and self._views_valid():
             self._bind_deferred()
@@ -519,6 +522,24 @@
                 out[f"domain_label_{m}"] = ddom[i]
         return out
 
+    def _param_token(self) -> None:
+        key = (self._P._version + sum([p._version for _, p in self._plist]), self._oc_writes)
+        if key != self._oc_sent:
+            _lib.check(self._lib.mmda_misa_set_param_token(self._h, ((key[0] & 0xFFFFFFFF) << 32) | (key[1] & 0xFFFFFFFF)), "set_param_token")
+            self._oc_sent = key
+
+    def _params_written(self) -> None:
+        self._oc_writes += 1
+
+    def parameters_changed(self) -> None:
+        self._params_written()
+
+    def operand_cache_info(self) -> Dict[str, object]:
+        info = _lib.OperandCacheInfo()
+        _lib.check(self._lib.mmda_misa_operand_cache_describe(self._h, C.byref(info)), "operand_cache_describe")
+        return dict(enabled=bool(info.enabled), token_known=bool(info.token_known), have=tuple(info.have), reused=tuple(info.reused),
+                    made=tuple(info.made))
+
     def _next_seed(self) -> int:
         self._seed = (self._seed * 6364136223846793005 + 1442695040888963407) & 0xFFFFFFFFFFFFFFFF
         return self._seed
@@ -527,6 +548,7 @@
         if not inference:
             self._sync_trainable()
         _lib.check(self._lib.mmda_misa_set_inference(self._h, int(inference)), "set_inference")
+        self._param_token()
         _lib.check(self._lib.mmda_misa_forward(self._h, t.data_ptr(), v.data_ptr(), a.data_ptr(), len_dev.data_ptr(),
                                                int(training), seed, _lib.stream_ptr()), "mmda_misa_forward")
         self._fwd_id += 1
@@ -607,6 +629,7 @@
         if global_stats:
             self._global_stats_step(t, v, a, len_dev, emo, training, seed, gs_owner)
         else:
+            self._param_token()
             _lib.check(self._lib.mmda_misa_train_step(self._h, t.data_ptr(), v.data_ptr(), a.data_ptr(), len_dev.data_ptr(),
                                                       emo.data_ptr(), int(training), seed, int(fused_adam), lr, clip, max(self._step, 1), s),
                        "mmda_misa_train_step")
@@ -621,6 +644,7 @@
             def early(n_floats, stream, _gs=1.0 / float(getattr(gs_owner, "world", 1))):
                 self._adam_range(0, int(n_floats), lr, clip, _gs, step_no, stream.cuda_stream, adam, "adam(early)")
         scale, done = self._exchange(grad_sync, early) if grad_sync is not None else (1.0, 0)
+        self._params_written()
         if custom:
             optimizer.step(clip_value=clip, grad_scale=scale)
         elif done > 0:
@@ -694,6 +718,7 @@
         return self._send_adam(self._rules(optimizer, clip_norm, exchange))
 
     def _adam_range(self, first: int, n: int, lr, clip, grad_scale, step, stream, adam, what: str):
+        self._params_written()
         ptrs = [x.data_ptr() + first * 4 for x in (self._P, self._G, self._M, self._V)]
         _optim.clamp_adam(self._lib, *ptrs, n, None, lr, clip, grad_scale, step, adam, None, stream, what)
 
@@ -733,10 +758,12 @@
                            grad_sync=None, accum_index: int = 0, accum_count: int = 1, clip_norm=None):
         eb, emo, seed, custom, _ = self._step_begin(batch, None, optimizer, clip_norm, do_adam, seed, exchange=grad_sync is not None,
                                                     accumulate=accum_index != 0 or accum_count != 1, encoded=True)
+        self._param_token()
         _lib.check(self._lib.mmda_misa_train_step_encoded(self._h, C.byref(eb), emo.data_ptr(), int(training), seed, int(do_adam and not custom),
                                                           lr, clip, max(self._step, 1), _lib.stream_ptr()), "mmda_misa_train_step_encoded")
         self._step_end(dict(encoded=batch, emo=emo))
         if custom:
+            self._params_written()
             optimizer.step(clip_value=clip, grad_scale=1.0)
 
     def forward_encoded(self, batch, keep=None):
@@ -749,6 +776,7 @@
         eb.tab_emo = None
         seed = self._next_seed()
         _lib.check(self._lib.mmda_misa_set_inference(self._h, 1), "set_inference")
+        self._param_token()
         _lib.check(self._lib.mmda_misa_forward_encoded(self._h, C.byref(eb), int(self.training), seed, _lib.stream_ptr()),
                    "mmda_misa_forward_encoded")
         self._fwd_id += 1
@@ -780,6 +808,7 @@
                                                                seed, exchange=grad_sync is not None, accumulate=True)
         s = _lib.stream_ptr()
         lib, h = self._lib, self._h
+        self._param_token()
         _lib.check(lib.mmda_misa_train_step(h, t.data_ptr(), v.data_ptr(), a.data_ptr(), len_dev.data_ptr(), emo.data_ptr(), int(training),
                                             seed, 0, lr, clip, max(self._step, 1), s), "mmda_misa_train_step")
         self._step_end(dict(t=t, v=v, a=a, len_dev=len_dev, emo=emo))
@@ -811,6 +840,7 @@
             self._acc_next, self._acc_count = index + 1, count
             return
         self._step += 1
+        self._params_written()
         _lib.check(lib.mmda_misa_adam_step_accumulated(h, self._acc.data_ptr() if count > 1 else None, ids_p, rows_p, self._acc_used, cap,
                                                        lr, clip, 1.0 / count, self._step, s), "mmda_misa_adam_step_accumulated")
         self._acc_used = 0
```

Result: no change. 55340 samples/s (median of 3 runs) (-0.1%).
